# aehogan/lammps-induced-dipole-polarization-pair-style

Hardware: AMD Instinct MI355X
Metric: atom-steps/sec (higher is better)
Workload: dtype f64

## Files before the change

### lammps-induced-dipole-polarization-pair-style_amd/csrc/lab/api_env_knobs.inc

```
  if (const char *e = getenv("POLAR_ABLATE")) h->ablate = atoi(e);
  if (const char *e = getenv("POLAR_HOST_COLORS")) h->host_colors = atoi(e) != 0;
  if (const char *e = getenv("POLAR_SWEEP_KERNEL")) h->sweep_kernel = atoi(e);
  if (const char *e = getenv("POLAR_TILE_WAVES")) h->tile_waves = atoi(e) == 8 ? 8 : 4;
  if (const char *e = getenv("POLAR_TILE_WIDE")) h->tile_wide = atoi(e) != 0;
  if (const char *e = getenv("POLAR_CACHE_R2")) h->cache_r2 = atoi(e);
  if (const char *e = getenv("POLAR_LJ_TYPED")) h->lj_typed = atoi(e) != 0;
  if (const char *e = getenv("POLAR_STATIC_XQ")) h->static_xq = atoi(e) != 0;
  if (const char *e = getenv("POLAR_POL_FIRST")) h->pol_first = atoi(e) != 0;
  if (const char *e = getenv("POLAR_LP_WG_PER_CU")) h->lp_wg_per_cu = atoi(e);
  if (const char *e = getenv("POLAR_LP_QM")) h->lp_quad_major = atoi(e) != 0;
  if (const char *e = getenv("POLAR_LP_TILES")) h->lp_tiles = atoi(e) == 1 ? 1 : 2;
  if (const char *e = getenv("POLAR_LP_ROWS")) h->lp_rows = std::max(1, std::min(64, atoi(e)));
  if (const char *e = getenv("POLAR_LP_PAIRS")) h->lp_pairs = atoi(e) != 0;
  if (const char *e = getenv("POLAR_CLUSTER_DIST")) h->cluster_dist = atof(e);
  if (const char *e = getenv("POLAR_CLUSTER_MAX")) h->cluster_max = std::max(1, std::min(4, atoi(e)));
  if (const char *e = getenv("POLAR_LP_DEPTH")) { int v = atoi(e); h->lp_depth = (v == 2 || v == 3) ? v : 0; }
  if (const char *e = getenv("POLAR_QUAD_BLOCK")) { int v = atoi(e); if (v >= 64 && v <= 1024 && v % 64 == 0) h->quad_block = v; }
  if (const char *e = getenv("POLAR_FIELD_BLOCK")) { int v = atoi(e); if (v >= 64 && v <= 1024 && v % 64 == 0) h->field_block = v; }
  if (const char *e = getenv("POLAR_FORCE_LITERAL")) h->force_literal = atoi(e) != 0;
  if (const char *e = getenv("POLAR_NL_DENSE")) h->nl_dense = atoi(e) != 0;
```

### lammps-induced-dipole-polarization-pair-style_amd/csrc/polar_api.hip

```cpp
#include "polar_handle.hpp"

namespace {
void upload_types(polar_handle *h, int ntypes, const double *const t[7]) {
  need_device(h);
  std::vector<double> pack;
  const double r_cmax = pack_lj_table(ntypes, t, pack);
  h->d_lj.ensure(pack.size());
  HIPCHECK(hipMemcpy(h->d_lj.p, pack.data(), pack.size() * sizeof(double), hipMemcpyHostToDevice));
  h->P.ntypes = ntypes;
  h->P.ljpack = h->d_lj.p;
  h->ntypes = ntypes;
  h->types_set = true;
  h->r_cmax = r_cmax;
  h->skin_valid = false;
}

void upload_coul(polar_handle *h, double g_ewald, double qqrd2e, const double *slj, const double *scoul, int nbits,
                 int mask, int shift, double tabinnersq, const double *const t[8]) {
  need_device(h);
  h->P.g_ewald = g_ewald; h->P.qqrd2e = qqrd2e;
  for (int k = 0; k < 4; k++) { h->P.special_lj[k] = slj[k]; h->P.special_coul[k] = scoul[k]; }
  h->P.ncoultablebits = nbits; h->P.ncoulmask = mask; h->P.ncoulshiftbits = shift; h->P.tabinnersq = tabinnersq;
  std::vector<double> pack;
  pack_coul_table(nbits, t, pack);
// ... 100 lines not shown
      const long long lo = t0 + cnt * part / nt, hi = t0 + cnt * (part + 1) / nt;
      int a = (int)(std::lower_bound(at.begin() + ii0, at.begin() + ii1, lo) - at.begin());
      const int b = (int)(std::lower_bound(at.begin() + ii0, at.begin() + ii1, hi) - at.begin());
      int worst = 0;
      for (; a < b; a++) {
        const int i = ilist[a], m = numneigh[i];
        const int *src = row(i);
        int *d = dst + (at[a] - t0);
        int mx = 0;
        for (int k = 0; k < m; k++) { const int v = src[k]; d[k] = v; const int j = v & 0x3FFFFFFF; mx = j > mx ? j : mx; }
        worst = mx > worst ? mx : worst;
      }
      if (worst >= nall) bad[(size_t)part * 16] = 1;
    }, nt);
    for (int t = 0; t < nt; t++) if (bad[(size_t)t * 16]) { HIPCHECK(hipStreamSynchronize(s)); throw InputError("neighbor index out of range"); }
    if (cnt > 0) HIPCHECK(hipMemcpyAsync(h->d_neigh.p + t0, dst, (size_t)cnt * sizeof(int), hipMemcpyHostToDevice, s));
    HIPCHECK(hipEventRecord(h->ev_nl[buf], s));
    ii0 = ii1; chunk++;
  }
  HIPCHECK(hipEventRecord(h->ev_list_up, s));
  h->list_up_pending = true;
  h->neigh_set = true;
  h->sym_valid = false; h->lj_ran = false;
  if (h->colors_valid) h->colors_recheck = true;
  h->device_list = false;
  h->full_list = h->user_full_list;
}
}


extern "C" {

const char *polar_kernel_version(void) { return POLAR_KERNEL_VERSION; }

int polar_device_count(void) {
  int n = 0;
  if (hipGetDeviceCount(&n) != hipSuccess) return 0;
  return n;
}

int polar_create(int device, polar_handle **out) {
  if (!out) return POLAR_ERR_STATE;
  polar_handle *h = new polar_handle();
  *out = h;
  h->device = device;
  if (const char *e = getenv("POLAR_COLOR_DIST")) h->color_dist = atof(e);
  h->color_keep = std::max(h->color_dist - 0.4, 0.75 * h->color_dist);
  if (const char *e = getenv("POLAR_COLOR_KEEP")) h->color_keep = atof(e);
  if (const char *e = getenv("POLAR_DETERMINISTIC")) h->deterministic = atoi(e) != 0;
#ifdef POLAR_LAB
#include "lab/api_env_knobs.inc"
#endif
  int n = polar_device_count();
  if (n <= 0 || device < 0 || device >= n) {
    h->have_device = false;
    h->err = "no usable HIP device";
    return POLAR_OK;
  }
  return guarded(h, [&]() {
    HIPCHECK(hipSetDevice(device));
    h->device_set = true;
    h->stream.create();
    for (auto &e : h->ev) e.create();
    {
      int prio_lo = 0, prio_hi = 0;
      HIPCHECK(hipDeviceGetStreamPriorityRange(&prio_lo, &prio_hi));
      h->lj_stream.create(hipStreamNonBlocking, prio_lo);
    }
    h->ev_fork.create(); h->ev_join.create();
    h->ev_lj0.create(); h->ev_lj1.create();
    h->ev_dl0.create(hipEventDisableTiming); h->ev_dl1.create(hipEventDisableTiming);
    h->ev_mu_ready.create(hipEventDisableTiming);
    for (auto &e : h->ev_fchunk) e.create(hipEventDisableTiming);
    for (auto &e : h->ev_ks) e.create();
    h->dl_stream.create(hipStreamNonBlocking);
    if (getenv("POLAR_NO_OVERLAP")) h->overlap_lj = false;
    if (const char *e = getenv("POLAR_LJ_PERS")) h->lj_pers = atoi(e);
    if (const char *e = getenv("POLAR_LJ_SKIN")) h->lj_skin = atoi(e) != 0;
    if (const char *e = getenv("POLAR_NL_INERT")) h->nl_inert = atoi(e) != 0;
    if (const char *e = getenv("POLAR_CELL_INERT")) h->cell_inert = atoi(e) != 0;
    if (const char *e = getenv("POLAR_LJ_PERS_THREADS")) h->lj_pers_threads = std::max(256, std::min(POLAR_LJ_PERS_THREADS, (atoi(e) / 64) * 64));
    { int ncu = 0; if (hipDeviceGetAttribute(&ncu, hipDeviceAttributeMultiprocessorCount, device) == hipSuccess) h->ncu = ncu; }
    h->h_scal.ensure(1);
    h->h_flags.ensure(16);
    h->h_ddtot.ensure(64 * 16);
    h->d_overflow.ensure(16); h->d_ddtot.ensure(64 * 16);
    h->d_scal.ensure(1);
    h->d_slots.ensure((size_t)POLAR_NSLOT * POLAR_SLOT_STRIDE);
    h->have_device = true;
    return POLAR_OK;
  });
}

int polar_destroy(polar_handle *h) {
  if (!h) return POLAR_OK;
  delete h;
  return POLAR_OK;
}

const char *polar_last_error(const polar_handle *h) { return h ? h->err.c_str() : "null handle"; }
const char *polar_last_warning(const polar_handle *h) { return h ? h->warn.c_str() : ""; }

int polar_pair_settings(polar_handle *h, int narg, const char *const *arg) {
  return guarded(h, [&]() { h->ph.settings(narg, arg); h->reset_plan(); return POLAR_OK; });
}
int polar_pair_coeff(polar_handle *h, int ntypes, int narg, const char *const *arg) {
  return guarded(h, [&]() { h->ph.coeff(ntypes, narg, arg); return POLAR_OK; });
}
int polar_pair_modify(polar_handle *h, int narg, const char *const *arg) {
  return guarded(h, [&]() { h->ph.modify(narg, arg); return POLAR_OK; });
}
int polar_pair_init(polar_handle *h, double g_ewald, double qqrd2e, const double special_lj[4],
                    const double special_coul[4]) {
  return guarded(h, [&]() {
    PairHost &p = h->ph;
    p.init(g_ewald, qqrd2e, special_lj, special_coul);
    h->coul_set = false;
    h->field_ready = false;
    if (h->have_device) {
      HIPCHECK(hipSetDevice(h->device));
      const double *t[7] = {p.lj1.data(), p.lj2.data(), p.lj3.data(), p.lj4.data(), p.offset.data(), p.cut_ljsq.data(), p.cutsq.data()};
      upload_types(h, p.ntypes, t);
      if (p.ncoultablebits == 0) {
        const double *c[8];
        double dummy = 0.0;
        for (int k = 0; k < 8; k++) c[k] = &dummy;
        upload_coul(h, g_ewald, qqrd2e, special_lj, special_coul, 0, 0, 0, 0.0, c);
      }
    }
    return POLAR_OK;
  });
}
double polar_pair_cut(const polar_handle *h, int i, int j) {
  if (!h || !h->ph.inited || i < 1 || j < 1 || i > h->ph.ntypes || j > h->ph.ntypes) return -1.0;
  return std::sqrt(h->ph.cutsq[(size_t)i * h->ph.w() + j]);
}
double polar_pair_single(const polar_handle *h, double qi, double qj, int itype, int jtype, double rsq,
                         double factor_coul, double factor_lj, double *fforce) {
  double ff = 0.0, e;
  try {
    e = h->ph.single(qi, qj, itype, jtype, rsq, factor_coul, factor_lj, ff);
  } catch (const std::exception &ex) {
    const_cast<polar_handle *>(h)->err = ex.what();
    e = ff = std::nan("");
  }
  if (fforce) *fforce = ff;
  return e;
}
const void *polar_pair_extract(const polar_handle *h, const char *name, int *dim) {
  if (!h || !name) return nullptr;
  if (dim) *dim = 0;
  if (strcmp(name, "cut_coul") == 0) return &h->ph.st.cut_coul;
  if (strcmp(name, "nl_dense") == 0) return &h->nl_dense_used;
  if (strcmp(name, "lj_walked") == 0 || strcmp(name, "lj_entries") == 0) {
    polar_handle *m = const_cast<polar_handle *>(h);
    if (guarded(m, [&]() { lj_counters(m); return POLAR_OK; }) != POLAR_OK) return nullptr;
    return name[3] == 'w' ? &h->lj_walked : &h->lj_entries;
  }
  if (strcmp(name, "cell_active") == 0) {
    polar_handle *m = const_cast<polar_handle *>(h);
    m->cell_active = 0.0;
    if (h->have_device && h->sorted && h->ph.st.dd_cutoff > 0.0 && h->ncell > 0 && h->d_cell_first.p) {
      long long v = 0;
      if (guarded(m, [&]() {
            HIPCHECK(hipSetDevice(m->device));
            HIPCHECK(hipMemcpyAsync(&v, m->d_cell_first.p + m->ncell, sizeof(v), hipMemcpyDeviceToHost, m->stream));
            HIPCHECK(hipStreamSynchronize(m->stream));
            return POLAR_OK;
          }) != POLAR_OK) return nullptr;
      m->cell_active = (double)v;
    }
    return &h->cell_active;
  }
  if (strcmp(name, "nl_entries") == 0 || strcmp(name, "force_rows") == 0) {
    polar_handle *m = const_cast<polar_handle *>(h);
    if (guarded(m, [&]() { inert_counters(m); return POLAR_OK; }) != POLAR_OK) return nullptr;
    return name[0] == 'n' ? &h->nl_entries : &h->force_rows;
  }
  if (strcmp(name, "ewald_field_at_ms") == 0) { if (dim) *dim = 1; return h->ew_fa_ms; }
  if (strcmp(name, "ewald_field_ms") == 0) { if (dim) *dim = 0; return &h->ew_field_ms; }
  if (dim) *dim = 2;
  if (strcmp(name, "epsilon") == 0) return h->ph.epsilon.data();
  if (strcmp(name, "sigma") == 0) return h->ph.sigma.data();
  if (strcmp(name, "cut_lj") == 0) return h->ph.cut_lj.data();
  return nullptr;
}
int polar_get_settings(const polar_handle *h, polar_settings *out) {
  if (!h || !out) return POLAR_ERR_STATE;
  *out = h->ph.st;
  return POLAR_OK;
}
int polar_restart_pack(const polar_handle *h, void *buf, int max_bytes) {
  if (!h) return POLAR_ERR_STATE;
  return restart_pack(h->ph.st, buf, max_bytes);
}
int polar_restart_unpack(polar_handle *h, const void *buf, int nbytes) {
  return guarded(h, [&]() {
    h->ph.st = restart_unpack(h->ph.st, buf, nbytes);
    h->reset_plan();
    return POLAR_OK;
  });
}
int polar_set_settings(polar_handle *h, const polar_settings *s) {
  return guarded(h, [&]() {
    check_solver_choice(*s);
    polar_settings v = *s;
    if (v.polar_sor == 0.0) v.polar_sor = 1.0;
    if (!(v.polar_sor > 0.0 && v.polar_sor < 2.0)) throw InputError("polar_sor must lie in (0, 2)");
    if (v.polar_accel < 0 || v.polar_accel > POLAR_ACCEL_MAX) throw InputError("polar_accel must lie in 0 .. 8");
    if (!(v.polar_ewald >= 0.0 && v.polar_ewald < 1.0)) throw InputError("polar_ewald must lie in [0, 1)");
    h->ph.st = v;
    h->colors_valid = false;
    h->field_ready = false;
    return POLAR_OK;
  });
}
int polar_set_types(polar_handle *h, int ntypes, const double *lj1, const double *lj2, const double *lj3,
                    const double *lj4, const double *offset, const double *cut_ljsq, const double *cutsq) {
  return guarded(h, [&]() {
    HIPCHECK(hipSetDevice(h->device));
    const double *t[7] = {lj1, lj2, lj3, lj4, offset, cut_ljsq, cutsq};
    upload_types(h, ntypes, t);
    return POLAR_OK;
  });
}
int polar_set_coul(polar_handle *h, double g_ewald, double qqrd2e, const double special_lj[4],
                   const double special_coul[4], int nbits, int mask, int shift, double tabinnersq,
                   const double *rtable, const double *drtable, const double *ftable, const double *dftable,
                   const double *ctable, const double *dctable, const double *etable, const double *detable) {
  return guarded(h, [&]() {
    const double *c[8] = {rtable, drtable, ftable, dftable, ctable, dctable, etable, detable};
    h->ph.set_tables(nbits, mask, shift, tabinnersq, c);
    h->field_ready = false;
    h->ph.g_ewald = g_ewald; h->ph.qqrd2e = qqrd2e;
    for (int k = 0; k < 4; k++) { h->ph.special_lj[k] = special_lj[k]; h->ph.special_coul[k] = special_coul[k]; }
    if (h->have_device) {
      HIPCHECK(hipSetDevice(h->device));
      double dummy = 0.0;
      if (nbits <= 0) for (int k = 0; k < 8; k++) c[k] = &dummy;
      upload_coul(h, g_ewald, qqrd2e, special_lj, special_coul, nbits > 0 ? nbits : 0, mask, shift, tabinnersq, c);
    }
    return POLAR_OK;
  });
}

int polar_set_box(polar_handle *h, const double boxlo[3], const double prd[3], const double tilt[3],
                  const int periodic[3], int triclinic) {
  return guarded(h, [&]() {
    const bool tri = triclinic != 0;
    Box nb{};
    nb.triclinic = tri ? 1 : 0;
    nb.xy = tri && tilt ? tilt[0] : 0.0;
    nb.xz = tri && tilt ? tilt[1] : 0.0;
    nb.yz = tri && tilt ? tilt[2] : 0.0;
    bool same = h->box_set;
    for (int k = 0; k < 3; k++) {
      if (!(prd[k] > 0.0) || !std::isfinite(prd[k])) throw InputError("box lengths must be positive and finite");
      nb.prd[k] = prd[k]; nb.half[k] = 0.5 * prd[k]; nb.inv[k] = 1.0 / prd[k]; nb.periodic[k] = periodic[k] ? 1 : 0;
      same = same && h->boxlo[k] == boxlo[k] && h->box.prd[k] == nb.prd[k] && h->box.periodic[k] == nb.periodic[k];
      h->boxlo[k] = boxlo[k];
    }
    same = same && h->box.triclinic == nb.triclinic && h->box.xy == nb.xy && h->box.xz == nb.xz && h->box.yz == nb.yz;
    h->box = nb;
    h->box_set = true;
    h->field_ready = false;
    if (!same) h->colors_valid = false;
    return POLAR_OK;
  });
}

int polar_set_atoms(polar_handle *h, int nlocal, int nghost, const double *x, const double *q, const double *alpha,
                    const int *type, const int *molecule) {
  return guarded(h, [&]() {
    need_device(h);
    HIPCHECK(hipSetDevice(h->device));
    if (nlocal < 0 || nghost < 0) throw InputError("negative atom count");
    h->force_ran = false;
    h->field_ready = false;
    const size_t nall = (size_t)nlocal + nghost;
    const size_t words = 3 * nall + nall + nall + (nall + 1) / 2 + (nall + 1) / 2 + 8;
    double *st = staging(h, std::max(words, 3 * nall + 6 * (size_t)nlocal));
    double *sx = st, *sq = sx + 3 * nall, *sa = sq + nall;
    int *stype = reinterpret_cast<int *>(sa + nall), *smol = stype + 2 * ((nall + 1) / 2);
    struct Ext { double lo[3], hi[3]; int bad, neg; char pad[56]; };
    const int nparts = nall < (1u << 14) ? 1 : std::min(8, HostPool::get().width());
    Ext ext[8];
    for (auto &e : ext) { for (int k = 0; k < 3; k++) { e.lo[k] = 1e300; e.hi[k] = -1e300; } e.bad = e.neg = 0; }
    const size_t per = ((nall + nparts - 1) / nparts + 3) / 4 * 4;
    HostPool::get().run([&](int part) {
      Ext &e = ext[part];
      const size_t a0 = std::min(nall, (size_t)part * per), a1 = std::min(nall, ((size_t)part + 1) * per);
      if (!scan_positions(x, sx, a0, a1, e.lo, e.hi)) e.bad = 1;
      memcpy(sq + a0, q + a0, (a1 - a0) * sizeof(double));
      memcpy(sa + a0, alpha + a0, (a1 - a0) * sizeof(double));
      memcpy(stype + a0, type + a0, (a1 - a0) * sizeof(int));
      memcpy(smol + a0, molecule + a0, (a1 - a0) * sizeof(int));
      double amin = 0.0;
      for (size_t k = a0; k < a1; k++) amin = alpha[k] < amin ? alpha[k] : amin;
      if (amin < 0.0) e.neg = 1;
    }, nparts);
    for (const auto &e : ext) {
      if (e.bad) throw InputError("non-finite atom coordinate");
      if (e.neg) throw InputError("Invalid value in set command");
    }
    if (nlocal != h->nlocal) { h->colors_valid = false; h->mu_resident = false; }
    else if (h->colors_valid) {
// ... 598 lines not shown
```

### lammps-induced-dipole-polarization-pair-style_amd/csrc/polar_common.hpp

```cpp
#pragma once

#include <hip/hip_runtime.h>
#include <stdint.h>

#ifdef POLAR_LAB
#define POLAR_LAB_PARAM , int ablate
#define POLAR_LAB_PASS , ablate
#define POLAR_ABL(bit) (ablate & (bit))
#else
#define POLAR_LAB_PARAM
#define POLAR_LAB_PASS
#define POLAR_ABL(bit) 0
#endif

namespace polar {


struct __attribute__((aligned(64))) AtomRec {
  double x, mx;
  double y, my;
  double z, mz;
  double q, a;
};

struct Box {
  double prd[3], half[3], inv[3];
  double xy, xz, yz;
  int periodic[3];
  int triclinic;
};

struct Scal {
  double eng_vdwl, eng_coul, u_self, u_ef, u_dd;
  double virial[6];
  double change;
  double last_change;
  unsigned long long rmin_bits;
  int iterations, done, status, cur, sweeps, pad;
  double det_change;
};

#define POLAR_NSLOT 1024
#define POLAR_SLOT_STRIDE 16
enum { SL_EVDWL = 0, SL_ECOUL, SL_USELF, SL_UEF, SL_UDD, SL_V0, SL_V1, SL_V2, SL_V3, SL_V4, SL_V5, SL_CHANGE, SL_RMIN };
__device__ __forceinline__ double *slot_ptr(double *slots, int field) {
  return slots + (size_t)(blockIdx.x & (POLAR_NSLOT - 1)) * POLAR_SLOT_STRIDE + field;
}

#define POLAR_WAVE 64
#define POLAR_BLOCK 256
#define POLAR_ROWS_PER_BLOCK (POLAR_BLOCK / POLAR_WAVE)

template <int CTRL, int ROWMASK>
__device__ __forceinline__ double dpp_get(double v) {
  const int lo = __builtin_amdgcn_update_dpp(0, __double2loint(v), CTRL, ROWMASK, 0xF, false);
  const int hi = __builtin_amdgcn_update_dpp(0, __double2hiint(v), CTRL, ROWMASK, 0xF, false);
  return __hiloint2double(hi, lo);
}
__device__ __forceinline__ int xcd_block(int b, int nblocks) {
  const int chunk = (nblocks + 7) >> 3;
  const int lb = (b & 7) * chunk + (b >> 3);
  return lb < nblocks ? lb : -1;
}

template <int CTRL>
__device__ __forceinline__ double dpp_full(double v) {
  const int lo = __builtin_amdgcn_update_dpp(0, __double2loint(v), CTRL, 0xF, 0xF, true);
  const int hi = __builtin_amdgcn_update_dpp(0, __double2hiint(v), CTRL, 0xF, 0xF, true);
  return __hiloint2double(hi, lo);
}
__device__ __forceinline__ double wave_uniform(double v) {
  const int lo = __builtin_amdgcn_readfirstlane(__double2loint(v));
  const int hi = __builtin_amdgcn_readfirstlane(__double2hiint(v));
  return __hiloint2double(hi, lo);
}
__device__ __forceinline__ AtomRec uniform_rec(const AtomRec &r) {
  AtomRec u;
  u.x = wave_uniform(r.x); u.mx = wave_uniform(r.mx); u.y = wave_uniform(r.y); u.my = wave_uniform(r.my);
  u.z = wave_uniform(r.z); u.mz = wave_uniform(r.mz); u.q = wave_uniform(r.q); u.a = wave_uniform(r.a);
  return u;
}
__device__ __forceinline__ double lane63(double v) {
  const int lo = __builtin_amdgcn_readlane(__double2loint(v), 63);
  const int hi = __builtin_amdgcn_readlane(__double2hiint(v), 63);
  return __hiloint2double(hi, lo);
}
__device__ __forceinline__ double wave_sum(double v) {
  v += dpp_full<0xB1>(v);
  v += dpp_full<0x4E>(v);
  v += dpp_full<0x141>(v);
  v += dpp_full<0x140>(v);
  v += dpp_get<0x142, 0xA>(v);
  v += dpp_get<0x143, 0xC>(v);
  return lane63(v);
}
__device__ __forceinline__ double wave_min(double v) {
#pragma unroll
  for (int off = 32; off > 0; off >>= 1) v = fmin(v, __shfl_xor(v, off, 64));
  return v;
}

__device__ __forceinline__ double wrap_ci(double d, double L, double h, int periodic) {
  if (periodic) {
    if (d < 0.0) {
      while (d < 0.0) d += L;
      if (d > h) d -= L;
    } else {
      while (d > 0.0) d -= L;
      if (d < -h) d += L;
    }
  }
  return d;
}

__device__ __forceinline__ void min_image_del(const Box &b, double xi, double yi, double zi, double xj, double yj,
                                              double zj, double &dx, double &dy, double &dz) {
  if (!b.triclinic) {
    dx = -wrap_ci(xj - xi, b.prd[0], b.half[0], b.periodic[0]);
    dy = -wrap_ci(yj - yi, b.prd[1], b.half[1], b.periodic[1]);
    dz = -wrap_ci(zj - zi, b.prd[2], b.half[2], b.periodic[2]);
    return;
  }
  double ex = xj - xi, ey = yj - yi, ez = zj - zi;
  if (b.periodic[2]) {
    if (ez < 0.0) {
      while (ez < 0.0) { ez += b.prd[2]; ey += b.yz; ex += b.xz; }
      if (ez > b.half[2]) { ez -= b.prd[2]; ey -= b.yz; ex -= b.xz; }
    } else {
      while (ez > 0.0) { ez -= b.prd[2]; ey -= b.yz; ex -= b.xz; }
      if (ez < -b.half[2]) { ez += b.prd[2]; ey += b.yz; ex += b.xz; }
    }
  }
  if (b.periodic[1]) {
    if (ey < 0.0) {
      while (ey < 0.0) { ey += b.prd[1]; ex += b.xy; }
      if (ey > b.half[1]) { ey -= b.prd[1]; ex -= b.xy; }
    } else {
      while (ey > 0.0) { ey -= b.prd[1]; ex -= b.xy; }
      if (ey < -b.half[1]) { ey += b.prd[1]; ex += b.xy; }
    }
  }
  ex = wrap_ci(ex, b.prd[0], b.half[0], b.periodic[0]);
  dx = -ex; dy = -ey; dz = -ez;
}

__device__ __forceinline__ double quad_xor(double v, const int which) {
  int lo = __double2loint(v), hi = __double2hiint(v);
  if (which == 1) {
    lo = __builtin_amdgcn_update_dpp(0, lo, 0xB1, 0xF, 0xF, true);
    hi = __builtin_amdgcn_update_dpp(0, hi, 0xB1, 0xF, 0xF, true);
  } else {
    lo = __builtin_amdgcn_update_dpp(0, lo, 0x4E, 0xF, 0xF, true);
    hi = __builtin_amdgcn_update_dpp(0, hi, 0x4E, 0xF, 0xF, true);
  }
  return __hiloint2double(hi, lo);
}
__device__ __forceinline__ double quad_sum(double v) {
  v += quad_xor(v, 1);
  v += quad_xor(v, 2);
  return v;
}

struct RowList {
  const int *cnt;
  long long pitch;
};
__device__ __forceinline__ void row_range(const RowList &L, int i, long long &beg, long long &end) {
  beg = (long long)i * L.pitch;
  const long long c = L.cnt[i];
  end = beg + (c < L.pitch ? c : L.pitch);
}

__device__ __forceinline__ void min_image_rint(const Box &b, double xi, double yi, double zi, double xj, double yj,
                                               double zj, double &dx, double &dy, double &dz) {
  double ex = xi - xj, ey = yi - yj, ez = zi - zj;
  const double nz = b.periodic[2] ? rint(ez * b.inv[2]) : 0.0;
  ez = fma(-b.prd[2], nz, ez); ey = fma(-b.yz, nz, ey); ex = fma(-b.xz, nz, ex);
  const double ny = b.periodic[1] ? rint(ey * b.inv[1]) : 0.0;
  ey = fma(-b.prd[1], ny, ey); ex = fma(-b.xy, ny, ex);
  const double nx = b.periodic[0] ? rint(ex * b.inv[0]) : 0.0;
  ex = fma(-b.prd[0], nx, ex);
  dx = ex; dy = ey; dz = ez;
}
template <bool TRI>
__device__ __forceinline__ bool min_image_rint_w(const Box &b, double xi, double yi, double zi, double xj, double yj,
                                                 double zj, double &dx, double &dy, double &dz) {
  double ex = xi - xj, ey = yi - yj, ez = zi - zj;
  const double nz = b.periodic[2] ? rint(ez * b.inv[2]) : 0.0;
  ez = fma(-b.prd[2], nz, ez);
  if (TRI) { ey = fma(-b.yz, nz, ey); ex = fma(-b.xz, nz, ex); }
  const double ny = b.periodic[1] ? rint(ey * b.inv[1]) : 0.0;
  ey = fma(-b.prd[1], ny, ey);
  if (TRI) ex = fma(-b.xy, ny, ex);
  const double nx = b.periodic[0] ? rint(ex * b.inv[0]) : 0.0;
  ex = fma(-b.prd[0], nx, ex);
  dx = ex; dy = ey; dz = ez;
  return nz != 0.0 || ny != 0.0 || nx != 0.0;
}
template <bool TRI>
__device__ __forceinline__ unsigned long long min_image_rint_m(const Box &b, double xi, double yi, double zi, double xj, double yj,
                                                               double zj, double &dx, double &dy, double &dz) {
  double ex = xi - xj, ey = yi - yj, ez = zi - zj;
  const double nz = rint(ez * b.inv[2]);
  ez = fma(-b.prd[2], nz, ez);
  if (TRI) { ey = fma(-b.yz, nz, ey); ex = fma(-b.xz, nz, ex); }
  const double ny = rint(ey * b.inv[1]);
  ey = fma(-b.prd[1], ny, ey);
  if (TRI) ex = fma(-b.xy, ny, ex);
  const double nx = rint(ex * b.inv[0]);
  ex = fma(-b.prd[0], nx, ex);
  dx = ex; dy = ey; dz = ez;
  return __builtin_amdgcn_ballot_w64(nz != 0.0) | __builtin_amdgcn_ballot_w64(ny != 0.0) | __builtin_amdgcn_ballot_w64(nx != 0.0);
}
__host__ __device__ __forceinline__ void frac_coords(const Box &b, const double lo[3], double x, double y, double z, double fr[3]) {
  fr[2] = (z - lo[2]) * b.inv[2];
  if (b.triclinic) {
    fr[1] = ((y - lo[1]) - b.yz * fr[2] * 1.0) * b.inv[1];
    fr[0] = ((x - lo[0]) - b.xy * fr[1] - b.xz * fr[2]) * b.inv[0];
  } else {
    fr[1] = (y - lo[1]) * b.inv[1];
    fr[0] = (x - lo[0]) * b.inv[0];
  }
}
template <bool EXACT>
__device__ __forceinline__ void pair_del(const Box &b, double xi, double yi, double zi, double xj, double yj,
                                         double zj, double &dx, double &dy, double &dz) {
  if (EXACT) min_image_del(b, xi, yi, zi, xj, yj, zj, dx, dy, dz);
  else min_image_rint(b, xi, yi, zi, xj, yj, zj, dx, dy, dz);
}

__host__ __device__ __forceinline__ long long lp_slot(long long e, int qm = 1) {
  const long long p = e & 63;
  const long long lane = qm ? (((p & 15) << 2) | (p >> 4)) : p;
  return ((e >> 8) << 8) + (lane << 2) + ((e >> 6) & 3);
}
__host__ __device__ __forceinline__ unsigned lp_slot32(unsigned e, int qm) {
  const unsigned p = e & 63u;
  const unsigned lane = qm ? (((p & 15u) << 2) | (p >> 4)) : p;
  return (e & ~255u) + (lane << 2) + ((e >> 6) & 3u);
}

#define POLAR_NL_SAMEMOL 0x40000000
#define POLAR_NL_MASK 0x3FFFFFFF

enum { SITE_INERT = 0, SITE_CHARGED = 1, SITE_POLAR = 2 };
__host__ __device__ __forceinline__ bool site_is_inert(double q, double alpha) { return q == 0.0 && alpha == 0.0; }

// ... 148 lines not shown
```

### lammps-induced-dipole-polarization-pair-style_amd/csrc/polar_handle.hpp

```cpp
#pragma once
#include <hip/hip_runtime.h>

#include <algorithm>
#include <initializer_list>
#include <utility>
#include <chrono>
#include <cmath>
#include <cstdio>
#include <cstdlib>
#include <exception>
#include <cstring>
#include <numeric>
#include <string>
#include <thread>
#include <mutex>
#include <condition_variable>
#include <functional>
#include <memory>
#include <stdexcept>
#include <unistd.h>
#include <vector>

#include "pair_host.hpp"
#include "polar_input.hpp"
// ... 23 lines not shown
inline int nblk_xcd(long long n, int per) { return ((nblk(n, per) + 7) / 8) * 8; }

inline double min_image_dist2(const Box &b, const double *xi, const double *xj) {
  double d[3] = {xi[0] - xj[0], xi[1] - xj[1], xi[2] - xj[2]};
  if (b.triclinic) {
    if (b.periodic[2]) { const double n = std::nearbyint(d[2] / b.prd[2]); d[2] -= n * b.prd[2]; d[1] -= n * b.yz; d[0] -= n * b.xz; }
    if (b.periodic[1]) { const double n = std::nearbyint(d[1] / b.prd[1]); d[1] -= n * b.prd[1]; d[0] -= n * b.xy; }
    if (b.periodic[0]) d[0] -= b.prd[0] * std::nearbyint(d[0] / b.prd[0]);
  } else {
    for (int k = 0; k < 3; k++)
      if (b.periodic[k]) d[k] -= b.prd[k] * std::nearbyint(d[k] / b.prd[k]);
  }
  return d[0] * d[0] + d[1] * d[1] + d[2] * d[2];
}

struct polar_handle {
  int device = -1;
  bool have_device = false;
  bool device_set = false;
  Stream stream;
  std::string err, warn;
  PairHost ph;
  bool types_set = false, coul_set = false, box_set = false, atoms_set = false, neigh_set = false;
  int ntypes = 0;
  LJCoulParams P{};
  Box box{};
  double boxlo[3] = {0, 0, 0};
  int nlocal = 0, nghost = 0;
  int row_lo = 0, row_hi = -1;
  int full_list = 0;
  int newton_pair = 1;
  int step_eflag = 0, step_vflag = 0;
  bool in_step = false;
  std::vector<double> hx, halpha;
  DBuf<double> d_x, d_q, d_alpha, d_f, d_ef, d_F, d_mu, d_rank, d_dmu, d_tab, d_lj;
  DBuf<int> d_type, d_mol, d_order, d_pos, d_ilist, d_numneigh, d_neigh, d_rows;
  DBuf<int> d_mol_s, d_perm, d_inv, d_rows_orig, d_ownrows;
  DBuf<double> d_ef_s, d_T6, d_Minv, d_gsN, d_gsAT, d_cb, d_gs_part, d_eatom, d_vatom, d_dd_r2, d_fpol;
  bool dense_gs = false;
  CellGrid grid{};
  long long ncell = 0;
  bool sorted = false;
  DBuf<long long> d_first, d_sym_first;
  DBuf<int> d_gs_cnt;
  DBuf<long long> d_scan_a, d_scan_b;
  DBuf<int> d_sym_cnt, d_sym_fill, d_sym_j;
  bool sym_valid = false;
  DBuf<long long> d_sym_cfirst;
  DBuf<int> d_sym_cend, d_lj_walk;
  DBuf<unsigned char> d_sym_cls;
  DBuf<double4> d_xq_snap;
  DBuf<unsigned long long> d_lj_drift;
  double r_cmax = 0.0;
  int lj_skin = 1;
  bool skin_valid = false;
  int skin_nall = 0;
  bool lj_ran = false;
  bool lj_sym_last = false, lj_walk_last = false; int lj_rows_last = 0;
  double lj_walked = 0.0, lj_entries = 0.0;
  int nl_inert = 1;
  int cell_inert = 1;
  bool cell_split = false;
  double cell_active = 0.0;
  bool force_ran = false, force_listed = false; int force_nrows = 0;
  double nl_entries = 0.0, force_rows = 0.0;
  DBuf<unsigned long long> d_inert_sums;
  DBuf<AtomRec> d_rec0, d_rec1;
  DBuf<Scal> d_scal;
  DBuf<double> d_slots;
  DBuf<int> d_cell_id, d_cell_cnt, d_cell_fill, d_nl_cnt, d_dd_cnt, d_nl_j, d_dd_j, d_dd_wrap;
  DBuf<long long> d_cell_first, d_nl_first, d_dd_first;
  DBuf<double2> d_dd_s;
  DBuf<int2> d_lpdesc;
  DBuf<double> d_lp_pend;
  DBuf<double> d_lp_part;
  int lp_npart = 0;
  DBuf<int> d_slot;
  std::vector<int> h_cl;
  DBuf<int> d_cl_orig, d_cl_cnt, d_cl_wrap, d_cl_tw;
  DBuf<int4> d_cl_s;
  long long cl_pitch = 0;
  int ncl = 0;
  double cluster_dist = 2.0;
  int cluster_max = 4;
  long long cl_slots = 0;
  DBuf<double4> d_xq, d_pos4, d_xq_s;
  long long nl_pairs = 0, dd_pairs = 0;
  long long nl_pitch = 0, dd_pitch = 0;
  DBuf<int> d_overflow;
  DBuf<unsigned long long> d_ddtot;
  PinBuf<int> h_flags;
  PinBuf<unsigned long long> h_ddtot;
  int inum = 0;
  long long nneigh = 0;
  bool mu_resident = false;
  DBuf<double> d_dbgf;
  DBuf<double> d_acc_x, d_acc_f, d_acc_g, d_acc_dF, d_acc_dG, d_acc_part;
  DBuf<AccelState> d_acc_state;
  long long acc_pitch = 0; int acc_rows = 0;
  DBuf<double> d_mu0;
  bool mu0_saved = false;
  int attempt = 0;
  int last_sweeps = 0;
  bool mu_host_in_sync = false;
  std::vector<int> color_off;
  std::vector<int> color_sub;
  int color_nsub = 1;
  DBuf<int> d_bflag; int bflag_n = 0;
  std::vector<PinBuf<int>> h_nl_stage; std::vector<Event> ev_nl;
  Stream up_stream; Event ev_list_up; bool list_up_pending = false;
  std::vector<long long> h_first; std::vector<int> h_nn, h_ilist;
  bool colors_global = false;
  std::vector<int> user_colors;
  bool user_colors_clashed = false;
  std::vector<int> h_rows;
  bool colors_valid = false;
  double color_keep = 2.0;
  bool slots_by_color = false;
  long long color_epoch = 0;
  long long slots_epoch = -1;
  bool colors_recheck = false;
  std::vector<int> h_color;
  DBuf<int> d_color_orig, d_color_s;
  DBuf<int> d_klist;
  DBuf<int> d_cadj, d_cdeg, d_ccnt, d_cflags, d_crelabel;
  DBuf<unsigned long long> d_cprio;
  DBuf<double> d_cstat;
  DBuf<long long> d_coff;
  PinBuf<int> h_cflags;
  PinBuf<double> h_cstat;
  PinBuf<long long> h_coff;
  int cadj_pitch = 16;
  int host_colors = 0;
  int colors_reused = 0, colors_rebuilt = 0;
  double ms_color_host = 0.0;
  double color_dist = 2.4;
  int field_block = 256;
  double bbox_lo[3] = {0, 0, 0}, bbox_hi[3] = {0, 0, 0};
  long long global_count = 0;
  DBuf<double> d_xchg; DBuf<int> d_xidx;
  bool device_list = false;
  int user_full_list = 0;
  long long lj_pitch = 0;
  DBuf<double4> d_ljpos; DBuf<int2> d_ljaux; DBuf<int> d_tag, d_nspecial, d_special, d_ljcell_id, d_ljcell_cnt, d_ljcell_fill; DBuf<long long> d_ljcell_first; DBuf<double> d_cutneighsq;
  int lj_typed = 1;
  bool lj_tab_arith = false;
  int lj_pers = 1;
  int ncu = 0;
  int lj_pers_threads = 768;
  bool sym_typed = false, dev_typed = false;
  int static_xq = 1;
  int pol_first = 1;
  double nl_dense_used = 1.0;
#ifdef POLAR_LAB
  int nl_dense = 1;
  int force_literal = 0;
#endif
  int part_k = 0, part_n = 1;
  int lp_wg_per_cu = 0;
  int lp_quad_major = 1;
  int quad_block = POLAR_BLOCK;
  int lp_tiles = 2;
  int lp_rows = 1;
  int lp_pairs = 0;
  DBuf<int> d_ulead, d_udd_j;
  DBuf<long long> d_upos;
  DBuf<int2> d_unit;
  DBuf<int4> d_udesc;
  std::vector<int> unit_off;
  long long upitch = 0;
  int lp_depth = 0;
  int cache_r2 = -1;
  int stream_mode = 1;
  int sweep_kernel = 2;
  int ablate = 0;
  DBuf<SRec> d_srec0, d_srec1;
  DBuf<TileHdr> d_thdr;
  DBuf<TileRowEnt> d_trow;
  DBuf<int> d_un_j;
  DBuf<unsigned short> d_dd16;
  DBuf<double> d_pend;
  int un_pitch = 0;
  int un_lds = 0;
  long long pitch16 = 0;
  int tile_max_u = 0;
  bool tile_reported = false;
  double dens = 0.0;
  std::vector<TileLaunch> tile_launches;
  TileLaunch tile_all{};
  size_t tile_lds_attr[16] = {0, 0, 0, 0, 0, 0, 0, 0, 0, 0, 0, 0, 0, 0, 0, 0};
  size_t tile_build_lds_attr = 0;
  int tile_waves = 4;
  int tile_wide = 0;
  int tile_sw[3] = {2, 2, 2};
  int deterministic = 0;
  PinBuf<Scal> h_scal;
  Event ev[8];
  Stream lj_stream;
  Event ev_fork, ev_join, ev_lj0, ev_lj1, ev_dl0, ev_dl1;
  Stream dl_stream;
  Event ev_mu_ready;
  double *early_mu = nullptr, *early_ef = nullptr, *user_mu = nullptr, *user_ef = nullptr;
  Event ev_fchunk[4];
  bool overlap_lj = true;
  bool lj_forked = false;
  std::vector<double> h_tmp;
  PinBuf<double> h_stage;
  DBuf<double> d_trace;
  DBuf<double4> d_ew_kv; DBuf<int4> d_ew_hkl, d_ew_rows;
  DBuf<double2> d_ew_s, d_ew_m, d_ew_part;
  DBuf<double> d_ew_erec, d_ew_vpart, d_ew_out;
  std::vector<double> ew_key;
  int ew_nk = 0, ew_nrow = 0, ew_nm = 0;
  double ew_cell[6] = {0, 0, 0, 0, 0, 0};
  Event ev_ks[4];
  int ntrace = 0;
  bool field_ready = false;
  DBuf<double> d_fa_x, d_fa_out;
  DBuf<int> d_fa_idx;
  Event ev_fa[2];
  DBuf<double> d_fa_part, d_fa_q;
  bool ew_q_valid = false;
  Event ev_fa_k;
  double ew_fa_ms[2] = {0.0, 0.0};
  double ew_field_ms = 0.0;
  ~polar_handle() {
    if (!device_set) return;
    (void)hipSetDevice(device);
    for (hipStream_t s : {(hipStream_t)stream, (hipStream_t)lj_stream, (hipStream_t)up_stream, (hipStream_t)dl_stream})
      if (s) (void)hipStreamSynchronize(s);
  }
  void reset_plan() { field_ready = false; colors_valid = false; nl_pitch = dd_pitch = 0; cl_pitch = 0; un_pitch = 0; pitch16 = 0; }
};
inline int fail(polar_handle *h, int code, const std::string &m) {
  if (h) h->err = m;
  return code;
}

template <typename F>
int guarded(polar_handle *h, F &&fn) {
  if (!h) return POLAR_ERR_STATE;
  try {
    return fn();
  } catch (...) {
    return error_code(h->err);
  }
}

inline double *staging(polar_handle *h, size_t count) {
  if (count > h->h_stage.cap) {
    if (h->h_stage.p) {
      if (h->stream) (void)hipStreamSynchronize(h->stream);
      if (h->dl_stream) (void)hipStreamSynchronize(h->dl_stream);
    }
    h->h_stage.release();
    h->h_stage.ensure(count + count / 4 + 1024);
  }
  return h->h_stage.p;
}

inline void need_device(polar_handle *h) {
  if (!h->have_device) throw NoDevice();
}

class HostPool {
 public:
  static HostPool &get() { static HostPool p; return p; }
  int width() const { return (int)th_.size() + 1; }
  void run(const std::function<void(int)> &fn, int parts) {
    if (parts <= 1 || th_.empty() || getpid() != pid_) { for (int k = 0; k < parts; k++) fn(k); return; }
    std::unique_lock<std::mutex> job(job_m_);
    {
      std::lock_guard<std::mutex> g(m_);
      fn_ = &fn; parts_ = parts; pending_ = std::min(parts - 1, (int)th_.size()); gen_++; failed_ = nullptr;
    }
    cv_.notify_all();
    std::exception_ptr mine;
    try {
      fn(0);
      for (int k = (int)th_.size() + 1; k < parts; k++) fn(k);
    } catch (...) { mine = std::current_exception(); }
    std::unique_lock<std::mutex> g(m_);
    done_.wait(g, [&] { return pending_ == 0; });
    fn_ = nullptr;
    std::exception_ptr theirs = failed_;
    failed_ = nullptr;
    g.unlock();
    if (mine) std::rethrow_exception(mine);
    if (theirs) std::rethrow_exception(theirs);
  }
 private:
  HostPool() {
    pid_ = getpid();
    const unsigned hw = std::thread::hardware_concurrency();
    const int n = hw >= 16 ? 7 : (hw >= 4 ? 3 : (hw >= 2 ? (int)hw - 1 : 0));
    for (int t = 0; t < n; t++) th_.emplace_back([this, t]() { loop(t); });
  }
  ~HostPool() {
    { std::lock_guard<std::mutex> g(m_); stop_ = true; gen_++; }
    cv_.notify_all();
    for (auto &t : th_) t.join();
  }
  void loop(int t) {
    unsigned long long seen = 0;
    for (;;) {
      const std::function<void(int)> *fn = nullptr;
      int part = -1;
// ... 100 lines not shown
```

### lammps-induced-dipole-polarization-pair-style_amd/csrc/polar_lists.hpp

```cpp
#pragma once

#include "polar_common.hpp"
#include "polar_nl_dense.hpp"
#include "polar_plan.hpp"

namespace polar {

struct CellGrid {
  int trim;
  int nc[3];
  double lo[3], inv[3];
};

__device__ __forceinline__ int cell_of(const CellGrid &g, const Box &b, double x, double y, double z) {
  int c[3];
  double fr3[3];
  frac_coords(b, g.lo, x, y, z, fr3);
#pragma unroll
  for (int k = 0; k < 3; k++) {
    double fr = fr3[k];
    fr -= floor(fr);
    int ck = (int)(fr * g.nc[k]);
    c[k] = ck >= g.nc[k] ? g.nc[k] - 1 : ck;
  }
// ... 309 lines not shown
  }
}
static __global__ __launch_bounds__(64) void k_color_ball(const int *__restrict__ count, int cap, const int *__restrict__ list, const int *__restrict__ prev,
                                                   int *__restrict__ state, const double4 *__restrict__ pos4, Box box, double reachsq, int top, int hops,
                                                   int budget, int apitch, const int *__restrict__ adj, const int *__restrict__ deg, int *__restrict__ color_s) {
  __shared__ int ball[64];
  const int m_all = *count;
  const int w = blockIdx.x, lane = threadIdx.x;
  if (m_all > cap || w >= m_all) return;
  if (prev[w]) { if (lane == 0) state[w] = 1; return; }
  const int v = list[w];
  const double4 rv = pos4[v];
  bool blocked = false;
  for (int q = lane; q < w; q += 64) {
    if (prev[q]) continue;
    const double4 rq = pos4[list[q]];
    double dx, dy, dz;
    min_image_del(box, rv.x, rv.y, rv.z, rq.x, rq.y, rq.z, dx, dy, dz);
    blocked |= dx * dx + dy * dy + dz * dz < reachsq;
  }
  if (__ballot(blocked)) { if (lane == 0) state[w] = 0; return; }
  if (lane == 0) state[w] = 1;
  if (lane == 0) ball[0] = v;
  int m = 1, level0 = 0;
  __syncthreads();
  for (int hop = 0; hop < hops; hop++) {
    const int level1 = m;
    for (int q = level0; q < level1 && m < 64; q++) {
      const int node = ball[q];
      const int d = deg[node];
      int j = lane < d ? adj[(size_t)node * apitch + lane] : -1;
      if (j >= 0 && deg[j] < 0) j = -1;
      if (j >= 0) for (int k = 0; k < m; k++) if (ball[k] == j) { j = -1; break; }
      const unsigned long long fresh = __ballot(j >= 0);
      const int at = m + __popcll(fresh & ((1ull << lane) - 1ull));
      if (j >= 0 && at < 64) ball[at] = j;
      m = min(64, m + __popcll(fresh));
      __syncthreads();
    }
    level0 = level1;
  }
  unsigned long long in = 0ull, allow = 0ull;
  if (lane < m) {
    const int node = ball[lane];
    unsigned long long used = 0ull;
    const int d = deg[node];
    for (int k = 0; k < d; k++) {
      const int j = adj[(size_t)node * apitch + k];
      int at = -1;
      for (int q = 0; q < m; q++) if (ball[q] == j) { at = q; break; }
      if (at >= 0) in |= 1ull << at;
      else { const int cj = color_s[j]; if (cj >= 0) used |= 1ull << cj; }
    }
    allow = ~used & ((1ull << top) - 1ull);
  }
  int mycol = -1;
  int k = 0;
  for (int step = 0; step < budget && k >= 0 && k < m; step++) {
    const unsigned long long ek = __shfl(in, k, 64) & ((1ull << k) - 1ull);
    const bool nb = (ek >> lane) & 1ull;
    unsigned long long ok = __shfl(allow, k, 64);
    for (int c = 0; c < top; c++)
      if (((ok >> c) & 1ull) && __ballot(nb && mycol == c)) ok &= ~(1ull << c);
    const int cur = __shfl(mycol, k, 64);
    if (cur >= 0) ok &= ~((2ull << cur) - 1ull);
    if (ok) {
      const int c = __ffsll((long long)ok) - 1;
      if (lane == k) mycol = c;
      k++;
      if (lane == k) mycol = -1;
    } else {
      if (lane == k) mycol = -1;
      k--;
    }
  }
  if (k >= m && lane < m) color_s[ball[lane]] = mycol;
}
static __global__ void k_color_regroup(int n, const int *__restrict__ deg, const int *__restrict__ class_rank, const int *__restrict__ perm,
                                int *__restrict__ color_s, unsigned long long *__restrict__ prio) {
  const int i = blockIdx.x * blockDim.x + threadIdx.x;
  if (i >= n || deg[i] < 0) return;
  const unsigned o = (unsigned)perm[i];
  prio[i] = ((unsigned long long)(63 - class_rank[color_s[i]]) << 56) | ((unsigned long long)(color_hash(o) >> 8) << 32) | o;
  color_s[i] = -1;
}
static __global__ __launch_bounds__(256) void k_color_stats(int n, const int *__restrict__ color_s, const double *__restrict__ rank,
                                                     double *__restrict__ sums, const int *__restrict__ perm, int own_lo, int own_hi) {
  __shared__ double part[128];
  if (threadIdx.x < 128) part[threadIdx.x] = 0.0;
  __syncthreads();
  const int i = blockIdx.x * blockDim.x + threadIdx.x;
  int c = i < n ? color_s[i] : -1;
  if (c >= 0) { const int o = perm[i]; if (o < own_lo || o >= own_hi) c = -1; }
  if (c >= 0) {
    atomicAdd(&part[2 * c], 1.0);
    atomicAdd(&part[2 * c + 1], rank ? rank[i] : 1.0);
  }
  __syncthreads();
  if (threadIdx.x < 128 && part[threadIdx.x] != 0.0) atomicAdd(sums + threadIdx.x, part[threadIdx.x]);
}
static __global__ void k_color_relabel(int n, const int *__restrict__ relabel, const int *__restrict__ perm, int *__restrict__ color_s,
                                int *__restrict__ color_orig) {
  const int i = blockIdx.x * blockDim.x + threadIdx.x;
  if (i >= n) return;
  const int c = color_s[i] >= 0 ? relabel[color_s[i]] : -1;
  color_s[i] = c;
  color_orig[perm[i]] = c;
}
__device__ __forceinline__ int color_class(int j, const int *__restrict__ color_s, const int *__restrict__ perm, int own_lo, int own_hi,
                                           const int *__restrict__ sub, int nsub) {
  const int c = color_s[j];
  if (c < 0) return -1;
  const int o = perm[j];
  if (o < own_lo || o >= own_hi) return -1;
  return sub ? nsub * c + sub[o] : c;
}
static __global__ void k_color_cellcount(long long ncell, int nclass, const long long *__restrict__ cell_first, const int *__restrict__ npol,
                                  const int *__restrict__ color_s, int *__restrict__ cnt, const int *__restrict__ perm, int own_lo, int own_hi,
                                  const int *__restrict__ sub, int nsub) {
  const long long c = blockIdx.x * (long long)blockDim.x + threadIdx.x;
  if (c >= ncell) return;
  const int a = (int)cell_first[c], e = a + npol[c];
  for (int q = 0; q < nclass; q++) {
    int k = 0;
    for (int j = a; j < e; j++) k += color_class(j, color_s, perm, own_lo, own_hi, sub, nsub) == q;
    cnt[(size_t)q * ncell + c] = k;
  }
}
static __global__ void k_color_fill(long long ncell, int nclass, const long long *__restrict__ cell_first, const int *__restrict__ npol,
                             const int *__restrict__ color_s, const int *__restrict__ perm, const long long *__restrict__ off,
                             int *__restrict__ rows_orig, int own_lo, int own_hi, const int *__restrict__ sub, int nsub) {
  const long long c = blockIdx.x * (long long)blockDim.x + threadIdx.x;
  if (c >= ncell) return;
  const int a = (int)cell_first[c], e = a + npol[c];
  for (int q = 0; q < nclass; q++) {
    long long w = off[(size_t)q * ncell + c];
    for (int j = a; j < e; j++) if (color_class(j, color_s, perm, own_lo, own_hi, sub, nsub) == q) rows_orig[w++] = perm[j];
  }
}

__device__ __forceinline__ int prefix_count(unsigned long long m, int base) {
  return __builtin_amdgcn_mbcnt_hi((unsigned)(m >> 32), __builtin_amdgcn_mbcnt_lo((unsigned)m, base));
}
struct NlRunLanes {
  int s0v, k0v, s1v, k1v, endv;
  unsigned m1;
  __device__ __forceinline__ int s0(int sr) const { return __builtin_amdgcn_readlane(s0v, sr); }
  __device__ __forceinline__ int k0(int sr) const { return __builtin_amdgcn_readlane(k0v, sr); }
  __device__ __forceinline__ int s1(int sr) const { return __builtin_amdgcn_readlane(s1v, sr); }
  __device__ __forceinline__ int k1(int sr) const { return __builtin_amdgcn_readlane(k1v, sr); }
  __device__ __forceinline__ int end(int sr) const { return __builtin_amdgcn_readlane(endv, sr); }
  __device__ __forceinline__ bool two(int sr) const { return (m1 >> sr) & 1u; }
};
template <bool TRI, bool RECHECK, bool DENSE = true>
static __global__ __launch_bounds__(POLAR_BLOCK) void k_nl_build(const int *__restrict__ rows, int nrows,
                                                          const double4 *__restrict__ pos4, Box box, CellGrid g,
                                                          const long long *__restrict__ cell_first, double cutallsq,
                                                          double ddcutsq, long long nl_pitch, long long dd_pitch,
                                                          int *__restrict__ nl_cnt, int *__restrict__ dd_cnt,
                                                          int *__restrict__ nl_j, int *__restrict__ dd_j,
                                                          double *__restrict__ dd_r2, int pad_dd,
                                                          int dd_shift_qm, int dd_pad_index, int *__restrict__ dd_wrap,
                                                          const int *__restrict__ color_s, double colordistsq,
                                                          int *__restrict__ color_conflict,
                                                          const int *__restrict__ dd_slot,
                                                          int *__restrict__ overflow,
                                                          unsigned long long *__restrict__ dd_total) {
  const int dd_shift = dd_shift_qm & 255, dd_qm = dd_shift_qm >> 8;
  const int lane = threadIdx.x & 63;
  const int row = blockIdx.x * POLAR_ROWS_PER_BLOCK + (threadIdx.x >> 6);
  if (row >= nrows) return;
  const int i = __builtin_amdgcn_readfirstlane(rows ? rows[row] : row);
  const double4 ri = pos4[i];
  const int imol = __double2hiint(ri.w), ipol = __double2loint(ri.w) >= SITE_POLAR;
  const int icol = (RECHECK && color_s && ipol) ? color_s[i] : -2;
  bool clash = RECHECK && color_s && ipol && icol < 0;
  int cc[3];
  double uu[3], edge[3];
  {
    double fr3[3];
    frac_coords(box, g.lo, ri.x, ri.y, ri.z, fr3);
#pragma unroll
    for (int k = 0; k < 3; k++) {
      double fr = fr3[k];
      fr -= floor(fr);
      const double t = fr * g.nc[k];
      int ck = (int)t;
      ck = ck >= g.nc[k] ? g.nc[k] - 1 : ck;
      cc[k] = __builtin_amdgcn_readfirstlane(ck);
      uu[k] = wave_uniform(t - ck); edge[k] = wave_uniform(box.prd[k] / g.nc[k]);
    }
  }
  const int c0 = cc[0], c1 = cc[1], c2 = cc[2];
  const int slot_i = __builtin_amdgcn_readfirstlane(dd_slot ? dd_slot[i] : i);
  const long long nl0 = (long long)i * nl_pitch, dd0 = (long long)(slot_i >= 0 ? slot_i : 0) * dd_pitch;
  char *const nl_row = reinterpret_cast<char *>(nl_j + nl0), *const dd_row = reinterpret_cast<char *>(dd_j + dd0);
  char *const r2_row = reinterpret_cast<char *>(dd_r2 ? dd_r2 + dd0 : nullptr);
  const char *const pos_b = reinterpret_cast<const char *>(pos4);
  const int nl_cap = (int)nl_pitch, dd_cap = (int)dd_pitch;
  const unsigned long long dd_im = (ipol && slot_i >= 0) ? ~0ull : 0ull;
  Box pbox = box;
#pragma unroll
  for (int k = 0; k < 3; k++) { pbox.inv[k] = box.periodic[k] ? box.inv[k] : 0.0; pbox.periodic[k] = 1; }
  int ncount = 0, dcount = 0;
  unsigned long long wrap_m = 0ull;
  const int same_i = imol != 0 ? POLAR_NL_SAMEMOL : 0;
  const unsigned long long below = (lane == 0) ? 0ull : (~0ull >> (64 - lane));
  const int n0 = g.nc[0], n1 = g.nc[1], n2 = g.nc[2];
  const int zlo = n2 >= 5 ? c2 - 2 : 0, zcnt = n2 >= 5 ? 5 : n2;
  const int ylo = n1 >= 5 ? c1 - 2 : 0, ycnt = n1 >= 5 ? 5 : n1;
  const double reach = sqrt(cutallsq > ddcutsq ? cutallsq : ddcutsq) + 1e-6;
  const double reach2 = wave_uniform(reach * reach);
  const int nsr = zcnt * ycnt;
  int ra0 = 0, rb0 = 0, ra1 = 0, rb1 = 0;
  if (lane < nsr) {
    const int lz = (lane >= ycnt) + (lane >= 2 * ycnt) + (lane >= 3 * ycnt) + (lane >= 4 * ycnt);
    const int zz = zlo + lz, yy = ylo + (lane - lz * ycnt);
    int b2 = zz, b1 = yy;
    bool ok = true;
    if (b2 < 0 || b2 >= n2) { if (!box.periodic[2]) ok = false; b2 = b2 < 0 ? b2 + n2 : b2 - n2; }
    if (b1 < 0 || b1 >= n1) { if (!box.periodic[1]) ok = false; b1 = b1 < 0 ? b1 + n1 : b1 - n1; }
    double dzmin = 0.0, dymin = 0.0;
    if (n2 >= 5) { const int d = zz - c2; dzmin = d > 0 ? (d - uu[2]) * edge[2] : (d < 0 ? (uu[2] - (d + 1)) * edge[2] : 0.0); }
    if (n1 >= 5) { const int d = yy - c1; dymin = d > 0 ? (d - uu[1]) * edge[1] : (d < 0 ? (uu[1] - (d + 1)) * edge[1] : 0.0); }
    const double rem2 = reach2 - dzmin * dzmin - dymin * dymin;
    if (g.trim && rem2 < 0.0) ok = false;
    int xlo = n0 >= 5 ? c0 - 2 : 0, xhi = n0 >= 5 ? c0 + 2 : n0 - 1;
    if (ok && g.trim && n0 >= 5) {
      const double xr = sqrt(rem2) / edge[0];
      int lo_off = (int)floor(uu[0] - xr), hi_off = (int)floor(uu[0] + xr);
      lo_off = lo_off < -2 ? -2 : lo_off; hi_off = hi_off > 2 ? 2 : hi_off;
      xlo = c0 + lo_off; xhi = c0 + hi_off;
    }
    if (ok) {
      const long long rowbase = ((long long)b2 * n1 + b1) * n0;
      const int xa = xlo < 0 ? 0 : xlo, xb = xhi >= n0 ? n0 - 1 : xhi;
      ra0 = (int)cell_first[rowbase + xa]; rb0 = (int)cell_first[rowbase + xb + 1];
      if (box.periodic[0]) {
        if (xlo < 0) { ra1 = (int)cell_first[rowbase + xlo + n0]; rb1 = (int)cell_first[rowbase + n0]; }
        else if (xhi >= n0) { ra1 = (int)cell_first[rowbase]; rb1 = (int)cell_first[rowbase + xhi - n0 + 1]; }
      }
    }
  }
  auto candidate = [&](const int p, const bool valid) {
    const int j = valid ? p : i;
    const double4 rj = *reinterpret_cast<const double4 *>(pos_b + ((unsigned)j << 5));
    double ex, ey, ez;
    const unsigned long long shifted = min_image_rint_m<TRI>(pbox, ri.x, ri.y, ri.z, rj.x, rj.y, rj.z, ex, ey, ez);
    const double rsq = ex * ex + ey * ey + ez * ez;
    const unsigned long long m_pair = __builtin_amdgcn_ballot_w64(j != i);
    const int jkind = __double2loint(rj.w);
    const unsigned long long m_nl = m_pair & __builtin_amdgcn_ballot_w64(rsq <= cutallsq) & __builtin_amdgcn_ballot_w64(jkind != SITE_INERT);
    const unsigned long long m_dd = m_pair & dd_im & __builtin_amdgcn_ballot_w64(jkind >= SITE_POLAR) & __builtin_amdgcn_ballot_w64(rsq < ddcutsq);
    wrap_m |= m_dd & shifted;
    const bool in_nl = (j != i) & (rsq <= cutallsq) & (jkind != SITE_INERT);
    const bool in_dd = (j != i) & (dd_im != 0ull) & (jkind >= SITE_POLAR) & (rsq < ddcutsq);
    if (RECHECK) { if (icol >= 0 && j != i && rsq < colordistsq && jkind >= SITE_POLAR && color_s[j] == icol) clash = true; }
    int jmol = __double2hiint(rj.w);
    asm("" : "+v"(jmol));
    const int same = imol == jmol ? same_i : 0;
    const int kn = prefix_count(m_nl, ncount), kd = prefix_count(m_dd, dcount);
    if (in_nl && kn < nl_cap) *reinterpret_cast<int *>(nl_row + ((unsigned)kn << 2)) = j | same;
    if (in_dd && kd < dd_cap) {
      *reinterpret_cast<int *>(dd_row + ((dd_shift ? lp_slot32((unsigned)kd, dd_qm) : (unsigned)kd) << 2)) = j << dd_shift;
      if (dd_r2) *reinterpret_cast<double *>(r2_row + ((unsigned)kd << 3)) = rsq;
    }
    ncount += __popcll(m_nl);
    dcount += __popcll(m_dd);
  };
  if (DENSE) {
    const int len = nl_run_len(ra0, rb0, ra1, rb1);
    int inc = len;
    inc += __builtin_amdgcn_update_dpp(0, inc, 0x111, 0xF, 0xF, true);
    inc += __builtin_amdgcn_update_dpp(0, inc, 0x112, 0xF, 0xF, true);
    inc += __builtin_amdgcn_update_dpp(0, inc, 0x114, 0xF, 0xF, true);
    inc += __builtin_amdgcn_update_dpp(0, inc, 0x118, 0xF, 0xF, true);
    const int row0 = __builtin_amdgcn_readlane(inc, 15);
    inc += (lane >= 16 && lane < 32) ? row0 : 0;
    const int total = __builtin_amdgcn_readlane(inc, 31);
    const NlRunEntry e = nl_run_entry(ra0, rb0, ra1, rb1, inc - len);
    const NlRunLanes tab{e.s0, e.k0, e.s1, e.k1, e.end, (unsigned)__ballot(rb1 > ra1)};
    unsigned rem = (unsigned)__ballot(len > 0);
    for (int t0 = 0; t0 < total; t0 += 64) {
      const int g = t0 + lane;
      const int k = nl_dense_shift(tab, rem, t0, g);
      candidate(g + k, g < total);
    }
  } else {
    for (int sr = 0; sr < nsr; sr++) {
#pragma unroll
      for (int piece = 0; piece < 2; piece++) {
        const int a = __builtin_amdgcn_readlane(piece ? ra1 : ra0, sr), b = __builtin_amdgcn_readlane(piece ? rb1 : rb0, sr);
        for (int base = a; base < b; base += 64) candidate(base + lane, base + lane < b);
      }
    }
  }
  if (pad_dd) {
    const int have = dcount < dd_pitch ? dcount : (int)dd_pitch;
    const int padded = (have + 63) & ~63;
    for (int k = have + lane; k < padded; k += 64) {
      dd_j[dd0 + (dd_shift ? lp_slot(k, dd_qm) : (long long)k)] = (dd_pad_index >= 0 ? dd_pad_index : i) << dd_shift;
      if (dd_r2) dd_r2[dd0 + k] = 1e60;
    }
  }
  if (RECHECK && color_s && __ballot(clash) != 0ull && lane == 0) atomicOr(color_conflict, 1);
  if (lane == 0) {
    nl_cnt[i] = ncount; dd_cnt[i] = dcount;
    if (dd_wrap) dd_wrap[i] = wrap_m != 0ull;
    if (ncount > nl_pitch || dcount > dd_pitch) atomicMax(overflow, ncount > dcount ? ncount : dcount);
    if (dcount) atomicAdd(dd_total + (blockIdx.x & 63) * 16, (unsigned long long)(dcount < dd_pitch ? dcount : (int)dd_pitch));
  }
}

#ifdef POLAR_LAB
#include "lab/lists_paired_rows.hpp"
#endif

#ifdef POLAR_LAB
#include "lab/lists_cluster_rows.hpp"
#endif

struct LJGrid {
  int nc[3];
  double lo[3], inv[3];
};
__device__ __forceinline__ int lj_cell_of(const LJGrid &g, double x, double y, double z) {
  const double p[3] = {x, y, z};
  int c[3];
#pragma unroll
  for (int k = 0; k < 3; k++) {
    int ck = (int)floor((p[k] - g.lo[k]) * g.inv[k]);
    c[k] = ck < 0 ? 0 : (ck >= g.nc[k] ? g.nc[k] - 1 : ck);
  }
  return (c[2] * g.nc[1] + c[1]) * g.nc[0] + c[0];
}
static __global__ void k_lj_cell_count(int nall, const double *__restrict__ x, LJGrid g, int *__restrict__ cell_id,
                                int *__restrict__ cell_cnt) {
  int i = blockIdx.x * blockDim.x + threadIdx.x;
  if (i >= nall) return;
  const int c = lj_cell_of(g, x[3 * i], x[3 * i + 1], x[3 * i + 2]);
  cell_id[i] = c;
  atomicAdd(&cell_cnt[c], 1);
}
static __global__ void k_lj_cell_fill(int nall, const int *__restrict__ cell_id, const long long *__restrict__ cell_first,
                               int *__restrict__ fill, const double *__restrict__ x, const int *__restrict__ type,
                               const int *__restrict__ mol, const int *__restrict__ tag, double4 *__restrict__ pos,
                               int2 *__restrict__ aux) {
  int i = blockIdx.x * blockDim.x + threadIdx.x;
  if (i >= nall) return;
  const int c = cell_id[i];
  const int s = (int)cell_first[c] + atomicAdd(&fill[c], 1);
  pos[s] = make_double4(x[3 * i], x[3 * i + 1], x[3 * i + 2], __hiloint2double(mol[i], type[i]));
  aux[s] = make_int2(i, tag ? tag[i] : i + 1);
}

static __global__ __launch_bounds__(POLAR_BLOCK) void k_lj_nl_build(int row_lo, int nrows, int ntypes, const double *__restrict__ x,
                                                             const int *__restrict__ type, const int *__restrict__ mol,
                                                             const double4 *__restrict__ pos, const int2 *__restrict__ aux,
                                                             LJGrid g, const long long *__restrict__ cell_first,
                                                             const double *__restrict__ cutneighsq, Box box,
                                                             int exclude_intra, const int *__restrict__ nspecial,
                                                             const int *__restrict__ special, int maxspecial, int sf1,
                                                             int sf2, int sf3, long long pitch, int *__restrict__ cnt,
                                                             int *__restrict__ out_j, int *__restrict__ overflow,
                                                             unsigned long long *__restrict__ total, int typed) {
  extern __shared__ double cn_lds[];
  const int w = ntypes + 1;
  for (int t = threadIdx.x; t < w * w; t += blockDim.x) cn_lds[t] = cutneighsq[t];
  __syncthreads();
  const int lane = threadIdx.x & 63;
  const int r_ = blockIdx.x * POLAR_ROWS_PER_BLOCK + (threadIdx.x >> 6);
  if (r_ >= nrows) return;
  const int i = row_lo + r_;
  const double xi = x[3 * i], yi = x[3 * i + 1], zi = x[3 * i + 2];
  const int itype = type[i], imol = mol[i];
  const double *cn = cn_lds + itype * w;
  int n1 = 0, n2 = 0, n3 = 0;
  if (nspecial) { n1 = nspecial[3 * i]; n2 = nspecial[3 * i + 1]; n3 = nspecial[3 * i + 2]; }
  const int *sp = special ? special + (size_t)i * maxspecial : nullptr;
  const int ci = lj_cell_of(g, xi, yi, zi);
  const int n0 = g.nc[0], n1c = g.nc[1], n2c = g.nc[2];
// ... 180 lines not shown
```

### lammps-induced-dipole-polarization-pair-style_amd/csrc/polar_plan.hpp

```cpp
#pragma once

#include <algorithm>
#include <cmath>
#include <cstddef>
#include <vector>

namespace polar {

constexpr double PLAN_PI = 3.14159265358979323846;

struct PlanD4 { double x, y, z, w; };
struct PlanI4 { int x, y, z, w; };

inline int nblk(long long n, int per) { return n <= 0 ? 1 : (int)((n + per - 1) / per); }

template <class B>
inline void box_widths(const B &b, double w[3]) {
  w[0] = b.prd[0]; w[1] = b.prd[1]; w[2] = b.prd[2];
  if (!b.triclinic) return;
  const double vol = b.prd[0] * b.prd[1] * b.prd[2];
  const double bxc[3] = {b.prd[1] * b.prd[2], -b.xy * b.prd[2], b.xy * b.yz - b.prd[1] * b.xz};
  w[0] = vol / std::sqrt(bxc[0] * bxc[0] + bxc[1] * bxc[1] + bxc[2] * bxc[2]);
  w[1] = vol / (b.prd[0] * std::sqrt(b.prd[2] * b.prd[2] + b.yz * b.yz));
}
inline bool ewald_short_box(const double width[3], double cut_coul) {
  return cut_coul > 0.5 * std::min(width[0], std::min(width[1], width[2]));
}

inline bool list_grid(const double width[3], const int periodic[3], double cutall, int nc[3]) {
  for (int k = 0; k < 3; k++)
    if (periodic[k] && width[k] < 2.0 * cutall * (1.0 - 1e-12)) return false;
  for (int k = 0; k < 3; k++) nc[k] = std::max(1, (int)std::floor(width[k] / (0.5 * cutall)));
  return true;
}

#if defined(__HIPCC__)
#define POLAR_PLAN_FN __host__ __device__ inline
#else
#define POLAR_PLAN_FN inline
#endif
POLAR_PLAN_FN long long cell_bin(long long c, long long ncell, bool inert, bool split) { return (split && inert) ? ncell + c : c; }
struct CellBins { long long nbins, cnt, fill, fill_back, first; };
inline CellBins cell_bins(long long ncell, bool split) {
  const long long nb = split ? 2 * ncell : ncell;
  return CellBins{nb, nb + 1, 2 * (nb + 1), nb + 1, nb + 2};
}
inline bool cell_bins_fit(long long ncell, bool split) { return cell_bins(ncell, split).nbins < (1ll << 31) - 1; }

inline long long pitch_first(double mean, double factor) { return (((long long)(factor * mean) + 64) / 64 + 1) * 64; }
inline long long pitch_grown(int flag) { return ((long long)(1.25 * flag) / 64 + 1) * 64; }
inline int pitch_forced(int value) { return ((std::max(64, value) + 63) / 64) * 64; }

inline double occupied_volume(int n, const double *x, const double lo[3], const double prd[3], double cutall) {
  double vol = prd[0] * prd[1] * prd[2];
  int nc[3];
  long long tot = 1;
  for (int k = 0; k < 3; k++) { nc[k] = std::max(1, std::min(64, (int)(prd[k] / cutall))); tot *= nc[k]; }
  std::vector<char> occ((size_t)tot, 0);
  for (int a = 0; a < n; a++) {
    long long c = 0, mul = 1;
    for (int k = 0; k < 3; k++) {
      double fr = (x[3 * (size_t)a + k] - lo[k]) / prd[k];
      fr -= std::floor(fr);
      c += mul * std::min(nc[k] - 1, (int)(fr * nc[k]));
      mul *= nc[k];
    }
    occ[(size_t)c] = 1;
  }
  long long filled = 0;
  for (char v : occ) filled += v;
  if (filled > 0) vol *= (double)filled / (double)tot;
  return vol;
}

inline int stream_mode(int cache_r2, int sweep_kernel, long long dd_pairs, int own_rows, long long dd_pitch) {
  int mode = cache_r2;
  if (sweep_kernel == 1) mode = 0;
  if (sweep_kernel == 2) mode = 3;
  if (sweep_kernel >= 3) mode = 4;
  if (mode < 0) {
    const double est_pairs = dd_pairs > 0 ? (double)dd_pairs : 0.35 * (double)own_rows * (double)dd_pitch;
    mode = (12.0 * est_pairs < 200.0e6) ? 1 : 2;
  }
  return mode;
}

struct EwaldPlan {
  std::vector<PlanD4> kv;
  std::vector<PlanI4> hkl, rows;
  int nk = 0, nrow = 0, nm = 0;
  double cell[6] = {0, 0, 0, 0, 0, 0};
};
template <class B>
inline EwaldPlan ewald_kvectors(const B &b, double g, double acc) {
  EwaldPlan p;
  const double lx = b.prd[0], ly = b.prd[1], lz = b.prd[2], xy = b.xy, xz = b.xz, yz = b.yz;
  const double i00 = 1.0 / lx, i01 = -xy / (lx * ly), i02 = (xy * yz - ly * xz) / (lx * ly * lz), i11 = 1.0 / ly,
               i12 = -yz / (ly * lz), i22 = 1.0 / lz;
  const double vol = lx * ly * lz, twopi = 2.0 * PLAN_PI;
  const double kcut = 2.0 * g * std::sqrt(-std::log(acc)), kcut2 = kcut * kcut;
  const int hm = (int)std::floor(kcut * lx / twopi), km = (int)std::floor(kcut * std::sqrt(xy * xy + ly * ly) / twopi),
            lm = (int)std::floor(kcut * std::sqrt(xz * xz + yz * yz + lz * lz) / twopi);
  for (int ih = 0; ih <= hm; ih++)
    for (int ik = (ih == 0 ? 0 : -km); ik <= km; ik++) {
      int row = -1;
      for (int il = (ih == 0 && ik == 0 ? 1 : -lm); il <= lm; il++) {
        const double kx = twopi * (ih * i00), ky = twopi * (ih * i01 + ik * i11), kz = twopi * (ih * i02 + ik * i12 + il * i22);
        const double k2 = kx * kx + ky * ky + kz * kz;
        if (k2 > kcut2 || k2 == 0.0) continue;
        if (row < 0) { row = (int)p.rows.size(); p.rows.push_back(PlanI4{ih, ik, il, (int)p.kv.size()}); }
        p.kv.push_back(PlanD4{kx, ky, kz, 8.0 * PLAN_PI / vol * std::exp(-k2 / (4.0 * g * g)) / k2});
        p.hkl.push_back(PlanI4{ih, ik, il, 0});
      }
    }
  p.nk = (int)p.kv.size();
  p.nrow = (int)p.rows.size();
  p.rows.push_back(PlanI4{0, 0, 0, p.nk});
  p.nm = std::max(hm, std::max(km, lm));
  p.cell[0] = i00; p.cell[1] = i01; p.cell[2] = i02; p.cell[3] = i11; p.cell[4] = i12; p.cell[5] = i22;
  return p;
}

inline size_t ewald_lds_per_atom(int nm) { return 3 * (size_t)(nm + 1) * 16 + 3 * sizeof(double); }
inline int ewald_tile(int nm) { return (int)std::max<size_t>(1, std::min<size_t>(32, (48 * 1024) / ewald_lds_per_atom(nm))); }
struct SfacChunks { int kb, nchunk, chunk; };
inline SfacChunks ewald_sfac_chunks(int n, int nk, int tile) {
  SfacChunks c;
  c.kb = nblk(nk, 256);
  c.nchunk = std::max(1, std::min(nblk(std::max(n, 1), tile), nblk(4096, c.kb)));
  c.chunk = std::max(1, nblk(std::max(n, 1), c.nchunk));
  c.nchunk = nblk(std::max(n, 1), c.chunk);
  return c;
}

inline bool dense_gs_fits(int n) { return n > 64 && 48.0 * (double)n * (double)n <= 3.2e10; }
inline int dense_gs_block(int n) { return n >= 1024 ? 256 : n >= 384 ? 128 : 64; }

struct SweepEnd {
  bool mix;
  bool decide_in_mix;
  int count;
  bool reduce;
  bool jacobi;
};
inline SweepEnd sweep_end(int sw, int max_sweeps, bool fixed_iteration, bool gs, bool accel, int reduce_every) {
  const bool lazy = fixed_iteration && gs;
  SweepEnd e;
  e.mix = accel && (!lazy || sw < max_sweeps - 1);
  e.decide_in_mix = accel && !lazy;
  if (lazy) e.count = sw == max_sweeps - 2 ? max_sweeps - 1 : sw == max_sweeps - 1 ? 1 : 0;
  else e.count = accel ? 0 : 1;
  e.reduce = reduce_every > 0 && !fixed_iteration && !accel && ((sw % reduce_every) == reduce_every - 1 || sw >= max_sweeps - 1);
  e.jacobi = !gs;
  return e;
}
inline bool look_at_state(int last_sweeps, int sw, int every, int step = 1) {
  const int done_sweeps = sw + 1;
  const int pred = last_sweeps;
  if (pred <= 0) return (sw % every) == every - 1;
  if (done_sweeps < pred) return (done_sweeps % 16) == 0;
  const int past = done_sweeps - pred;
  if (past <= 4 * step) return (past % step) == 0;
  return (past % every) == 0;
}

}
```

### lammps-induced-dipole-polarization-pair-style_amd/csrc/polar_rows.hpp

```cpp
#pragma once

#include "polar_common.hpp"
#include "polar_force_pair.hpp"
#include "polar_skin.hpp"
#ifdef POLAR_LAB
#include "lab/force_pair_literal.hpp"
#define POLAR_LIT_PARAM , int literal
#define POLAR_LIT_PASS , literal
#else
#define POLAR_LIT_PARAM
#define POLAR_LIT_PASS
#endif

namespace polar {

static __global__ void k_pack(int n, const int *__restrict__ perm, const double *__restrict__ x, const double *__restrict__ q,
                       const double *__restrict__ alpha, const int *__restrict__ mol, const double *__restrict__ mu0,
                       AtomRec *__restrict__ r0, AtomRec *__restrict__ r1, int *__restrict__ mol_s,
                       double4 *__restrict__ pos4, double4 *__restrict__ xq_s, int wrap, Box box, double lo0, double lo1,
                       double lo2, int keep_inert) {
  int i = blockIdx.x * blockDim.x + threadIdx.x;
  if (i == n) {
    AtomRec d;
    d.x = n > 0 ? x[0] : 0.0; d.y = n > 0 ? x[1] : 0.0; d.z = n > 0 ? x[2] : 0.0;
    d.mx = d.my = d.mz = d.q = d.a = 0.0;
    r0[n] = d; r1[n] = d;
  }
  if (i >= n) return;
  const int o = perm ? perm[i] : i;
  AtomRec r;
  r.x = x[3 * o]; r.y = x[3 * o + 1]; r.z = x[3 * o + 2]; r.q = q[o];
  if (wrap) {
    const double lo[3] = {lo0, lo1, lo2};
    double fr[3];
    frac_coords(box, lo, r.x, r.y, r.z, fr);
    const double n2 = box.periodic[2] ? floor(fr[2]) : 0.0, n1 = box.periodic[1] ? floor(fr[1]) : 0.0,
                 n0 = box.periodic[0] ? floor(fr[0]) : 0.0;
    r.z -= n2 * box.prd[2]; r.y -= n2 * box.yz + n1 * box.prd[1]; r.x -= n2 * box.xz + n1 * box.xy + n0 * box.prd[0];
  }
  r.mx = mu0 ? mu0[3 * o] : 0.0; r.my = mu0 ? mu0[3 * o + 1] : 0.0; r.mz = mu0 ? mu0[3 * o + 2] : 0.0;
  r.a = alpha[o];
  r0[i] = r;
  r1[i] = r;
  mol_s[i] = mol[o];
  if (pos4) pos4[i] = make_double4(r.x, r.y, r.z, __hiloint2double(mol[o], r.a != 0.0 ? SITE_POLAR : ((site_is_inert(r.q, r.a) && !keep_inert) ? SITE_INERT : SITE_CHARGED)));
  if (xq_s) xq_s[i] = make_double4(r.x, r.y, r.z, r.q);
}

template <bool ALLPAIRS, int PASS>
static __global__ __launch_bounds__(POLAR_BLOCK) void k_rank(int nlocal, int ntotal, const double *__restrict__ x,
                                                      const double *__restrict__ alpha, const int *__restrict__ mol,
                                                      Box box, RowList nl,
                                                      const int *__restrict__ nl_j,
                                                      const AtomRec *__restrict__ rec,
                                                      const int *__restrict__ mol_s, Scal *scal,
                                                      double *__restrict__ slots,
                                                      double *__restrict__ rank_metric, int nchunk) {
  const int lane = threadIdx.x & 63;
  const int gw = blockIdx.x * POLAR_ROWS_PER_BLOCK + (threadIdx.x >> 6);
  if (gw >= nlocal * nchunk) return;
  const int i = gw % nlocal, chunk = gw / nlocal;
  const double xi = ALLPAIRS ? x[3 * i] : rec[i].x, yi = ALLPAIRS ? x[3 * i + 1] : rec[i].y,
               zi = ALLPAIRS ? x[3 * i + 2] : rec[i].z, ai = ALLPAIRS ? alpha[i] : rec[i].a;
  const int mi = ALLPAIRS ? mol[i] : mol_s[i];
  double rmin = (PASS == 1) ? 1000.0 : __longlong_as_double((long long)scal->rmin_bits);
  double rmin2 = 1.0e6;
  const double far2 = (rmin * 1.5) * (rmin * 1.5) * 1.000001;
  double acc = 0.0;
  long long beg = 0, end = ntotal;
  if (!ALLPAIRS) row_range(nl, i, beg, end);
  else if (nchunk > 1) { const long long per = ((ntotal + nchunk - 1) / nchunk + 255) / 256 * 256; beg = chunk * per; end = beg + per < ntotal ? beg + per : ntotal; }
  constexpr int U = ALLPAIRS ? 4 : 1;
  for (long long base = beg; base < end; base += 64 * U) {
    double px[U], py[U], pz[U], pa[U];
    int pj[U], pm[U];
#pragma unroll
    for (int u = 0; u < U; u++) {
      const long long p = base + 64 * u + lane;
      pj[u] = i;
      if (p < end) pj[u] = ALLPAIRS ? (int)p : (nl_j[p] & POLAR_NL_MASK);
      if (ALLPAIRS) {
        px[u] = x[3 * pj[u]]; py[u] = x[3 * pj[u] + 1]; pz[u] = x[3 * pj[u] + 2];
        pa[u] = alpha[pj[u]]; pm[u] = mol[pj[u]];
      } else {
        const AtomRec rj = rec[pj[u]];
        px[u] = rj.x; py[u] = rj.y; pz[u] = rj.z; pa[u] = rj.a; pm[u] = mol_s[pj[u]];
      }
    }
#pragma unroll
    for (int u = 0; u < U; u++) {
      bool hit = false;
      double term = 0.0;
      if (pj[u] != i) {
        double dx, dy, dz;
        if (ALLPAIRS) { dx = xi - px[u]; dy = yi - py[u]; dz = zi - pz[u]; }
        else min_image_rint(box, xi, yi, zi, px[u], py[u], pz[u], dx, dy, dz);
        const double rsq = dx * dx + dy * dy + dz * dz;
        const bool molok = (mi != pm[u]) || mi == 0;
        if (PASS == 1) {
          if (ai > 0 && pa[u] > 0 && molok) rmin2 = fmin(rmin2, rsq);
        } else if (rsq < far2 && molok && rmin * 1.5 > sqrt(rsq)) {
          hit = true;
          term = ai * pa[u];
        }
      }
      if (PASS == 2) {
        unsigned long long m = __ballot(hit);
        while (m) {
          const int b = __ffsll((long long)m) - 1;
          acc += __shfl(term, b, 64);
          m &= m - 1;
        }
      }
    }
  }
  if (PASS == 1) {
    rmin = wave_min(fmin(rmin, sqrt(rmin2)));
    if (lane == 0)
      atomicMin((unsigned long long *)slot_ptr(slots, SL_RMIN), (unsigned long long)__double_as_longlong(rmin));
  } else {
    if (lane == 0) rank_metric[i] = acc;
  }
}

static __global__ __launch_bounds__(POLAR_BLOCK) void k_rank_order(int n, const double *__restrict__ rk, int *__restrict__ order, int *__restrict__ pos) {
  const int lane = threadIdx.x & 63;
  const int i = blockIdx.x * POLAR_ROWS_PER_BLOCK + (threadIdx.x >> 6);
  if (i >= n) return;
  const double ri = rk[i];
  int before = 0;
  for (int j0 = 0; j0 < n; j0 += 64) {
    const int j = j0 + lane;
    const double rj = j < n ? rk[j] : 0.0;
    before += __popcll(__ballot(j < n && (rj > ri || (rj == ri && j < i))));
  }
  if (lane == 0) { pos[i] = before; order[before] = i; }
}

struct LJCoulParams {
  int ntypes, newton_pair, nlocal;
  int full_list;
  int ncoultablebits, ncoulmask, ncoulshiftbits;
  int ablate;
  int typed_list;
  int tab_lowmask;
  int i_special[2];
  double dr_special[2];
  double tabinnersq, cut_coulsq, g_ewald, qqrd2e;
  double special_lj[4], special_coul[4];
  const double *ljpack;
  const double *ctab;
};

static __global__ void k_pack_lj(int nall, const double *__restrict__ x, const double *__restrict__ q, double4 *__restrict__ xq,
                                 const double4 *__restrict__ snap, unsigned long long *__restrict__ dmax2_bits) {
  int i = blockIdx.x * blockDim.x + threadIdx.x;
  double d2 = 0.0;
  if (i < nall) {
    const double4 p = make_double4(x[3 * i], x[3 * i + 1], x[3 * i + 2], q[i]);
    xq[i] = p;
    if (snap) {
      const double4 o = snap[i];
      const double dx = p.x - o.x, dy = p.y - o.y, dz = p.z - o.z;
      d2 = dx * dx + dy * dy + dz * dz;
// ... 178 lines not shown
          const int itable = (rbits & P.ncoulmask) >> P.ncoulshiftbits;
          const double2 *bin = reinterpret_cast<const double2 *>(P.ctab + (size_t)itable * 8);
          double2 rdr, fdf;
          if (TAB == 2) {
            rdr.x = (double)__int_as_float(rbits & ~P.tab_lowmask);
            rdr.y = __hiloint2double((1173 - P.ncoulshiftbits - ((rbits >> 23) & 0xFF)) << 20, 0);
            if (itable == P.i_special[0]) rdr.y = P.dr_special[0];
            if (itable == P.i_special[1]) rdr.y = P.dr_special[1];
          } else rdr = bin[0];
          if (TAB == 0) {
            fdf = bin[1];
            if (EFLAG) tab_e = bin[2];
          } else {
            const double4 t4 = ctab_lds[itable];
            fdf = make_double2(t4.x, t4.y);
            if (EFLAG) tab_e = make_double2(t4.z, t4.w);
          }
          fraction = ((double)rsqf - rdr.x) * rdr.y;
          forcecoul = qiqj * (fdf.x + fraction * fdf.y);
          if (factor_coul < 1.0) {
            const double2 cdc = bin[3];
            prefactor = qiqj * (cdc.x + fraction * cdc.y);
            forcecoul -= (1.0 - factor_coul) * prefactor;
          }
        }
      }
      if (rsq < lj[1]) {
        r6inv = r2inv * r2inv * r2inv;
        forcelj = r6inv * (lj[2] * r6inv - lj[3]);
      }
      const double fpair = (forcecoul + factor_lj * forcelj) * r2inv;
      fx += delx * fpair; fy += dely * fpair; fz += delz * fpair;
      if (!P.full_list && (P.newton_pair || j < P.nlocal) && !(P.ablate & 32)) {
        atomicAdd(&f[3 * j], -delx * fpair);
        atomicAdd(&f[3 * j + 1], -dely * fpair);
        atomicAdd(&f[3 * j + 2], -delz * fpair);
      }
      double wgt = 1.0;
      if (P.full_list) wgt = 0.5;
      else if (!P.newton_pair) wgt = 0.5 * ((i < P.nlocal) + (j < P.nlocal));
      if (EFLAG) {
        if (rsq < P.cut_coulsq) {
          double ecoul;
          if (direct) ecoul = prefactor * erfc_;
          else ecoul = qiqj * (tab_e.x + fraction * tab_e.y);
          if (factor_coul < 1.0) ecoul -= (1.0 - factor_coul) * prefactor;
          ec += wgt * ecoul;
        }
        if (rsq < lj[1]) ev += wgt * factor_lj * (r6inv * (lj[4] * r6inv - lj[5]) - lj[6]);
      }
      if (VPAIR) {
        v0 += wgt * delx * delx * fpair; v1 += wgt * dely * dely * fpair; v2 += wgt * delz * delz * fpair;
        v3 += wgt * delx * dely * fpair; v4 += wgt * delx * delz * fpair; v5 += wgt * dely * delz * fpair;
      }
    }
  }
  fx = wave_sum(fx); fy = wave_sum(fy); fz = wave_sum(fz);
  if (lane == 0) {
    atomicAdd(&f[3 * i], fx); atomicAdd(&f[3 * i + 1], fy); atomicAdd(&f[3 * i + 2], fz);
  }
  if (EFLAG) {
    ev = wave_sum(ev); ec = wave_sum(ec);
    ev_sum += ev; ec_sum += ec;
    if (lane == 0 && eatom) eatom[i] += ev + ec;
  }
  if (VPAIR) {
    v0 = wave_sum(v0); v1 = wave_sum(v1); v2 = wave_sum(v2); v3 = wave_sum(v3); v4 = wave_sum(v4); v5 = wave_sum(v5);
    vsum[0] += v0; vsum[1] += v1; vsum[2] += v2; vsum[3] += v3; vsum[4] += v4; vsum[5] += v5;
    if (lane == 0 && vatom) {
      double *va = vatom + 6 * (size_t)i;
      va[0] += v0; va[1] += v1; va[2] += v2; va[3] += v3; va[4] += v4; va[5] += v5;
    }
  }
}
template <bool EFLAG, bool VPAIR>
__device__ __forceinline__ void ljcoul_tally(double *__restrict__ slots, int slot, int lane, int vglobal, double ev, double ec, const double (&v)[6]) {
  if (lane != 0) return;
  double *s = slots + (size_t)(slot & (POLAR_NSLOT - 1)) * POLAR_SLOT_STRIDE;
  if (EFLAG) { atomicAdd(s + SL_EVDWL, ev); atomicAdd(s + SL_ECOUL, ec); }
  if (VPAIR && vglobal) {
    atomicAdd(s + SL_V0, v[0]); atomicAdd(s + SL_V1, v[1]); atomicAdd(s + SL_V2, v[2]);
    atomicAdd(s + SL_V3, v[3]); atomicAdd(s + SL_V4, v[4]); atomicAdd(s + SL_V5, v[5]);
  }
}

template <bool EFLAG, bool VPAIR>
static __global__ __launch_bounds__(POLAR_BLOCK) void k_ljcoul(LJCoulParams P, int inum, const int *__restrict__ ilist,
                                                        const int *__restrict__ numneigh,
                                                        const long long *__restrict__ first,
                                                        const int *__restrict__ neigh,
                                                        const double4 *__restrict__ xq, const int *__restrict__ type,
                                                        double *__restrict__ f, double *__restrict__ slots,
                                                        double *__restrict__ eatom, double *__restrict__ vatom,
                                                        int vglobal) {
  extern __shared__ double lj_lds[];
  const int w = P.ntypes + 1;
  for (int t = threadIdx.x; t < w * w * 8; t += blockDim.x) lj_lds[t] = P.ljpack[t];
  __syncthreads();
  const int lane = threadIdx.x & 63;
  const int ii = blockIdx.x * POLAR_ROWS_PER_BLOCK + (threadIdx.x >> 6);
  if (ii >= inum) return;
  const int i = ilist ? ilist[ii] : ii;
  const int jnum = numneigh ? numneigh[i] : (int)(first[i + 1] - first[i]);
  if (jnum == 0) return;
  double ev = 0.0, ec = 0.0, v[6] = {0, 0, 0, 0, 0, 0};
  ljcoul_row<EFLAG, VPAIR, 0>(P, i, jnum, neigh + first[i], xq[i], xq, type, lj_lds, nullptr, lane, f, eatom, vatom, ev, ec, v);
  ljcoul_tally<EFLAG, VPAIR>(slots, blockIdx.x, lane, vglobal, ev, ec, v);
}

#define POLAR_LJ_PERS_THREADS 1024
template <bool EFLAG, bool VPAIR, int TAB>
static __global__ __launch_bounds__(POLAR_LJ_PERS_THREADS) void k_ljcoul_pers(LJCoulParams P, int inum, const int *__restrict__ ilist,
                                                        const int *__restrict__ numneigh,
                                                        const long long *__restrict__ first,
                                                        const int *__restrict__ neigh,
                                                        const double4 *__restrict__ xq, const int *__restrict__ type,
                                                        double *__restrict__ f, double *__restrict__ slots,
                                                        double *__restrict__ eatom, double *__restrict__ vatom,
                                                        int vglobal) {
  extern __shared__ double lj_lds[];
  const int w = P.ntypes + 1, nlj = (w * w * 8 + 3) & ~3;
  double4 *ctab_lds = reinterpret_cast<double4 *>(lj_lds + nlj);
  for (int t = threadIdx.x; t < w * w * 8; t += blockDim.x) lj_lds[t] = P.ljpack[t];
  const int ntable = 1 << P.ncoultablebits;
  for (int b = threadIdx.x; b < ntable; b += blockDim.x) {
    const double2 *bin = reinterpret_cast<const double2 *>(P.ctab + (size_t)b * 8);
    const double2 fdf = bin[1], ede = bin[2];
    ctab_lds[b] = make_double4(fdf.x, fdf.y, ede.x, ede.y);
  }
  __syncthreads();
  const int lane = threadIdx.x & 63, wv = threadIdx.x >> 6, nwv = blockDim.x >> 6;
  double ev = 0.0, ec = 0.0;
  for (int ii = blockIdx.x + gridDim.x * wv; ii < inum; ii += gridDim.x * nwv) {
    const int i = ilist ? ilist[ii] : ii;
    const int jnum = numneigh ? numneigh[i] : (int)(first[i + 1] - first[i]);
    if (jnum == 0) continue;
    double v[6] = {0, 0, 0, 0, 0, 0};
    ljcoul_row<EFLAG, VPAIR, TAB>(P, i, jnum, neigh + first[i], xq[i], xq, type, lj_lds, ctab_lds, lane, f, eatom, vatom, ev, ec, v);
    if (VPAIR) ljcoul_tally<false, true>(slots, ii, lane, vglobal, 0.0, 0.0, v);
  }
  const double none[6] = {0, 0, 0, 0, 0, 0};
  ljcoul_tally<EFLAG, false>(slots, blockIdx.x * nwv + wv, lane, 0, ev, ec, none);
}

template <bool ALLPAIRS, bool EW>
static __device__ __forceinline__ void static_field_body(const int *__restrict__ rows, int nrows, int nlocal,
                                                              const AtomRec *__restrict__ rec,
                                                              const int *__restrict__ mol, Box box,
                                                              RowList nl,
                                                              const int *__restrict__ nl_j, double cut_coulsq,
                                                              double e2s, double gamma, int use_previous,
                                                              double *__restrict__ ef, AtomRec *__restrict__ rec0,
                                                              AtomRec *__restrict__ rec1, const double4 *__restrict__ xq_s,
                                                              double g_ewald, const double *__restrict__ erec) {
  const int lane = threadIdx.x & 63;
  const int row = blockIdx.x * POLAR_ROWS_PER_BLOCK + (threadIdx.x >> 6);
  if (row >= nrows) return;
  const int i = rows ? rows[row] : row;
  const AtomRec ri = uniform_rec(rec[i]);
  const int mi = mol[i];
  const double f_shift = -1.0 / cut_coulsq;
  double ex = 0, ey = 0, ez = 0;
  long long beg = 0, end = nlocal;
  if (!ALLPAIRS) row_range(nl, i, beg, end);
  if (ALLPAIRS) {
    for (long long p = beg + lane; p < end; p += 64) {
      const int j = (int)p;
      if (j == i) continue;
      const AtomRec rj = rec[j];
      double dx, dy, dz;
      pair_del<ALLPAIRS>(box, ri.x, ri.y, ri.z, rj.x, rj.y, rj.z, dx, dy, dz);
      const double rsq = dx * dx + dy * dy + dz * dz;
      if (EW) {
        if (rsq <= cut_coulsq) {
          const double ef_temp = ewald_b1(rsq, g_ewald, (mi != mol[j]) || mi == 0) * rj.q;
          ex += ef_temp * dx; ey += ef_temp * dy; ez += ef_temp * dz;
        }
      } else if (rsq <= cut_coulsq && ((mi != mol[j]) || mi == 0)) {
        const double rinv = rsqrt(rsq);
        const double ef_temp = (rinv * rinv + f_shift) * rinv * rj.q;
        ex += ef_temp * dx; ey += ef_temp * dy; ez += ef_temp * dz;
      }
    }
  } else {
    __shared__ double2 s_stage[POLAR_ROWS_PER_BLOCK][64 * 5];
    double2 *stage = s_stage[threadIdx.x >> 6];
    for (long long base = beg; base < end; base += 64) {
      const long long p = base + lane;
      const bool valid = p < end;
      const int e = valid ? nl_j[p] : i;
      const int j = e & POLAR_NL_MASK;
      double xj, yj, zj, qj;
      if (xq_s) { const XQ t = fetch_xq(xq_s, j, stage, lane); xj = t.a.x; yj = t.a.y; zj = t.b.x; qj = t.b.y; }
      else { const RecQuad rj = fetch_records(rec, j, stage, lane); xj = rj.a.x; yj = rj.b.x; zj = rj.c.x; qj = rj.d.x; }
      double dx, dy, dz;
      pair_del<ALLPAIRS>(box, ri.x, ri.y, ri.z, xj, yj, zj, dx, dy, dz);
      const double rsq = dx * dx + dy * dy + dz * dz;
      if (EW) {
        if (valid && j != i && rsq <= cut_coulsq) {
          const double ef_temp = ewald_b1(rsq, g_ewald, !(e & POLAR_NL_SAMEMOL)) * qj;
          ex += ef_temp * dx; ey += ef_temp * dy; ez += ef_temp * dz;
        }
      } else if (valid && j != i && rsq <= cut_coulsq && !(e & POLAR_NL_SAMEMOL)) {
        const double rinv = rsqrt(rsq);
        const double ef_temp = (rinv * rinv + f_shift) * rinv * qj;
        ex += ef_temp * dx; ey += ef_temp * dy; ez += ef_temp * dz;
      }
    }
  }
  ex = wave_sum(ex); ey = wave_sum(ey); ez = wave_sum(ez);
  if (lane == 0) {
    ex *= e2s; ey *= e2s; ez *= e2s;
    if (EW) { ex += erec[3 * i]; ey += erec[3 * i + 1]; ez += erec[3 * i + 2]; }
    ef[3 * i] = ex; ef[3 * i + 1] = ey; ef[3 * i + 2] = ez;
    if (!use_previous) {
      const double a = ri.a;
      double mx = a * ex, my = a * ey, mz = a * ez;
      mx *= gamma; my *= gamma; mz *= gamma;
      rec0[i].mx = mx; rec0[i].my = my; rec0[i].mz = mz;
      rec1[i].mx = mx; rec1[i].my = my; rec1[i].mz = mz;
    }
  }
}

template <bool ALLPAIRS>
static __global__ __launch_bounds__(POLAR_BLOCK) void k_static_field(const int *__restrict__ rows, int nrows, int nlocal,
                                                              const AtomRec *__restrict__ rec,
                                                              const int *__restrict__ mol, Box box,
                                                              RowList nl,
                                                              const int *__restrict__ nl_j, double cut_coulsq,
                                                              double e2s, double gamma, int use_previous,
                                                              double *__restrict__ ef, AtomRec *__restrict__ rec0,
                                                              AtomRec *__restrict__ rec1, const double4 *__restrict__ xq_s) {
  static_field_body<ALLPAIRS, false>(rows, nrows, nlocal, rec, mol, box, nl, nl_j, cut_coulsq, e2s, gamma, use_previous, ef, rec0, rec1,
                                     xq_s, 0.0, nullptr);
}
template <bool ALLPAIRS>
static __global__ __launch_bounds__(POLAR_BLOCK) void k_ew_static_field(const int *__restrict__ rows, int nrows, int nlocal,
                                                                 const AtomRec *__restrict__ rec,
                                                                 const int *__restrict__ mol, Box box,
                                                                 RowList nl,
                                                                 const int *__restrict__ nl_j, double cut_coulsq,
                                                                 double e2s, double gamma, int use_previous,
                                                                 double *__restrict__ ef, AtomRec *__restrict__ rec0,
                                                                 AtomRec *__restrict__ rec1, const double4 *__restrict__ xq_s,
                                                                 double g_ewald, const double *__restrict__ erec) {
  static_field_body<ALLPAIRS, true>(rows, nrows, nlocal, rec, mol, box, nl, nl_j, cut_coulsq, e2s, gamma, use_previous, ef, rec0, rec1,
                                    xq_s, g_ewald, erec);
}

struct PairMath {
  const ExpCoef &K;
  double g_ewald;
  __device__ __forceinline__ double rsqrt(double x) const { return rsqrt_pos3(x); }
  __device__ __forceinline__ double exp_neg(double x) const { return exp_neg_fast<12>(x, K); }
  __device__ __forceinline__ void ewald_b12(double rsq, bool kept, double &b1, double &b2) const { polar::ewald_b12(rsq, g_ewald, kept, b1, b2); }
};

template <bool ALLPAIRS, int DAMP, bool EFLAG, bool VPAIR, bool EW>
static __device__ __forceinline__ void polar_force_body(const int *__restrict__ rows, int nrows, const int *__restrict__ perm,
                                                             int nlocal, const Scal *scal_in,
                                                             const AtomRec *__restrict__ recA,
                                                             const AtomRec *__restrict__ recB,
                                                             const int *__restrict__ mol, Box box,
                                                             RowList nl,
                                                             const int *__restrict__ nl_j, double cut_coulsq,
                                                             double ddcutsq, double pd, double e2s,
                                                             double *__restrict__ f, double *__restrict__ slots,
                                                             double *__restrict__ vatom, int vglobal, ExpCoef K,
                                                             double *__restrict__ dbg6, double g_ewald, int skip_inert POLAR_LIT_PARAM) {
  const int lane = threadIdx.x & 63;
  const int row = blockIdx.x * POLAR_ROWS_PER_BLOCK + (threadIdx.x >> 6);
  if (row >= nrows) return;
  const int i = rows ? rows[row] : row;
  const AtomRec *__restrict__ rec = __builtin_amdgcn_readfirstlane(scal_in->cur) ? recB : recA;
  const AtomRec ri = uniform_rec(rec[i]);
  if (skip_inert && site_is_inert(ri.q, ri.a)) return;
  const int mi = mol[i];
  const PairRow pri = make_pair_row(ri.mx, ri.my, ri.mz, ri.q, ri.a, e2s);
  const PairCut cut{cut_coulsq, ddcutsq, -1.0 / cut_coulsq, pd};
  const PairMath pm{K, g_ewald};
  double fx = 0, fy = 0, fz = 0, uef = 0, udd = 0;
  double v0 = 0, v1 = 0, v2 = 0, v3 = 0, v4 = 0, v5 = 0;
  const bool isdbg = dbg6 && (perm ? perm[i] : i) == 0;
  double ddx = 0, ddy = 0, ddz = 0;
  long long beg = 0, end = nlocal;
  if (!ALLPAIRS) row_range(nl, i, beg, end);
  Box pbox = box;
  if (!ALLPAIRS) {
#pragma unroll
    for (int k = 0; k < 3; k++) { pbox.inv[k] = box.periodic[k] ? box.inv[k] : 0.0; pbox.periodic[k] = 1; }
  }
  int e_n1 = i, e_n2 = i;
  if (!ALLPAIRS) {
    if (beg + lane < end) e_n1 = nl_j[beg + lane];
    if (beg + lane + 64 < end) e_n2 = nl_j[beg + lane + 64];
  }
  AtomRec r_n1 = rec[e_n1 & POLAR_NL_MASK];
  for (long long p = beg + lane; p < end; p += 64) {
    const int e = ALLPAIRS ? (int)p : e_n1;
    const int j = ALLPAIRS ? e : (e & POLAR_NL_MASK);
    const AtomRec rj = ALLPAIRS ? rec[j] : r_n1;
    if (!ALLPAIRS) {
      e_n1 = e_n2;
      r_n1 = *reinterpret_cast<const AtomRec *>(reinterpret_cast<const char *>(rec) + ((unsigned)(e_n1 & POLAR_NL_MASK) << 6));
      e_n2 = p + 128 < end ? nl_j[p + 128] : i;
    }
    if (j == i) continue;
    const bool molok = ALLPAIRS ? ((mi != mol[j]) || mi == 0) : !(e & POLAR_NL_SAMEMOL);
    double dx, dy, dz;
    pair_del<ALLPAIRS>(pbox, ri.x, ri.y, ri.z, rj.x, rj.y, rj.z, dx, dy, dz);
    double px, py, pz;
#ifdef POLAR_LAB
    if (literal) {
      double qx, qy, qz, ue, ud;
      polar_force_pair_literal<ALLPAIRS, DAMP, EFLAG, EW>(K, g_ewald, dx, dy, dz, ri, rj, molok, cut_coulsq, ddcutsq, pd, e2s, px, py, pz,
                                                          qx, qy, qz, ue, ud);
      fx += px; fy += py; fz += pz;
      ddx += qx; ddy += qy; ddz += qz;
      if (VPAIR) { px += qx; py += qy; pz += qz; }
      if (EFLAG) { uef += ue; udd += ud; }
    } else
#endif
    polar_force_pair<ALLPAIRS, DAMP, EFLAG, EW, VPAIR>(pm, dx, dy, dz, pri, rj.mx, rj.my, rj.mz, rj.q, rj.a, molok, cut, fx, fy, fz,
                                                       ddx, ddy, ddz, uef, udd, px, py, pz);
    if (VPAIR) {
      v0 += 0.5 * dx * px; v1 += 0.5 * dy * py; v2 += 0.5 * dz * pz;
      v3 += 0.5 * dx * py; v4 += 0.5 * dx * pz; v5 += 0.5 * dy * pz;
    }
  }
  fx += ddx; fy += ddy; fz += ddz;
  fx = wave_sum(fx); fy = wave_sum(fy); fz = wave_sum(fz);
  if (lane == 0) {
    const int o = perm ? perm[i] : i;
    atomicAdd(&f[3 * o], fx); atomicAdd(&f[3 * o + 1], fy); atomicAdd(&f[3 * o + 2], fz);
  }
  if (isdbg) {
    ddx = wave_sum(ddx); ddy = wave_sum(ddy); ddz = wave_sum(ddz);
    if (lane == 0) { dbg6[0] = fx; dbg6[1] = fy; dbg6[2] = fz; dbg6[3] = ddx; dbg6[4] = ddy; dbg6[5] = ddz; }
  }
  if (EFLAG) {
    uef = wave_sum(uef); udd = wave_sum(udd);
    if (lane == 0) {
      if (ri.a != 0.0) atomicAdd(slot_ptr(slots, SL_USELF), 0.5 * (ri.mx * ri.mx + ri.my * ri.my + ri.mz * ri.mz) / ri.a);
      atomicAdd(slot_ptr(slots, SL_UEF), 0.5 * uef);
      atomicAdd(slot_ptr(slots, SL_UDD), 0.5 * udd);
    }
  }
  if (VPAIR) {
    v0 = wave_sum(v0); v1 = wave_sum(v1); v2 = wave_sum(v2); v3 = wave_sum(v3); v4 = wave_sum(v4); v5 = wave_sum(v5);
    if (lane == 0) {
      if (vglobal) {
        atomicAdd(slot_ptr(slots, SL_V0), v0); atomicAdd(slot_ptr(slots, SL_V1), v1); atomicAdd(slot_ptr(slots, SL_V2), v2);
        atomicAdd(slot_ptr(slots, SL_V3), v3); atomicAdd(slot_ptr(slots, SL_V4), v4); atomicAdd(slot_ptr(slots, SL_V5), v5);
      }
      if (vatom) {
        double *va = vatom + 6 * (size_t)(perm ? perm[i] : i);
        va[0] += v0; va[1] += v1; va[2] += v2; va[3] += v3; va[4] += v4; va[5] += v5;
      }
    }
  }
}

template <bool ALLPAIRS, int DAMP, bool EFLAG, bool VPAIR>
static __global__ __launch_bounds__(POLAR_BLOCK) void k_polar_force(
    const int *__restrict__ rows, int nrows, const int *__restrict__ perm, int nlocal, const Scal *scal_in,
    const AtomRec *__restrict__ recA, const AtomRec *__restrict__ recB, const int *__restrict__ mol, Box box, RowList nl,
    const int *__restrict__ nl_j, double cut_coulsq, double ddcutsq, double pd, double e2s, double *__restrict__ f,
    double *__restrict__ slots, double *__restrict__ vatom, int vglobal, ExpCoef K, double *__restrict__ dbg6, int skip_inert POLAR_LIT_PARAM) {
  polar_force_body<ALLPAIRS, DAMP, EFLAG, VPAIR, false>(rows, nrows, perm, nlocal, scal_in, recA, recB, mol, box, nl, nl_j, cut_coulsq, ddcutsq, pd, e2s, f, slots, vatom, vglobal, K, dbg6, 0.0, skip_inert POLAR_LIT_PASS);
}
template <bool ALLPAIRS, int DAMP, bool EFLAG, bool VPAIR>
static __global__ __launch_bounds__(POLAR_BLOCK) void k_ew_polar_force(
    const int *__restrict__ rows, int nrows, const int *__restrict__ perm, int nlocal, const Scal *scal_in,
    const AtomRec *__restrict__ recA, const AtomRec *__restrict__ recB, const int *__restrict__ mol, Box box, RowList nl,
    const int *__restrict__ nl_j, double cut_coulsq, double ddcutsq, double pd, double e2s, double *__restrict__ f,
    double *__restrict__ slots, double *__restrict__ vatom, int vglobal, ExpCoef K, double *__restrict__ dbg6, double g_ewald, int skip_inert POLAR_LIT_PARAM) {
  polar_force_body<ALLPAIRS, DAMP, EFLAG, VPAIR, true>(rows, nrows, perm, nlocal, scal_in, recA, recB, mol, box, nl, nl_j, cut_coulsq, ddcutsq, pd, e2s, f, slots, vatom, vglobal, K, dbg6, g_ewald, skip_inert POLAR_LIT_PASS);
}

static __global__ void k_add_into(long long n, const double *__restrict__ src, double *__restrict__ dst) {
  long long i = blockIdx.x * (long long)blockDim.x + threadIdx.x;
  if (i < n) dst[i] += src[i];
}

static __global__ __launch_bounds__(POLAR_BLOCK) void k_virial_fdotr(int nall, const double *__restrict__ x,
                                                              const double *__restrict__ f, double *__restrict__ slots) {
  double v[6] = {0, 0, 0, 0, 0, 0};
  for (int i = blockIdx.x * blockDim.x + threadIdx.x; i < nall; i += gridDim.x * blockDim.x) {
    const double fx = f[3 * i], fy = f[3 * i + 1], fz = f[3 * i + 2];
    const double xx = x[3 * i], yy = x[3 * i + 1], zz = x[3 * i + 2];
    v[0] += fx * xx; v[1] += fy * yy; v[2] += fz * zz; v[3] += fy * xx; v[4] += fz * xx; v[5] += fz * yy;
  }
  const int lane = threadIdx.x & 63;
#pragma unroll
  for (int k = 0; k < 6; k++) {
    double s = wave_sum(v[k]);
    if (lane == 0 && s != 0.0) atomicAdd(slot_ptr(slots, SL_V0 + k), s);
  }
}

}

#undef POLAR_LIT_PARAM
#undef POLAR_LIT_PASS
```

### lammps-induced-dipole-polarization-pair-style_amd/csrc/polar_step.hip

```cpp
#include "polar_handle.hpp"

void launch_scan(long long n, const int *in, long long *out, DBuf<long long> &tot, hipStream_t s) {
  const int nb = (int)std::max<long long>(1, (n + POLAR_SCAN_ITEMS - 1) / POLAR_SCAN_ITEMS);
  tot.ensure((size_t)nb + 1);
  k_scan_block<<<nb, 1024, 0, s>>>(n, in, out, tot.p);
  if (nb > 1) {
    k_scan_totals<<<1, 1024, 0, s>>>(nb, tot.p, out + n);
    k_scan_add<<<nblk(n - POLAR_SCAN_ITEMS, 256), 256, 0, s>>>(n, out, tot.p);
  }
}

void build_cells(polar_handle *h) {
  const polar_settings &st = h->ph.st;
  const int n = h->nlocal;
  const double cutall = std::max(st.cut_coul, st.dd_cutoff);
  double width[3];
  box_widths(h->box, width);
  CellGrid &g = h->grid;
  if (!list_grid(width, h->box.periodic, cutall, g.nc))
    throw InputError("dd_cutoff mode needs box lengths >= 2*max(cut_coul,dd_cutoff); use exact mode (dd_cutoff 0)");
  g.trim = 1;
#ifdef POLAR_LAB
  if (const char *e = getenv("POLAR_NL_TRIM")) g.trim = atoi(e);
#endif
  if (h->box.triclinic) g.trim = 0;
  long long ncell = 1;
  for (int k = 0; k < 3; k++) {
    if (h->sweep_kernel == 4 && k == 0 && h->tile_wide) g.nc[k] = std::max(1, (int)std::floor(width[k] / cutall));
    if (h->sweep_kernel == 4 && h->box.periodic[k] && g.nc[k] >= 7 && (g.nc[k] & 1)) g.nc[k] -= 1;
    h->tile_sw[k] = std::max(1, std::min(2, (int)std::ceil(st.dd_cutoff / (width[k] / g.nc[k]) - 1e-9)));
    g.lo[k] = h->boxlo[k];
    g.inv[k] = g.nc[k] / h->box.prd[k];
    ncell *= g.nc[k];
  }
  h->ncell = ncell;
  if (h->sweep_kernel == 4) {
    struct Cls { int start, stride, count; };
    std::vector<Cls> cls[3];
    for (int k = 0; k < 3; k++) {
      const int nc = g.nc[k];
      const bool seam = h->box.periodic[k] && (nc & 1) && nc > 1;
      const int lim = seam ? nc - 1 : nc;
      if ((lim + 1) / 2 > 0) cls[k].push_back(Cls{0, 2, (lim + 1) / 2});
      if (lim / 2 > 0) cls[k].push_back(Cls{1, 2, lim / 2});
      if (seam) cls[k].push_back(Cls{nc - 1, 1, 1});
    }
    h->tile_launches.clear();
    for (const Cls &cz : cls[2]) for (const Cls &cy : cls[1]) for (const Cls &cx : cls[0]) {
      TileLaunch L;
      L.start[0] = cx.start; L.stride[0] = cx.stride; L.count[0] = cx.count;
      L.start[1] = cy.start; L.stride[1] = cy.stride; L.count[1] = cy.count;
      L.start[2] = cz.start; L.stride[2] = cz.stride; L.count[2] = cz.count;
      for (int k = 0; k < 3; k++) L.nc[k] = g.nc[k];
      h->tile_launches.push_back(L);
    }
    for (int k = 0; k < 3; k++) { h->tile_all.start[k] = 0; h->tile_all.stride[k] = 1; h->tile_all.count[k] = g.nc[k]; h->tile_all.nc[k] = g.nc[k]; }
  }
  hipStream_t s = h->stream;
  const bool split = h->nl_inert && h->cell_inert;
  if (!cell_bins_fit(ncell, split)) throw InputError("the list grid has more cells than a 32-bit bin index holds");
  const CellBins cb = cell_bins(ncell, split);
  const bool pol_first = h->pol_first || h->sweep_kernel == 4;
  h->cell_split = split;
  h->d_cell_id.ensure(n); h->d_cell_cnt.ensure(cb.cnt); h->d_cell_fill.ensure(cb.fill);
  h->d_cell_first.ensure(cb.first); h->d_perm.ensure(n + 1); h->d_inv.ensure(n + 1);
  zero_many(s, {{h->d_cell_cnt.p, (size_t)cb.cnt * sizeof(int)}, {h->d_cell_fill.p, (size_t)cb.fill * sizeof(int)}});
  k_cell_count<<<nblk(n, 256), 256, 0, s>>>(n, h->d_x.p, h->d_q.p, h->d_alpha.p, g, h->box, split ? ncell : 0, h->d_cell_id.p, h->d_cell_cnt.p);
  launch_scan(cb.nbins, h->d_cell_cnt.p, h->d_cell_first.p, h->d_scan_a, s);
  k_cell_fill<<<nblk(n, 256), 256, 0, s>>>(n, h->d_cell_id.p, h->d_cell_first.p, h->d_cell_fill.p,
                                           pol_first ? h->d_cell_fill.p + cb.fill_back : nullptr, h->d_alpha.p, h->d_perm.p, h->d_inv.p);
  k_cell_sort<<<nblk(cb.nbins, 4), 256, 0, s>>>(cb.nbins, h->d_cell_first.p, pol_first ? h->d_cell_fill.p : nullptr, h->d_perm.p, h->d_inv.p);
  h->sorted = true;
  if (sharded(h)) {
    h->d_ownrows.ensure(own_n(h) + 1);
    k_map_range<<<nblk(own_n(h), 256), 256, 0, s>>>(own_lo(h), own_n(h), h->d_inv.p, h->d_ownrows.p);
  }
}

void compute_slots(polar_handle *h) {
  const polar_settings &st = h->ph.st;
  const bool gs = st.polar_gs || st.polar_gs_ranked;
  const int n = h->nlocal;
  hipStream_t s = h->stream;
  h->d_slot.ensure(n + 1);
  HIPCHECK(hipMemsetAsync(h->d_slot.p, 0xFF, (size_t)(n + 1) * sizeof(int), s));
  if (gs && h->colors_valid) {
    const int tot = h->color_off.empty() ? 0 : h->color_off.back();
    if (tot > 0) k_slot_from_rows<<<nblk(tot, 256), 256, 0, s>>>(tot, h->d_rows.p, h->d_slot.p);
    h->slots_by_color = true;
    h->slots_epoch = h->color_epoch;
  } else {
    k_slot_from_rows<<<nblk(own_n(h), 256), 256, 0, s>>>(own_n(h), own_rows(h), h->d_slot.p);
    h->slots_by_color = false;
  }
}

void build_lists(polar_handle *h) {
  const polar_settings &st = h->ph.st;
  const int n = h->nlocal;
  const double cutall = std::max(st.cut_coul, st.dd_cutoff);
  hipStream_t s = h->stream;
  const CellGrid &g = h->grid;
  if (h->nl_pitch == 0 && getenv("POLAR_INIT_PITCH")) h->nl_pitch = h->dd_pitch = pitch_forced(atoi(getenv("POLAR_INIT_PITCH")));
  if (h->nl_pitch == 0) {
    const double vol = occupied_volume(n, h->hx.data(), g.lo, h->box.prd, cutall);
    h->dens = n / vol;
    double mean = n / vol * 4.18879020478639 * cutall * cutall * cutall;
    h->nl_pitch = h->dd_pitch = pitch_first(mean, 1.5);
  }
  if (h->sweep_kernel == 2) h->dd_pitch = ((h->dd_pitch + 255) / 256) * 256;
  if ((h->sweep_kernel == 2 || h->sweep_kernel == 3) && ((long long)n + 1) * (long long)sizeof(AtomRec) >= (1ll << 31))
    throw InputError("more than 2^25 atoms on one handle: the 32-bit record offsets of the sweep's index stream would wrap (shard the system)");
  h->d_nl_cnt.ensure(n + 1); h->d_dd_cnt.ensure(n + 1);
  h->d_nl_j.ensure((size_t)n * h->nl_pitch + 64);
  if (h->sweep_kernel < 3) h->d_dd_j.ensure((size_t)n * h->dd_pitch + 1024);
  else h->d_dd_j.ensure(64);
  const int mode = h->stream_mode = stream_mode(h->cache_r2, h->sweep_kernel, h->dd_pairs, own_n(h), h->dd_pitch);
  const bool r2c = mode == 1;
  if (mode == 1) h->d_dd_r2.ensure((size_t)n * h->dd_pitch + 64);
  else if (mode == 0) h->d_dd_s.ensure((size_t)n * h->dd_pitch + 64);
  double *r2p = r2c ? h->d_dd_r2.p : nullptr;
  double2 *sp = mode == 0 ? h->d_dd_s.p : nullptr;
  bool fuse = mode != 0 && mode != 4;
#ifdef POLAR_LAB
  if (getenv("POLAR_NO_FUSE_R2")) fuse = false;
#endif
  const double cutallsq = cutall * cutall, ddsq = mode == 4 ? -1.0 : st.dd_cutoff * st.dd_cutoff;
  const int nr = own_n(h);
  const int *rows = own_rows(h);
  zero_many(s, {{h->d_nl_cnt.p, (size_t)(n + 1) * sizeof(int)}, {h->d_dd_cnt.p, (size_t)(n + 1) * sizeof(int)},
                {h->d_overflow.p, 16 * sizeof(int)}, {h->d_ddtot.p, 64 * 16 * sizeof(unsigned long long)}});
  const bool lp = mode == 3;
  if (lp) h->d_dd_wrap.ensure(n + 1);
  const bool recheck = h->colors_valid && h->colors_recheck && h->sweep_kernel < 3 && (int)h->h_color.size() == n;
  if (h->colors_recheck && !recheck) { h->colors_valid = false; h->colors_recheck = false; }
  if (recheck) {
    h->d_color_s.ensure(n + 1);
    k_color_map<<<nblk(n, 256), 256, 0, s>>>(n, h->d_perm.p, h->d_color_orig.p, h->d_color_s.p);
  }
  if (((long long)n + 1) * (long long)sizeof(double4) >= (1ll << 32))
    throw InputError("more than 2^27 atoms on one handle: the 32-bit position offsets of the list build would wrap (shard the system)");
#define NLB3(TRI, RC, DENSE)                                                                                                  \
  k_nl_build<TRI, RC, DENSE><<<nblk(nr, POLAR_ROWS_PER_BLOCK), POLAR_BLOCK, 0, s>>>(                                          \
      rows, nr, h->d_pos4.p, h->box, g, h->d_cell_first.p, cutallsq, ddsq, h->nl_pitch, h->dd_pitch, h->d_nl_cnt.p,            \
      h->d_dd_cnt.p, h->d_nl_j.p, h->d_dd_j.p, fuse ? r2p : nullptr, fuse ? 1 : 0, lp ? (6 | (h->lp_quad_major << 8)) : 0,    \
      lp ? n : -1, lp ? h->d_dd_wrap.p : nullptr, recheck ? h->d_color_s.p : nullptr, h->color_keep * h->color_keep,           \
      h->d_overflow.p + 8, lp ? h->d_slot.p : nullptr, h->d_overflow.p, h->d_ddtot.p)
#ifdef POLAR_LAB
#define NLB(TRI, RC) do { if (h->nl_dense) NLB3(TRI, RC, true); else NLB3(TRI, RC, false); } while (0)
  h->nl_dense_used = h->nl_dense ? 1.0 : 0.0;
#else
#define NLB(TRI, RC) NLB3(TRI, RC, true)
#endif
  if (h->box.triclinic) { if (recheck) NLB(true, true); else NLB(true, false); }
  else                  { if (recheck) NLB(false, true); else NLB(false, false); }
#undef NLB
#undef NLB3
  const RowList ddl{h->d_dd_cnt.p, h->dd_pitch};
  if (fuse || mode == 4) {
  }
#ifdef POLAR_LAB
  else if (st.damping_type == POLAR_DAMP_EXPONENTIAL)
    k_dd_scalars<0><<<nblk(nr, POLAR_ROWS_PER_BLOCK), POLAR_BLOCK, 0, s>>>(rows, nr, h->d_rec0.p, h->box, ddl, h->d_dd_j.p, st.polar_damp, sp, r2p);
  else
    k_dd_scalars<1><<<nblk(nr, POLAR_ROWS_PER_BLOCK), POLAR_BLOCK, 0, s>>>(rows, nr, h->d_rec0.p, h->box, ddl, h->d_dd_j.p, st.polar_damp, sp, r2p);
#endif
  HIPCHECK(hipMemcpyAsync(h->h_flags.p, h->d_overflow.p, sizeof(int), hipMemcpyDeviceToHost, s));
  HIPCHECK(hipMemcpyAsync(h->h_ddtot.p, h->d_ddtot.p, 64 * 16 * sizeof(unsigned long long), hipMemcpyDeviceToHost, s));
}
template <bool AP>
static void launch_rank(polar_handle *h, int pass) {
  const int n = h->nlocal, ntot = h->nlocal + h->nghost;
  dim3 grid(nblk(n, POLAR_ROWS_PER_BLOCK)), block(POLAR_BLOCK);
  if (pass == 2) k_fold_scal<<<1, POLAR_NSLOT, 0, h->stream>>>(h->d_scal.p, h->d_slots.p, 1);
  const int nchunk = (AP && pass == 1) ? std::max(1, std::min(16, 8192 / std::max(n, 1))) : 1;
  if (pass == 1)
    k_rank<AP, 1><<<nblk((long long)n * nchunk, POLAR_ROWS_PER_BLOCK), block, 0, h->stream>>>(n, ntot, h->d_x.p, h->d_alpha.p, h->d_mol.p, h->box, RowList{h->d_nl_cnt.p, h->nl_pitch},
                                                 h->d_nl_j.p, h->d_rec0.p, h->d_mol_s.p, h->d_scal.p, h->d_slots.p, h->d_rank.p, nchunk);
  else
    k_rank<AP, 2><<<grid, block, 0, h->stream>>>(n, ntot, h->d_x.p, h->d_alpha.p, h->d_mol.p, h->box, RowList{h->d_nl_cnt.p, h->nl_pitch},
                                                 h->d_nl_j.p, h->d_rec0.p, h->d_mol_s.p, h->d_scal.p, h->d_slots.p, h->d_rank.p, 1);
}

void launch_rank_pass(polar_handle *h, bool allpairs, int pass) {
  if (allpairs) launch_rank<true>(h, pass); else launch_rank<false>(h, pass);
}

template <bool AP, int DAMP, int EP>
void launch_field(polar_handle *h, int nrows, const int *rows) {
  const polar_settings &st = h->ph.st;
  if (nrows <= 0) return;
  const int fb = h->field_block;
  const size_t lds = AP ? 0 : (size_t)(fb / 64) * 64 * 5 * sizeof(double2);
  k_field<AP, DAMP, EP><<<nblk(nrows, fb / 64), fb, lds, h->stream>>>(
      nrows, rows, h->nlocal, h->d_rec0.p, h->d_rec1.p, h->box, RowList{h->d_dd_cnt.p, h->dd_pitch}, h->d_dd_j.p, h->d_dd_s.p,
      st.dd_cutoff * st.dd_cutoff, st.polar_damp, h->d_ef_s.p, h->d_F.p, h->d_scal.p, h->d_slots.p
#ifdef POLAR_LAB
      , h->ablate
#endif
      );
}
template <int EP>
void launch_field_dyn(polar_handle *h, bool ap, int nrows, const int *rows) {
  const bool expd = h->ph.st.damping_type == POLAR_DAMP_EXPONENTIAL;
  if (ap) { if (expd) launch_field<true, 0, EP>(h, nrows, rows); else launch_field<true, 1, EP>(h, nrows, rows); }
#ifdef POLAR_LAB
  else    { if (expd) launch_field<false, 0, EP>(h, nrows, rows); else launch_field<false, 1, EP>(h, nrows, rows); }
#else
  else throw std::logic_error("k_field's list branch exists in the lab build only");
#endif
}

#ifdef POLAR_LAB
#include "lab/launch_quad.inc"
#else
template <int EP> inline void launch_field_quad(polar_handle *, int, const int *) { throw std::logic_error("lab build only"); }
#endif

void prepare_lp(polar_handle *h) {
  const polar_settings &st = h->ph.st;
  const bool gs = st.polar_gs || st.polar_gs_ranked;
  const int tot = gs ? (h->color_off.empty() ? 0 : h->color_off.back()) : own_n(h);
  h->d_lpdesc.ensure((size_t)tot + 1);
  h->lp_npart = 0;
  if (deterministic(h)) {
    h->d_lp_pend.ensure(4 * (size_t)tot + 4);
    const int nlaunch = gs ? (int)h->color_off.size() - 1 : 1;
    h->lp_npart = tot / 256 + nlaunch + 1;
    h->d_lp_part.ensure((size_t)h->lp_npart + 1);
    HIPCHECK(hipMemsetAsync(h->d_lp_part.p, 0, (size_t)h->lp_npart * sizeof(double), h->stream));
  }
  if (tot > 0)
    k_lp_desc<<<nblk(tot, 256), 256, 0, h->stream>>>(tot, gs ? h->d_rows.p : own_rows(h), RowList{h->d_dd_cnt.p, h->dd_pitch},
                                                     h->d_dd_wrap.p, h->d_lpdesc.p);
}
template <int EP>
void launch_field_lp(polar_handle *h, int nrows, const int2 *desc) {
  const long long row0 = desc - h->d_lpdesc.p;
  if (nrows <= 0) return;
  const polar_settings &st = h->ph.st;
  const int qb = h->quad_block;
  const bool det = deterministic(h);
  const int nt = det ? 2 : h->lp_tiles;
  size_t lds = (size_t)(qb / 64) * nt * POLAR_LP_TILE;
  if (h->lp_wg_per_cu > 0) lds = std::max(lds, std::min((size_t)64 * 1024, (size_t)160 * 1024 / h->lp_wg_per_cu));
  if (lds > (size_t)64 * 1024) throw InputError("k_field_lp: workgroup size x tiles needs more than 64 KB of LDS (POLAR_QUAD_BLOCK <= 512 with two tiles)");
  const double omega = EP == EP_INPLACE ? st.polar_sor : 1.0;
#ifdef POLAR_LAB
#define POLAR_LAB_ARG , h->ablate
#else
#define POLAR_LAB_ARG
#endif
#define FL(D, NT, DT) k_field_lp<EP, D, NT, DT><<<nblk_xcd(nrows, qb / 64), qb, lds, h->stream>>>(                   \
      nrows, row0, desc, h->d_rec0.p, h->d_rec1.p, h->box, h->dd_pitch, h->d_dd_j.p,                               \
      st.polar_damp, make_expcoef(), h->d_ef_s.p, h->d_scal.p, h->d_slots.p, omega, h->d_lp_pend.p POLAR_LAB_ARG)
  const bool expd = st.damping_type == POLAR_DAMP_EXPONENTIAL;
#ifdef POLAR_LAB
#include "lab/launch_lpa.inc"
#endif
#ifdef POLAR_LAB
#include "lab/launch_lpr.inc"
#endif
  if (det) {
    if (expd) FL(0, 2, true); else FL(1, 2, true);
    int launch_no = 0;
    if (EP == EP_INPLACE) while (launch_no + 1 < (int)h->color_off.size() && h->color_off[launch_no] < row0) launch_no++;
    k_lp_commit<<<nblk(nrows, 256), 256, 0, h->stream>>>(nrows, row0, desc, h->d_lp_pend.p, h->d_rec0.p, h->d_rec1.p, EP == EP_JACOBI ? 1 : 0,
                                                      h->d_scal.p, h->d_lp_part.p + row0 / 256 + launch_no);
  } else {
    if (expd) FL(0, 2, false); else FL(1, 2, false);
  }
#undef FL
#undef POLAR_LAB_ARG
}

#ifdef POLAR_LAB
#include "lab/launch_cluster_tile.inc"
#else
template <int EP> inline void launch_field_cl(polar_handle *, int, int) { throw std::logic_error("lab build only"); }
inline size_t tile_lds_bytes(int) { return 0; }
inline int tile_lds_cap() { return 0; }
inline void build_tiles(polar_handle *) { throw std::logic_error("lab build only"); }
template <int EP> inline void launch_field_tile(polar_handle *, const TileLaunch &) { throw std::logic_error("lab build only"); }
#endif

#ifdef POLAR_LAB
#include "lab/build_units_paired_rows.inc"
#endif

void sweep_once(polar_handle *h, bool ap) {
  const polar_settings &st = h->ph.st;
  const bool gs = st.polar_gs || st.polar_gs_ranked;
  if (!ap && h->sweep_kernel == 4) {
    if (!gs) { launch_field_tile<EP_JACOBI>(h, h->tile_all); return; }
    const int ncol = (int)h->tile_launches.size();
    const int c0 = h->part_n > 1 ? ncol * h->part_k / h->part_n : 0, c1 = h->part_n > 1 ? ncol * (h->part_k + 1) / h->part_n : ncol;
    for (int c = c0; c < c1; c++) launch_field_tile<EP_INPLACE>(h, h->tile_launches[c]);
    return;
  }
  if (!ap && h->sweep_kernel == 3) {
    const int ncol = (int)h->color_off.size() - 1;
    for (int c = 0; c < ncol; c++) {
      if (gs) launch_field_cl<EP_INPLACE>(h, h->color_off[c + 1] - h->color_off[c], h->color_off[c]);
      else launch_field_cl<EP_JACOBI>(h, h->color_off[c + 1] - h->color_off[c], h->color_off[c]);
    }
    return;
  }
#ifdef POLAR_LAB
  if (!ap && h->sweep_kernel == 2 && h->lp_pairs && !deterministic(h) && h->part_n <= 1) {
    if (!gs) { launch_field_lp2<EP_JACOBI>(h, 0); return; }
    for (int c = 0; c + 1 < (int)h->unit_off.size(); c++) launch_field_lp2<EP_INPLACE>(h, c);
    return;
  }
#endif
  if (!ap && h->sweep_kernel == 2) {
    if (!gs) { launch_field_lp<EP_JACOBI>(h, own_n(h), h->d_lpdesc.p); return; }
    const int ncol = (int)h->color_off.size() - 1;
    const int c0 = h->part_n > 1 ? ncol * h->part_k / h->part_n : 0, c1 = h->part_n > 1 ? ncol * (h->part_k + 1) / h->part_n : ncol;
    for (int c = c0; c < c1; c++)
      launch_field_lp<EP_INPLACE>(h, h->color_off[c + 1] - h->color_off[c], h->d_lpdesc.p + h->color_off[c]);
    return;
  }
  if (!ap && h->sweep_kernel == 0) {
    if (!gs) { launch_field_quad<EP_JACOBI>(h, own_n(h), own_rows(h)); return; }
    const int ncol = (int)h->color_off.size() - 1;
    for (int c = 0; c < ncol; c++)
      launch_field_quad<EP_INPLACE>(h, h->color_off[c + 1] - h->color_off[c], h->d_rows.p + h->color_off[c]);
    return;
  }
  if (!gs) {
    launch_field_dyn<EP_JACOBI>(h, ap, own_n(h), own_rows(h));
    return;
  }
  const int ncol = (int)h->color_off.size() - 1;
  for (int c = 0; c < ncol; c++) {
    const int cnt = h->color_off[c + 1] - h->color_off[c];
    if (cnt <= 0) continue;
    launch_field_dyn<EP_INPLACE>(h, false, cnt, h->d_rows.p + h->color_off[c]);
  }
}

void sweep_phase(polar_handle *h, int c, int part) {
  const int ncol = (int)h->color_off.size() - 1;
  if (c < 0 || c >= ncol) throw std::logic_error("sweep_phase: no such colour");
  const int a = h->color_off[c], b = h->color_off[c + 1];
  const int m = (h->color_nsub == 2 && !deterministic(h)) ? h->color_sub[2 * c + 1] : b;
  const int lo = part == 2 ? m : a, hi = part == 1 ? m : b;
  launch_field_lp<EP_INPLACE>(h, hi - lo, h->d_lpdesc.p + lo);
}
template <bool AP, int DAMP>
void launch_force(polar_handle *h, int eflag, int vglobal, double *vatom, double *fdst) {
  const bool vpair = vglobal || vatom;
  const polar_settings &st = h->ph.st;
  dim3 grid(nblk(own_n(h), POLAR_ROWS_PER_BLOCK)), block(POLAR_BLOCK);
  const double ccs = st.cut_coul * st.cut_coul, dds = st.dd_cutoff * st.dd_cutoff, e2s = std::sqrt(h->P.qqrd2e);
  double *dbg6 = nullptr;
  if (st.debug) {
    h->d_dbgf.ensure(8);
    HIPCHECK(hipMemsetAsync(h->d_dbgf.p, 0, 8 * sizeof(double), h->stream));
    dbg6 = h->d_dbgf.p;
  }
  const bool ew = ewald_on(h);
  const double g = h->P.g_ewald;
#ifdef POLAR_LAB
#define POLAR_LIT_ARG , h->force_literal
#else
#define POLAR_LIT_ARG
#endif
#define LF(E, V)                                                                                                    \
  if (ew) k_ew_polar_force<AP, DAMP, E, V><<<grid, block, 0, h->stream>>>(own_rows(h), own_n(h), h->sorted ? h->d_perm.p : nullptr, h->nlocal, h->d_scal.p, h->d_rec0.p, h->d_rec1.p,  \
                                                               h->d_mol_s.p, h->box, RowList{h->d_nl_cnt.p, h->nl_pitch}, h->d_nl_j.p,  \
                                                               ccs, dds, st.polar_damp, e2s, fdst, h->d_slots.p, vatom, vglobal, make_expcoef(),  \
                                                               dbg6, g, h->nl_inert POLAR_LIT_ARG);             \
  else k_polar_force<AP, DAMP, E, V><<<grid, block, 0, h->stream>>>(own_rows(h), own_n(h), h->sorted ? h->d_perm.p : nullptr, h->nlocal, h->d_scal.p, h->d_rec0.p, h->d_rec1.p,  \
                                                               h->d_mol_s.p, h->box, RowList{h->d_nl_cnt.p, h->nl_pitch}, h->d_nl_j.p,  \
                                                               ccs, dds, st.polar_damp, e2s, fdst, h->d_slots.p, vatom, vglobal, make_expcoef(),  \
                                                               dbg6, h->nl_inert POLAR_LIT_ARG)
  h->force_ran = true; h->force_listed = !AP; h->force_nrows = own_n(h);
  if (eflag) { if (vpair) { LF(true, true); } else { LF(true, false); } }
  else       { if (vpair) { LF(false, true); } else { LF(false, false); } }
#undef LF
#undef POLAR_LIT_ARG
}

static_assert(sizeof(PlanD4) == sizeof(double4) && sizeof(PlanI4) == sizeof(int4), "polar_plan.hpp's vectors go to the device as bytes");

void ewald_upload_kvectors(polar_handle *h) {
  const Box &b = h->box;
  const double g = h->P.g_ewald, acc = h->ph.st.polar_ewald;
  std::vector<double> key = {b.prd[0], b.prd[1], b.prd[2], b.xy, b.xz, b.yz, g, acc};
  if (key == h->ew_key) return;
  const EwaldPlan p = ewald_kvectors(b, g, acc);
  const auto &kv = p.kv; const auto &hkl = p.hkl; const auto &rows = p.rows;
  h->ew_nk = p.nk; h->ew_nrow = p.nrow; h->ew_nm = p.nm;
  std::copy(p.cell, p.cell + 6, h->ew_cell);
  h->d_ew_kv.ensure(kv.size() + 1); h->d_ew_hkl.ensure(hkl.size() + 1); h->d_ew_rows.ensure(rows.size());
  h->d_ew_s.ensure(kv.size() + 1); h->d_ew_m.ensure(kv.size() + 1);
  if (!kv.empty()) {
    HIPCHECK(hipMemcpyAsync(h->d_ew_kv.p, kv.data(), kv.size() * sizeof(double4), hipMemcpyHostToDevice, h->stream));
    HIPCHECK(hipMemcpyAsync(h->d_ew_hkl.p, hkl.data(), hkl.size() * sizeof(int4), hipMemcpyHostToDevice, h->stream));
  }
  HIPCHECK(hipMemcpyAsync(h->d_ew_rows.p, rows.data(), rows.size() * sizeof(int4), hipMemcpyHostToDevice, h->stream));
  HIPCHECK(hipStreamSynchronize(h->stream));
  h->ew_key = key;
}

void ewald_check(polar_handle *h, int vflag) {
  const polar_settings &st = h->ph.st;
  if (sharded(h)) throw Unsupported("polar_ewald needs one handle over all atoms: on a row-sharded handle the structure factors would need an all-reduce across the ranks");
  if (st.rccl_halo) throw Unsupported("polar_ewald is not offered with rccl_halo yes: the structure factors would need an all-reduce across the ranks");
  if (!(h->box.periodic[0] && h->box.periodic[1] && h->box.periodic[2])) throw Unsupported("polar_ewald needs a box periodic in x, y and z");
  if (vflag & 4) throw Unsupported("polar_ewald offers no per-atom virial (vflag & 4): the reciprocal-space virial has no pairwise definition");
  if (!(h->P.g_ewald > 0.0)) throw InputError("polar_ewald needs g_ewald > 0 (polar_pair_init / polar_set_coul)");
  ewald_upload_kvectors(h);
  if ((size_t)ewald_tile(h->ew_nm) * ewald_lds_per_atom(h->ew_nm) > 64 * 1024)
    throw Unsupported("polar_ewald: the k-vector range per box axis is too large for the structure-factor kernel (raise the accuracy value or g_ewald)");
}

bool ewald_short_box(const polar_handle *h) {
  double width[3];
  box_widths(h->box, width);
  return ewald_short_box(width, h->ph.st.cut_coul);
}

EwCell ew_cell(const polar_handle *h) {
  const double *c = h->ew_cell;
  return EwCell{c[0], c[1], c[2], c[3], c[4], c[5]};
}

void ewald_sfac(polar_handle *h, bool mu, double2 *out) {
  const int n = h->nlocal, nk = h->ew_nk, nm = h->ew_nm;
  if (nk == 0) return;
  const int tile = ewald_tile(nm);
  const size_t lds = (size_t)tile * ewald_lds_per_atom(nm);
  const SfacChunks ck = ewald_sfac_chunks(n, nk, tile);
  const int kb = ck.kb, nchunk = ck.nchunk, chunk = ck.chunk;
  h->d_ew_part.ensure((size_t)nchunk * nk);
  dim3 grid(kb, nchunk);
  if (mu) k_ew_sfac<true><<<grid, 256, lds, h->stream>>>(nk, h->d_ew_hkl.p, h->d_ew_kv.p, n, chunk, tile, nm, ew_cell(h), h->d_scal.p, h->d_rec0.p, h->d_rec1.p, h->d_ew_part.p);
  else    k_ew_sfac<false><<<grid, 256, lds, h->stream>>>(nk, h->d_ew_hkl.p, h->d_ew_kv.p, n, chunk, tile, nm, ew_cell(h), nullptr, h->d_rec0.p, h->d_rec1.p, h->d_ew_part.p);
  k_ew_fold<<<kb, 256, 0, h->stream>>>(nk, nchunk, h->d_ew_part.p, out);
}

void ewald_field(polar_handle *h) {
  const int n = h->nlocal;
  HIPCHECK(hipEventRecord(h->ev_ks[0], h->stream));
  h->d_ew_erec.ensure(3 * (size_t)n + 3);
  ewald_sfac(h, false, h->d_ew_s.p);
  if (n > 0) {
    if (h->ew_nk > 0)
      k_ew_field<<<nblk(n, 256), 256, 0, h->stream>>>(n, h->ew_nrow, h->d_ew_rows.p, h->d_ew_kv.p, h->d_ew_s.p, ew_cell(h), std::sqrt(h->P.qqrd2e), h->d_rec0.p, h->d_ew_erec.p);
    else HIPCHECK(hipMemsetAsync(h->d_ew_erec.p, 0, 3 * (size_t)n * sizeof(double), h->stream));
  }
  HIPCHECK(hipEventRecord(h->ev_ks[1], h->stream));
}

void ewald_forces(polar_handle *h) {
  const int n = h->nlocal, nk = h->ew_nk;
  hipStream_t s = h->stream;
  HIPCHECK(hipEventRecord(h->ev_ks[2], s));
  ewald_sfac(h, true, h->d_ew_m.p);
  const int nba = nblk(std::max(n, 1), 256), nbk = nk > 0 ? nblk(nk, 256) : 0;
  h->d_ew_vpart.ensure(8 * (size_t)(nba + nbk)); h->d_ew_out.ensure(8);
  const double e2s = std::sqrt(h->P.qqrd2e), g = h->P.g_ewald;
  k_ew_force<<<nba, 256, 0, s>>>(n, nk > 0 ? h->ew_nrow : 0, h->d_ew_rows.p, h->d_ew_kv.p, h->d_ew_s.p, h->d_ew_m.p, ew_cell(h), e2s, h->d_scal.p,
                                 h->d_rec0.p, h->d_rec1.p, h->sorted ? h->d_perm.p : nullptr, h->d_ef_s.p, h->d_ew_erec.p, h->d_f.p, h->d_ew_vpart.p);
  if (nbk) k_ew_kvirial<<<nbk, 256, 0, s>>>(nk, h->d_ew_kv.p, h->d_ew_s.p, h->d_ew_m.p, e2s, 1.0 / (4.0 * g * g), h->d_ew_vpart.p + 8 * (size_t)nba);
  k_ew_finish<<<1, 256, 0, s>>>(nba + nbk, h->d_ew_vpart.p, h->d_ew_out.p);
  HIPCHECK(hipEventRecord(h->ev_ks[3], s));
}

void read_scal(polar_handle *h) {
  HIPCHECK(hipGetLastError());
  HIPCHECK(hipMemcpyAsync(h->h_scal.p, h->d_scal.p, sizeof(Scal), hipMemcpyDeviceToHost, h->stream));
  HIPCHECK(hipStreamSynchronize(h->stream));
}
#ifdef POLAR_LAB
#include "lab/build_cluster_lists.inc"
#else
void build_cluster_lists(polar_handle *) { throw std::logic_error("lab build only"); }
#endif
void debug_trace(polar_handle *h, int sw) {
  if (!h->ph.st.debug) return;
  h->d_trace.ensure((size_t)h->ph.st.iterations_max + 8);
  if (sw > h->ph.st.iterations_max + 1) return;
  const MuView mv = mu_view(h);
  k_debug_upolar<<<1, 1024, 0, h->stream>>>(h->nlocal, h->d_scal.p, mv.a, mv.b, mv.stride, h->d_ef_s.p, h->d_trace.p, sw, 0);
  h->ntrace = sw + 1;
}

bool accel_begin(polar_handle *h, bool ap) {
  const polar_settings &st = h->ph.st;
  const bool gs = st.polar_gs || st.polar_gs_ranked;
  if (st.polar_accel <= 0) return false;
  if (ap || !gs || h->sweep_kernel != 2) throw InputError("polar_accel needs the Gauss-Seidel sweep of list mode (dd_cutoff > 0 with polar_gs or polar_gs_ranked)");
  if (deterministic(h)) throw InputError("polar_accel and `deterministic yes` exclude each other");
  const int tot = h->color_off.empty() ? 0 : h->color_off.back();
  const long long pitch = ((long long)tot + 255) / 256 * 256;
  const int M = POLAR_ACCEL_MAXM;
  h->acc_pitch = pitch; h->acc_rows = tot;
  const bool fresh = h->d_acc_dF.cap < (size_t)M * 3 * pitch + 1;
  h->d_acc_x.ensure(3 * pitch + 1); h->d_acc_f.ensure(3 * pitch + 1); h->d_acc_g.ensure(3 * pitch + 1);
  h->d_acc_dF.ensure((size_t)M * 3 * pitch + 1); h->d_acc_dG.ensure((size_t)M * 3 * pitch + 1);
  h->d_acc_part.ensure((size_t)2 * M * nblk(tot, 256) + 2 * M); h->d_acc_state.ensure(1);
  if (fresh) {
    HIPCHECK(hipMemsetAsync(h->d_acc_dF.p, 0, h->d_acc_dF.cap * sizeof(double), h->stream));
    HIPCHECK(hipMemsetAsync(h->d_acc_dG.p, 0, h->d_acc_dG.cap * sizeof(double), h->stream));
  }
  k_accel_init<<<nblk(tot, 256), 256, 0, h->stream>>>(tot, pitch, h->d_lpdesc.p, h->d_rec0.p, h->d_acc_x.p, h->d_acc_state.p);
  return true;
}
static void launch_accel_diff(polar_handle *h, int tot, int nb, int ring) {
  k_accel_diff<POLAR_ACCEL_MAXM><<<nb, 256, 0, h->stream>>>(tot, h->acc_pitch, h->d_lpdesc.p, h->d_rec0.p, h->d_scal.p, h->d_acc_state.p, h->d_acc_x.p,
                                                           h->d_acc_f.p, h->d_acc_g.p, h->d_acc_dF.p, h->d_acc_dG.p, h->d_acc_part.p, ring);
}
static void launch_accel_mix(polar_handle *h, int tot, int nb);
void accel_export(polar_handle *h, double *dev_local_dots) {
  const int tot = h->acc_rows, nb = nblk(tot, 256), ring = std::min(h->ph.st.polar_accel, POLAR_ACCEL_MAXM);
// ... 180 lines not shown
    hipStream_t ms = s;
    h->lj_forked = h->overlap_lj && h->inum > 0;
    if (h->lj_forked) {
      HIPCHECK(hipEventRecord(h->ev_fork, ms));
      HIPCHECK(hipStreamWaitEvent(h->lj_stream, h->ev_fork, 0));
    }
    hipStream_t s = h->lj_forked ? h->lj_stream : ms;
    if (h->list_up_pending) {
      HIPCHECK(hipStreamWaitEvent(s, h->ev_list_up, 0));
    }
    HIPCHECK(hipEventRecord(h->ev_lj0, s));
    LJCoulParams P = h->P;
    P.newton_pair = h->newton_pair; P.nlocal = n; P.cut_coulsq = st.cut_coul * st.cut_coul; P.full_list = h->full_list; P.ablate = 0;
    h->d_xq.ensure(nall + 1);
    const size_t ljlds = (size_t)(h->ntypes + 1) * (h->ntypes + 1) * 8 * sizeof(double);
    if (ljlds > 64 * 1024) throw InputError("too many atom types for the LDS-resident LJ table (max 31)");
    dim3 block(POLAR_BLOCK);
    bool symmetrise = !h->full_list;
#ifdef POLAR_LAB
    if (getenv("POLAR_LJ_ATOMICS")) symmetrise = false;
#endif
    const bool lj_pairwise_virial = h->full_list && vmode == 2;
    if ((eatom || vatom) && !symmetrise && !h->full_list) throw InputError("per-atom tallies need the row-complete pair list");
    const bool sym_build = symmetrise && !h->sym_valid && h->inum > 0;
    const bool skin_kept = symmetrise && !sym_build && h->sym_valid && h->skin_valid && h->skin_nall == nall;
    if (skin_kept && h->lj_skin) {
      HIPCHECK(hipMemsetAsync(h->d_lj_drift.p, 0, sizeof(unsigned long long), s));
      k_pack_lj<<<nblk(nall, 256), 256, 0, s>>>(nall, h->d_x.p, h->d_q.p, h->d_xq.p, h->d_xq_snap.p, h->d_lj_drift.p);
    } else k_pack_lj<<<nblk(nall, 256), 256, 0, s>>>(nall, h->d_x.p, h->d_q.p, h->d_xq.p, nullptr, nullptr);
    if (sym_build) {
      dim3 g0(nblk(h->inum, POLAR_ROWS_PER_BLOCK));
      const int nclass = h->lj_skin ? SKIN_CLASSES : 1;
      const size_t nk = (size_t)nall * nclass;
      h->d_sym_cnt.ensure(nk + 4); h->d_sym_fill.ensure(nk + 4); h->d_sym_cfirst.ensure(nk + 2); h->d_sym_first.ensure(nall + 2);
      h->d_sym_j.ensure(2 * (size_t)h->nneigh + 64);
      if (h->lj_skin) {
        h->d_sym_cend.ensure(nk + 1); h->d_lj_walk.ensure(nall + 1); h->d_sym_cls.ensure((size_t)h->nneigh + 64);
        h->d_xq_snap.ensure(nall + 1); h->d_lj_drift.ensure(2);
      }
      HIPCHECK(hipMemsetAsync(h->d_sym_cnt.p, 0, (nk + 4) * sizeof(int), s));
      HIPCHECK(hipMemsetAsync(h->d_sym_fill.p, 0, (nk + 4) * sizeof(int), s));
      h->sym_typed = h->lj_typed && nall < (1 << 24) && h->ntypes < 64;
      const int *ty = h->sym_typed ? h->d_type.p : nullptr;
      if (h->lj_skin) {
        k_sym_count<SKIN_CLASSES><<<g0, block, 0, s>>>(h->inum, h->d_ilist.p, h->d_numneigh.p, h->d_first.p, h->d_neigh.p, h->d_xq.p, h->r_cmax,
                                                     h->d_sym_cnt.p, h->d_sym_cls.p, h->d_sym_fill.p);
        launch_scan((long long)nk, h->d_sym_cnt.p, h->d_sym_cfirst.p, h->d_scan_b, s);
        k_sym_ends<SKIN_CLASSES><<<nblk(nall + 1, 256), 256, 0, s>>>(nall, h->d_sym_cfirst.p, h->d_sym_first.p, h->d_sym_cend.p);
        k_sym_fill<SKIN_CLASSES><<<g0, block, 0, s>>>(h->inum, h->d_ilist.p, h->d_numneigh.p, h->d_first.p, h->d_neigh.p, h->d_sym_cfirst.p,
                                                    h->d_sym_fill.p, h->d_sym_j.p, ty, h->d_sym_cls.p);
        HIPCHECK(hipMemcpyAsync(h->d_xq_snap.p, h->d_xq.p, (size_t)nall * sizeof(double4), hipMemcpyDeviceToDevice, s));
        HIPCHECK(hipMemsetAsync(h->d_lj_drift.p, 0, sizeof(unsigned long long), s));
      } else {
        k_sym_count<1><<<g0, block, 0, s>>>(h->inum, h->d_ilist.p, h->d_numneigh.p, h->d_first.p, h->d_neigh.p, nullptr, 0.0,
                                          h->d_sym_cnt.p, nullptr, h->d_sym_fill.p);
        launch_scan((long long)nk, h->d_sym_cnt.p, h->d_sym_cfirst.p, h->d_scan_b, s);
        k_sym_ends<1><<<nblk(nall + 1, 256), 256, 0, s>>>(nall, h->d_sym_cfirst.p, h->d_sym_first.p, nullptr);
        k_sym_fill<1><<<g0, block, 0, s>>>(h->inum, h->d_ilist.p, h->d_numneigh.p, h->d_first.p, h->d_neigh.p, h->d_sym_cfirst.p,
                                         h->d_sym_fill.p, h->d_sym_j.p, ty, nullptr);
      }
      h->sym_valid = true; h->skin_valid = h->lj_skin != 0; h->skin_nall = nall;
    }
    const int nrows_lj = symmetrise ? (h->newton_pair ? nall : n) : h->inum;
    dim3 grid(nblk(nrows_lj, POLAR_ROWS_PER_BLOCK));
    if (symmetrise) P.full_list = 1;
    P.typed_list = symmetrise ? (h->sym_typed ? 1 : 0) : (h->device_list && h->dev_typed ? 1 : 0);
    const bool walk = (sym_build || skin_kept) && h->lj_skin && h->skin_valid && h->inum > 0;
    if (walk) k_lj_walk<<<nblk(nall, 256), 256, 0, s>>>(nall, h->d_sym_cend.p, h->d_lj_drift.p, h->r_cmax, h->d_lj_walk.p);
    h->lj_sym_last = symmetrise; h->lj_walk_last = walk; h->lj_rows_last = nrows_lj; h->lj_ran = h->inum > 0;
    const int *il = symmetrise ? nullptr : h->d_ilist.p;
    const int *nn = symmetrise ? (walk ? h->d_lj_walk.p : nullptr) : h->d_numneigh.p;
    const long long *fi = symmetrise ? h->d_sym_first.p : h->d_first.p;
    const int *nj = symmetrise ? h->d_sym_j.p : h->d_neigh.p;
    if (h->inum > 0) {
      const bool vrow = vmode == 1 || vatom || lj_pairwise_virial;
      const size_t ljlds_al = ((ljlds / sizeof(double) + 3) & ~(size_t)3) * sizeof(double);
      const size_t plds = ljlds_al + ((size_t)32 << P.ncoultablebits);
      const bool pers = h->lj_pers && P.ncoultablebits > 0 && plds <= (size_t)160 * 1024 && h->ncu > 0 && (nrows_lj >= 16 * h->ncu || h->lj_pers >= 2);
      if (pers) {
#define LJP(E, V, T) do {                                                                                                              \
          static size_t raised[64] = {0};    \
          size_t &rs = raised[h->device & 63];                                                                                          \
          if (rs < plds) { HIPCHECK(hipFuncSetAttribute((const void *)k_ljcoul_pers<E, V, T>, hipFuncAttributeMaxDynamicSharedMemorySize, (int)plds)); rs = plds; } \
          k_ljcoul_pers<E, V, T><<<h->ncu, h->lj_pers_threads, plds, s>>>(P, nrows_lj, il, nn, fi, nj, h->d_xq.p, h->d_type.p, h->d_f.p, h->d_slots.p, eatom, vatom, vmode == 1 || lj_pairwise_virial); \
        } while (0)
#define LJPT(E, V) do { if (h->lj_tab_arith) LJP(E, V, 2); else LJP(E, V, 1); } while (0)
        if (eflag) { if (vrow) LJPT(true, true); else LJPT(true, false); }
        else       { if (vrow) LJPT(false, true); else LJPT(false, false); }
#undef LJPT
#undef LJP
      } else {
#define LJ(E, V) k_ljcoul<E, V><<<grid, block, ljlds, s>>>(P, nrows_lj, il, nn, fi, nj, h->d_xq.p, h->d_type.p, h->d_f.p, h->d_slots.p, eatom, vatom, vmode == 1 || lj_pairwise_virial)
        if (eflag) { if (vrow) LJ(true, true); else LJ(true, false); }
        else       { if (vrow) LJ(false, true); else LJ(false, false); }
#undef LJ
      }
    }
    HIPCHECK(hipEventRecord(h->ev_lj1, s));
    if (h->lj_forked) HIPCHECK(hipEventRecord(h->ev_join, s));
  };
  bool lj_late = false;
#ifdef POLAR_LAB
  lj_late = getenv("POLAR_LJ_LATE") != nullptr;
#endif
  if (!lj_late) launch_lj();
  const double *mu0 = nullptr;
  if (st.use_previous) {
    if (h->attempt > 0) {
      if (h->mu0_saved) { HIPCHECK(hipMemcpyAsync(h->d_mu.p, h->d_mu0.p, 3 * (size_t)n * sizeof(double), hipMemcpyDeviceToDevice, s)); mu0 = h->d_mu.p; }
    } else {
      if (mu_host && !(h->mu_resident && h->mu_host_in_sync)) {
        HIPCHECK(hipMemcpyAsync(h->d_mu.p, mu_host, 3 * (size_t)n * sizeof(double), hipMemcpyHostToDevice, s));
        mu0 = h->d_mu.p;
      } else if (h->mu_resident) mu0 = h->d_mu.p;
      h->mu0_saved = mu0 != nullptr;
      if (mu0) { h->d_mu0.ensure(3 * (size_t)n + 3); HIPCHECK(hipMemcpyAsync(h->d_mu0.p, h->d_mu.p, 3 * (size_t)n * sizeof(double), hipMemcpyDeviceToDevice, s)); }
    }
  }
  h->sorted = false;
  h->dense_gs = false;
  const bool gs_mode = (st.polar_gs || st.polar_gs_ranked) && !st.zodid;
  bool ranked_done = false;
  if (ap && gs_mode && dense_gs_fits(n) && !getenv("POLAR_NO_DENSE_GS")) {
    h->dense_gs = true;
    if (st.polar_gs_ranked) {
      launch_rank<true>(h, 1); launch_rank<true>(h, 2);
      ranked_done = true;
      h->d_perm.ensure(n + 1); h->d_inv.ensure(n + 1);
      k_rank_order<<<nblk(n, POLAR_ROWS_PER_BLOCK), POLAR_BLOCK, 0, s>>>(n, h->d_rank.p, h->d_perm.p, h->d_inv.p);
      h->sorted = true;
    }
  }
  if (!ap) { build_cells(h); h->d_pos4.ensure(n + 1); if (h->static_xq) h->d_xq_s.ensure(n + 2); }
  k_pack<<<nblk(n + 1, 256), 256, 0, s>>>(n, h->sorted ? h->d_perm.p : nullptr, h->d_x.p, h->d_q.p, h->d_alpha.p, h->d_mol.p, mu0,
                                      h->d_rec0.p, h->d_rec1.p, h->d_mol_s.p, ap ? nullptr : h->d_pos4.p, (!ap && h->static_xq) ? h->d_xq_s.p : nullptr,
                                      (!ap && h->sweep_kernel == 4) ? 1 : 0, h->box, h->boxlo[0], h->boxlo[1], h->boxlo[2], h->nl_inert ? 0 : 1);
  if (!ap) {
    if (h->colors_valid && h->sweep_kernel < 3) map_color_rows(h);
    if (h->sweep_kernel == 2) compute_slots(h);
    build_lists(h);
    if (h->colors_valid && h->sweep_kernel == 3) build_cluster_lists(h);
    if (h->sweep_kernel == 4) build_tiles(h);
  }
  HIPCHECK(hipEventRecord(h->ev[1], s));

  if (st.polar_gs_ranked && (ap || (!h->colors_valid && h->sweep_kernel != 4)) && !ranked_done) {
    if (ap) { launch_rank<true>(h, 1); launch_rank<true>(h, 2); }
    else    { launch_rank<false>(h, 1); launch_rank<false>(h, 2); }
  }
  HIPCHECK(hipEventRecord(h->ev[2], s));

  HIPCHECK(hipEventRecord(h->ev[3], s));

  {
    dim3 grid(nblk(own_n(h), POLAR_ROWS_PER_BLOCK)), block(POLAR_BLOCK);
    const double ccs = st.cut_coul * st.cut_coul, e2s = std::sqrt(h->P.qqrd2e);
    if (ewald_on(h)) {
      ewald_field(h);
      const double g = h->P.g_ewald;
      if (ap) k_ew_static_field<true><<<grid, block, 0, s>>>(nullptr, n, n, h->d_rec0.p, h->d_mol_s.p, h->box, RowList{nullptr, 0}, nullptr, ccs, e2s, st.polar_gamma, st.use_previous, h->d_ef_s.p, h->d_rec0.p, h->d_rec1.p, nullptr, g, h->d_ew_erec.p);
      else    k_ew_static_field<false><<<grid, block, 0, s>>>(own_rows(h), own_n(h), n, h->d_rec0.p, h->d_mol_s.p, h->box, RowList{h->d_nl_cnt.p, h->nl_pitch}, h->d_nl_j.p, ccs, e2s, st.polar_gamma, st.use_previous, h->d_ef_s.p, h->d_rec0.p, h->d_rec1.p, h->static_xq ? h->d_xq_s.p : nullptr, g, h->d_ew_erec.p);
    } else if (ap) k_static_field<true><<<grid, block, 0, s>>>(nullptr, n, n, h->d_rec0.p, h->d_mol_s.p, h->box, RowList{nullptr, 0}, nullptr, ccs, e2s, st.polar_gamma, st.use_previous, h->d_ef_s.p, h->d_rec0.p, h->d_rec1.p, nullptr);
    else    k_static_field<false><<<grid, block, 0, s>>>(own_rows(h), own_n(h), n, h->d_rec0.p, h->d_mol_s.p, h->box, RowList{h->d_nl_cnt.p, h->nl_pitch}, h->d_nl_j.p, ccs, e2s, st.polar_gamma, st.use_previous, h->d_ef_s.p, h->d_rec0.p, h->d_rec1.p, h->static_xq ? h->d_xq_s.p : nullptr);
  }
#ifdef POLAR_LAB
  if (!ap && h->sweep_kernel == 4 && !st.zodid)
    k_srec_pack<<<nblk(n, 256), 256, 0, s>>>(n, h->d_rec0.p, h->d_srec0.p, h->d_srec1.p);
#endif
  HIPCHECK(hipEventRecord(h->ev[4], s));
  if (lj_late) launch_lj();
}

int phase_finish(polar_handle *h, polar_result *out) {
  const polar_settings &st = h->ph.st;
  const int n = h->nlocal, nall = h->nlocal + h->nghost;
  const bool ap = !(st.dd_cutoff > 0.0);
  const bool expd = st.damping_type == POLAR_DAMP_EXPONENTIAL;
  const int eflag = h->step_eflag, vmode = h->step_vflag % 4;
  hipStream_t s = h->stream;
#ifdef POLAR_LAB
  if (!ap && h->sweep_kernel == 4 && !st.zodid)
    k_srec_unpack<<<nblk(n, 256), 256, 0, s>>>(n, h->d_scal.p, h->d_srec0.p, h->d_srec1.p, h->d_rec0.p, h->d_rec1.p);
#endif
  k_fallback<<<nblk(n, 256), 256, 0, s>>>(n, h->d_scal.p, h->d_rec0.p, h->d_rec1.p, h->d_ef_s.p);
  HIPCHECK(hipEventRecord(h->ev[5], s));
  k_unpack<<<nblk(n, 256), 256, 0, s>>>(n, h->sorted ? h->d_perm.p : nullptr, h->d_scal.p, h->d_rec0.p, h->d_rec1.p, h->d_ef_s.p, h->d_mu.p, h->d_ef.p);
  if (h->early_mu && n > 0) {
    HIPCHECK(hipEventRecord(h->ev_mu_ready, s));
    HIPCHECK(hipStreamWaitEvent(h->dl_stream, h->ev_mu_ready, 0));
    HIPCHECK(hipMemcpyAsync(h->early_mu, h->d_mu.p, 3 * (size_t)n * sizeof(double), hipMemcpyDeviceToHost, h->dl_stream));
    if (h->early_ef) HIPCHECK(hipMemcpyAsync(h->early_ef, h->d_ef.p, 3 * (size_t)n * sizeof(double), hipMemcpyDeviceToHost, h->dl_stream));
    HIPCHECK(hipEventRecord(h->ev_dl1, h->dl_stream));
  }
  double *vatom = (h->step_vflag / 4) ? h->d_vatom.p : nullptr;
  auto join_lj = [&]() { if (h->lj_forked) { HIPCHECK(hipStreamWaitEvent(s, h->ev_join, 0)); h->lj_forked = false; } };
  if (vatom) join_lj();
  const bool split_f = h->full_list && vmode == 2;
  double *fdst = h->d_f.p;
  if (split_f) {
    h->d_fpol.ensure(3 * (size_t)n + 3);
    HIPCHECK(hipMemsetAsync(h->d_fpol.p, 0, 3 * (size_t)n * sizeof(double), s));
    fdst = h->d_fpol.p;
  }
  if (ap) { if (expd) launch_force<true, 0>(h, eflag, vmode == 1, vatom, fdst); else launch_force<true, 1>(h, eflag, vmode == 1, vatom, fdst); }
  else    { if (expd) launch_force<false, 0>(h, eflag, vmode == 1, vatom, fdst); else launch_force<false, 1>(h, eflag, vmode == 1, vatom, fdst); }
  join_lj();
  if (split_f) {
    k_virial_fdotr<<<std::min(1024, nblk(n, 256)), 256, 0, s>>>(n, h->d_x.p, h->d_fpol.p, h->d_slots.p);
    k_add_into<<<nblk(3 * (long long)n, 256), 256, 0, s>>>(3 * (long long)n, h->d_fpol.p, h->d_f.p);
  } else if (vmode == 2) k_virial_fdotr<<<std::min(1024, nblk(nall, 256)), 256, 0, s>>>(nall, h->d_x.p, h->d_f.p, h->d_slots.p);
  if (ewald_on(h)) ewald_forces(h);
  k_fold_scal<<<1, POLAR_NSLOT, 0, s>>>(h->d_scal.p, h->d_slots.p, 0);
  HIPCHECK(hipEventRecord(h->ev[6], s));
  if (h->early_mu && h->user_mu && n > 0) {
    HIPCHECK(hipEventSynchronize(h->ev_dl1));
    const double *sm = h->early_mu, *se = h->early_ef;
    double *um = h->user_mu, *ue = h->user_ef;
    host_chunks(3 * (size_t)n, [&](size_t a, size_t b) {
      memcpy(um + a, sm + a, (b - a) * sizeof(double));
      if (ue && se) memcpy(ue + a, se + a, (b - a) * sizeof(double));
    });
  }
  read_scal(h);
  h->mu_resident = true;
  h->mu_host_in_sync = false;

  const Scal &sc = *h->h_scal.p;
  out->eng_vdwl = sc.eng_vdwl; out->eng_coul = sc.eng_coul;
  out->u_self = sc.u_self; out->u_ef = sc.u_ef; out->u_dd = sc.u_dd;
  out->eng_pol = sc.u_self + sc.u_ef + sc.u_dd;
  for (int k = 0; k < 6; k++) out->virial[k] = sc.virial[k];
  if (ewald_on(h)) {
    double ew[7];
    HIPCHECK(hipMemcpyAsync(ew, h->d_ew_out.p, sizeof(ew), hipMemcpyDeviceToHost, h->stream));
    HIPCHECK(hipStreamSynchronize(h->stream));
    if (eflag) { out->u_ef = ew[0]; out->eng_pol = sc.u_self + ew[0] + sc.u_dd; }
    if (vmode) for (int k = 0; k < 6; k++) out->virial[k] += ew[1 + k];
    float a = 0.f, b = 0.f;
    HIPCHECK(hipEventElapsedTime(&a, h->ev_ks[0], h->ev_ks[1]));
    HIPCHECK(hipEventElapsedTime(&b, h->ev_ks[2], h->ev_ks[3]));
    out->ms_kspace = (double)a + (double)b;
    h->ew_field_ms = (double)a;
    out->nkvec = h->ew_nk;
  }
  long long rb = (long long)sc.rmin_bits;
  memcpy(&out->rmin, &rb, sizeof(double));
  out->rms_dmu = std::sqrt(std::max(0.0, sc.last_change));
  h->ntrace = std::min(h->ntrace, sc.sweeps);
  out->iterations = sc.iterations; out->sweeps = sc.sweeps; out->status = sc.status ? POLAR_WARN_NOT_CONVERGED : POLAR_OK;
  h->last_sweeps = (!st.fixed_iteration && !st.zodid && !sc.status && sc.done) ? sc.sweeps : 0;
  if (!ap) {
    unsigned long long tot = 0;
    for (int k = 0; k < 64; k++) tot += h->h_ddtot.p[16 * k];
    h->dd_pairs = (long long)tot;
  }
  out->dd_pairs = ap ? (long long)n * (n - 1) : h->dd_pairs;
  out->ms_color_host = h->ms_color_host;
  h->ms_color_host = 0.0;
  float ms;
  auto el = [&](int a, int b) { HIPCHECK(hipEventElapsedTime(&ms, h->ev[a], h->ev[b])); return (double)ms; };
  out->ms_list = el(0, 1); out->ms_rank = el(1, 2); out->ms_static = el(3, 4);
  HIPCHECK(hipEventElapsedTime(&ms, h->ev_lj0, h->ev_lj1));
  out->ms_ljcoul = ms;
  out->ms_solve = el(4, 5); out->ms_force = el(5, 6); out->ms_total = el(0, 6);
  if (sc.status) h->warn = "Number of iterations exceeding max_iterations, setting dipoles to alpha*E";
  return out->status;
}

void clear_flags(polar_handle *h) { for (int k = 0; k < 16; k++) h->h_flags.p[k] = 0; }
void tile_fallback(polar_handle *h) {
  h->sweep_kernel = 2;
  h->colors_valid = false; h->slots_by_color = false;
  h->nl_pitch = h->dd_pitch = 0;
  h->warn = "tile sweep unavailable for this system (cell neighbourhood beyond the LDS, or a cell beyond the builder's limits): row sweep in use";
}
bool grow_pitches(polar_handle *h) {
  bool again = false;
  if (h->h_flags.p[0] != 0) {
    h->nl_pitch = h->dd_pitch = std::max(pitch_grown(h->h_flags.p[0]), h->nl_pitch + 64);
    again = true;
  }
  if (h->h_flags.p[4] != 0) { h->cl_pitch = (((long long)(1.25 * h->h_flags.p[4]) + 255) / 256) * 256; again = true; }
  if (h->sweep_kernel == 4) {
    if (h->h_flags.p[7] != 0) { tile_fallback(h); return true; }
    if (h->h_flags.p[5] != 0) {
      const int need = (int)(((long long)(1.15 * h->h_flags.p[5]) + 16 + 63) / 64 * 64);
      if (need > tile_lds_cap()) { tile_fallback(h); return true; }
      h->un_pitch = std::max(h->un_pitch, need); h->un_lds = h->un_pitch;
      again = true;
    }
    if (h->h_flags.p[6] != 0) { h->pitch16 = ((long long)(1.25 * h->h_flags.p[6]) + 511) / 512 * 512; again = true; }
    if (!again && h->h_flags.p[9] > 0) {
      h->tile_max_u = h->h_flags.p[9];
      h->un_lds = std::min(h->un_pitch, (int)((long long)(1.06 * (h->tile_max_u + 1)) + 8 + 7) / 8 * 8);
      if (getenv("POLAR_DEBUG") && !h->tile_reported) {
        h->tile_reported = true;
        fprintf(stderr, "[polar] tile sweep: %lld cells (%d x %d x %d), %d launches per sweep, largest union %d records, union pitch %d, "
                "LDS request %zu bytes (%d records), row pitch %lld entries\n", h->ncell, h->grid.nc[0], h->grid.nc[1], h->grid.nc[2],
                (int)h->tile_launches.size(), h->tile_max_u, h->un_pitch, tile_lds_bytes(std::min(h->un_pitch, h->un_lds)), h->un_lds, h->pitch16);
      }
    }
  }
  return again;
}

int do_compute(polar_handle *h, int eflag, int vflag, const double *mu_host, polar_result *out) {
  memset(out, 0, sizeof(*out));
  const bool ap = !(h->ph.st.dd_cutoff > 0.0);
  int rc = 0;
  bool done = false;
  struct Attempt { polar_handle *h; ~Attempt() { h->attempt = 0; } } guard{h};
  for (int attempt = 0; attempt < 5; attempt++) {
    clear_flags(h);
    h->attempt = attempt;
    try {
      phase_begin(h, eflag, vflag, mu_host);
    } catch (const TileUnavailable &) {
// ... 157 lines not shown
```

Baseline: 17.10 million.

## Precompute list-build row constants on host and prefetch neighbor rows speculatively

Neighbor-list build kernel now receives host-precomputed cell edges, periodic inverses, window counts and reach squared instead of recomputing divisions and sqrt per wave. Static-field and polar-force kernels speculatively load the first two 64-entry chunks of each row's neighbor list alongside the count, before dependent record loads, and pipeline later chunk loads two iterations ahead. Final reductions of the three force/field components (plus energy) are merged into a single four-way DPP/shuffle reduction with lanes 0-3 writing results. This adds unconditional loads of row slots beyond the count, relying on the padded list allocation that now validates the pitch.

```diff
diff --git a/lammps-induced-dipole-polarization-pair-style_amd/csrc/lab/api_env_knobs.inc b/lammps-induced-dipole-polarization-pair-style_amd/csrc/lab/api_env_knobs.inc
--- a/lammps-induced-dipole-polarization-pair-style_amd/csrc/lab/api_env_knobs.inc
+++ b/lammps-induced-dipole-polarization-pair-style_amd/csrc/lab/api_env_knobs.inc
@@ -19,3 +19,5 @@
   if (const char *e = getenv("POLAR_FIELD_BLOCK")) { int v = atoi(e); if (v >= 64 && v <= 1024 && v % 64 == 0) h->field_block = v; }
   if (const char *e = getenv("POLAR_FORCE_LITERAL")) h->force_literal = atoi(e) != 0;
   if (const char *e = getenv("POLAR_NL_DENSE")) h->nl_dense = atoi(e) != 0;
+  if (const char *e = getenv("POLAR_ROW_CONSTS")) h->row_consts = atoi(e) != 0;
+  if (const char *e = getenv("POLAR_ROW_SPEC")) h->row_spec = atoi(e) != 0;
diff --git a/lammps-induced-dipole-polarization-pair-style_amd/csrc/polar_api.hip b/lammps-induced-dipole-polarization-pair-style_amd/csrc/polar_api.hip
--- a/lammps-induced-dipole-polarization-pair-style_amd/csrc/polar_api.hip
+++ b/lammps-induced-dipole-polarization-pair-style_amd/csrc/polar_api.hip
@@ -276,6 +276,8 @@
   if (dim) *dim = 0;
   if (strcmp(name, "cut_coul") == 0) return &h->ph.st.cut_coul;
   if (strcmp(name, "nl_dense") == 0) return &h->nl_dense_used;
+  if (strcmp(name, "row_consts") == 0) return &h->row_consts_used;
+  if (strcmp(name, "row_spec") == 0) return &h->row_spec_used;
   if (strcmp(name, "lj_walked") == 0 || strcmp(name, "lj_entries") == 0) {
     polar_handle *m = const_cast<polar_handle *>(h);
     if (guarded(m, [&]() { lj_counters(m); return POLAR_OK; }) != POLAR_OK) return nullptr;
diff --git a/lammps-induced-dipole-polarization-pair-style_amd/csrc/polar_common.hpp b/lammps-induced-dipole-polarization-pair-style_amd/csrc/polar_common.hpp
--- a/lammps-induced-dipole-polarization-pair-style_amd/csrc/polar_common.hpp
+++ b/lammps-induced-dipole-polarization-pair-style_amd/csrc/polar_common.hpp
@@ -93,6 +93,17 @@
   v += dpp_get<0x142, 0xA>(v);
   v += dpp_get<0x143, 0xC>(v);
   return lane63(v);
+}
+__device__ __forceinline__ double wave_sum4(double a, double b, double c, double d, int lane) {
+  const bool odd = lane & 1, hi = lane & 2;
+  double v = (odd ? b : a) + dpp_full<0xB1>(odd ? a : b);
+  double w = (odd ? d : c) + dpp_full<0xB1>(odd ? c : d);
+  v = (hi ? w : v) + dpp_full<0x4E>(hi ? v : w);
+  v += dpp_full<0x12C>(v);
+  v += dpp_full<0x128>(v);
+  v += __shfl_xor(v, 16, 64);
+  v += __shfl_xor(v, 32, 64);
+  return v;
 }
 __device__ __forceinline__ double wave_min(double v) {
 #pragma unroll
diff --git a/lammps-induced-dipole-polarization-pair-style_amd/csrc/polar_handle.hpp b/lammps-induced-dipole-polarization-pair-style_amd/csrc/polar_handle.hpp
--- a/lammps-induced-dipole-polarization-pair-style_amd/csrc/polar_handle.hpp
+++ b/lammps-induced-dipole-polarization-pair-style_amd/csrc/polar_handle.hpp
@@ -199,7 +199,11 @@
   int static_xq = 1;
   int pol_first = 1;
   double nl_dense_used = 1.0;
+  double row_consts_used = 1.0;
+  double row_spec_used = 1.0;
 #ifdef POLAR_LAB
+  int row_consts = 1;
+  int row_spec = 1;
   int nl_dense = 1;
   int force_literal = 0;
 #endif
diff --git a/lammps-induced-dipole-polarization-pair-style_amd/csrc/polar_lists.hpp b/lammps-induced-dipole-polarization-pair-style_amd/csrc/polar_lists.hpp
--- a/lammps-induced-dipole-polarization-pair-style_amd/csrc/polar_lists.hpp
+++ b/lammps-induced-dipole-polarization-pair-style_amd/csrc/polar_lists.hpp
@@ -485,9 +485,9 @@
   __device__ __forceinline__ int end(int sr) const { return __builtin_amdgcn_readlane(endv, sr); }
   __device__ __forceinline__ bool two(int sr) const { return (m1 >> sr) & 1u; }
 };
-template <bool TRI, bool RECHECK, bool DENSE = true>
+template <bool TRI, bool RECHECK, bool DENSE = true, bool HOSTC = true>
 static __global__ __launch_bounds__(POLAR_BLOCK) void k_nl_build(const int *__restrict__ rows, int nrows,
-                                                          const double4 *__restrict__ pos4, Box box, CellGrid g,
+                                                          const double4 *__restrict__ pos4, Box box, CellGrid g, NlRowConsts kc,
                                                           const long long *__restrict__ cell_first, double cutallsq,
                                                           double ddcutsq, long long nl_pitch, long long dd_pitch,
                                                           int *__restrict__ nl_cnt, int *__restrict__ dd_cnt,
@@ -521,7 +521,8 @@
       int ck = (int)t;
       ck = ck >= g.nc[k] ? g.nc[k] - 1 : ck;
       cc[k] = __builtin_amdgcn_readfirstlane(ck);
-      uu[k] = wave_uniform(t - ck); edge[k] = wave_uniform(box.prd[k] / g.nc[k]);
+      uu[k] = wave_uniform(t - ck);
+      edge[k] = HOSTC ? kc.edge[k] : wave_uniform(box.prd[k] / g.nc[k]);
     }
   }
   const int c0 = cc[0], c1 = cc[1], c2 = cc[2];
@@ -534,16 +535,20 @@
   const unsigned long long dd_im = (ipol && slot_i >= 0) ? ~0ull : 0ull;
   Box pbox = box;
 #pragma unroll
-  for (int k = 0; k < 3; k++) { pbox.inv[k] = box.periodic[k] ? box.inv[k] : 0.0; pbox.periodic[k] = 1; }
+  for (int k = 0; k < 3; k++) { pbox.inv[k] = HOSTC ? kc.pinv[k] : (box.periodic[k] ? box.inv[k] : 0.0); pbox.periodic[k] = 1; }
   int ncount = 0, dcount = 0;
   unsigned long long wrap_m = 0ull;
   const int same_i = imol != 0 ? POLAR_NL_SAMEMOL : 0;
   const unsigned long long below = (lane == 0) ? 0ull : (~0ull >> (64 - lane));
-  const int n0 = g.nc[0], n1 = g.nc[1], n2 = g.nc[2];
-  const int zlo = n2 >= 5 ? c2 - 2 : 0, zcnt = n2 >= 5 ? 5 : n2;
-  const int ylo = n1 >= 5 ? c1 - 2 : 0, ycnt = n1 >= 5 ? 5 : n1;
-  const double reach = sqrt(cutallsq > ddcutsq ? cutallsq : ddcutsq) + 1e-6;
-  const double reach2 = wave_uniform(reach * reach);
+  const int n0 = HOSTC ? kc.n[0] : g.nc[0], n1 = HOSTC ? kc.n[1] : g.nc[1], n2 = HOSTC ? kc.n[2] : g.nc[2];
+  const bool full0 = HOSTC ? kc.full[0] != 0 : n0 >= 5, full1 = HOSTC ? kc.full[1] != 0 : n1 >= 5, full2 = HOSTC ? kc.full[2] != 0 : n2 >= 5;
+  const int zlo = full2 ? c2 - 2 : 0, zcnt = HOSTC ? kc.cnt[2] : (n2 >= 5 ? 5 : n2);
+  const int ylo = full1 ? c1 - 2 : 0, ycnt = HOSTC ? kc.cnt[1] : (n1 >= 5 ? 5 : n1);
+  double reach2 = kc.reach2;
+  if (!HOSTC) {
+    const double reach = sqrt(cutallsq > ddcutsq ? cutallsq : ddcutsq) + 1e-6;
+    reach2 = wave_uniform(reach * reach);
+  }
   const int nsr = zcnt * ycnt;
   int ra0 = 0, rb0 = 0, ra1 = 0, rb1 = 0;
   if (lane < nsr) {
@@ -554,12 +559,12 @@
     if (b2 < 0 || b2 >= n2) { if (!box.periodic[2]) ok = false; b2 = b2 < 0 ? b2 + n2 : b2 - n2; }
     if (b1 < 0 || b1 >= n1) { if (!box.periodic[1]) ok = false; b1 = b1 < 0 ? b1 + n1 : b1 - n1; }
     double dzmin = 0.0, dymin = 0.0;
-    if (n2 >= 5) { const int d = zz - c2; dzmin = d > 0 ? (d - uu[2]) * edge[2] : (d < 0 ? (uu[2] - (d + 1)) * edge[2] : 0.0); }
-    if (n1 >= 5) { const int d = yy - c1; dymin = d > 0 ? (d - uu[1]) * edge[1] : (d < 0 ? (uu[1] - (d + 1)) * edge[1] : 0.0); }
+    if (full2) { const int d = zz - c2; dzmin = d > 0 ? (d - uu[2]) * edge[2] : (d < 0 ? (uu[2] - (d + 1)) * edge[2] : 0.0); }
+    if (full1) { const int d = yy - c1; dymin = d > 0 ? (d - uu[1]) * edge[1] : (d < 0 ? (uu[1] - (d + 1)) * edge[1] : 0.0); }
     const double rem2 = reach2 - dzmin * dzmin - dymin * dymin;
     if (g.trim && rem2 < 0.0) ok = false;
-    int xlo = n0 >= 5 ? c0 - 2 : 0, xhi = n0 >= 5 ? c0 + 2 : n0 - 1;
-    if (ok && g.trim && n0 >= 5) {
+    int xlo = full0 ? c0 - 2 : 0, xhi = full0 ? c0 + 2 : n0 - 1;
+    if (ok && g.trim && full0) {
       const double xr = sqrt(rem2) / edge[0];
       int lo_off = (int)floor(uu[0] - xr), hi_off = (int)floor(uu[0] + xr);
       lo_off = lo_off < -2 ? -2 : lo_off; hi_off = hi_off > 2 ? 2 : hi_off;
diff --git a/lammps-induced-dipole-polarization-pair-style_amd/csrc/polar_plan.hpp b/lammps-induced-dipole-polarization-pair-style_amd/csrc/polar_plan.hpp
--- a/lammps-induced-dipole-polarization-pair-style_amd/csrc/polar_plan.hpp
+++ b/lammps-induced-dipole-polarization-pair-style_amd/csrc/polar_plan.hpp
@@ -47,6 +47,31 @@
 }
 inline bool cell_bins_fit(long long ncell, bool split) { return cell_bins(ncell, split).nbins < (1ll << 31) - 1; }
 
+struct NlRowConsts {
+  double edge[3];
+  double reach2;
+  double pinv[3];
+  int n[3];
+  int full[3];
+  int cnt[3];
+};
+template <class B>
+inline NlRowConsts nl_row_consts(const B &box, const int nc[3], double cutallsq, double ddcutsq) {
+  NlRowConsts c;
+  for (int k = 0; k < 3; k++) {
+    c.edge[k] = box.prd[k] / nc[k];
+    c.pinv[k] = box.periodic[k] ? box.inv[k] : 0.0;
+    c.n[k] = nc[k];
+    c.full[k] = nc[k] >= 5;
+    c.cnt[k] = nc[k] >= 5 ? 5 : nc[k];
+  }
+  const double reach = std::sqrt(cutallsq > ddcutsq ? cutallsq : ddcutsq) + 1e-6;
+  c.reach2 = reach * reach;
+  return c;
+}
+
+inline bool pitch_ok(long long pitch) { return pitch >= 64 && pitch % 64 == 0; }
+inline size_t row_list_words(long long n, long long pitch) { return (size_t)n * (size_t)pitch + 64; }
 inline long long pitch_first(double mean, double factor) { return (((long long)(factor * mean) + 64) / 64 + 1) * 64; }
 inline long long pitch_grown(int flag) { return ((long long)(1.25 * flag) / 64 + 1) * 64; }
 inline int pitch_forced(int value) { return ((std::max(64, value) + 63) / 64) * 64; }
diff --git a/lammps-induced-dipole-polarization-pair-style_amd/csrc/polar_rows.hpp b/lammps-induced-dipole-polarization-pair-style_amd/csrc/polar_rows.hpp
--- a/lammps-induced-dipole-polarization-pair-style_amd/csrc/polar_rows.hpp
+++ b/lammps-induced-dipole-polarization-pair-style_amd/csrc/polar_rows.hpp
@@ -7,9 +7,15 @@
 #include "lab/force_pair_literal.hpp"
 #define POLAR_LIT_PARAM , int literal
 #define POLAR_LIT_PASS , literal
+#define POLAR_SPEC_PARAM , int row_spec
+#define POLAR_SPEC_PASS , row_spec
+#define POLAR_SPEC_ON (row_spec != 0)
 #else
 #define POLAR_LIT_PARAM
 #define POLAR_LIT_PASS
+#define POLAR_SPEC_PARAM
+#define POLAR_SPEC_PASS
+#define POLAR_SPEC_ON true
 #endif
 
 namespace polar {
@@ -494,17 +500,23 @@
                                                               double e2s, double gamma, int use_previous,
                                                               double *__restrict__ ef, AtomRec *__restrict__ rec0,
                                                               AtomRec *__restrict__ rec1, const double4 *__restrict__ xq_s,
-                                                              double g_ewald, const double *__restrict__ erec) {
+                                                              double g_ewald, const double *__restrict__ erec POLAR_SPEC_PARAM) {
   const int lane = threadIdx.x & 63;
   const int row = blockIdx.x * POLAR_ROWS_PER_BLOCK + (threadIdx.x >> 6);
   if (row >= nrows) return;
   const int i = rows ? rows[row] : row;
+  const bool spec = POLAR_SPEC_ON;
+  int w0 = 0, w1 = 0, wc = 0;
+  if (!ALLPAIRS && spec) { const int *wp = nl_j + (long long)i * nl.pitch + lane; w0 = wp[0]; w1 = wp[64]; wc = nl.cnt[i]; }
   const AtomRec ri = uniform_rec(rec[i]);
   const int mi = mol[i];
   const double f_shift = -1.0 / cut_coulsq;
   double ex = 0, ey = 0, ez = 0;
   long long beg = 0, end = nlocal;
-  if (!ALLPAIRS) row_range(nl, i, beg, end);
+  if (!ALLPAIRS) {
+    if (spec) { beg = (long long)i * nl.pitch; end = beg + (wc < nl.pitch ? wc : nl.pitch); }
+    else row_range(nl, i, beg, end);
+  }
   if (ALLPAIRS) {
     for (long long p = beg + lane; p < end; p += 64) {
       const int j = (int)p;
@@ -527,10 +539,17 @@
   } else {
     __shared__ double2 s_stage[POLAR_ROWS_PER_BLOCK][64 * 5];
     double2 *stage = s_stage[threadIdx.x >> 6];
+    int e_n1 = i, e_n2 = i;
+    if (spec) {
+      asm volatile("" : "+v"(w0), "+v"(w1));
+      e_n1 = beg + lane < end ? w0 : i; e_n2 = beg + lane + 64 < end ? w1 : i;
+    }
     for (long long base = beg; base < end; base += 64) {
       const long long p = base + lane;
       const bool valid = p < end;
-      const int e = valid ? nl_j[p] : i;
+      int e;
+      if (spec) { e = e_n1; e_n1 = e_n2; e_n2 = p + 128 < end ? nl_j[p + 128] : i; }
+      else e = valid ? nl_j[p] : i;
       const int j = e & POLAR_NL_MASK;
       double xj, yj, zj, qj;
       if (xq_s) { const XQ t = fetch_xq(xq_s, j, stage, lane); xj = t.a.x; yj = t.a.y; zj = t.b.x; qj = t.b.y; }
@@ -550,6 +569,21 @@
       }
     }
   }
+  if (spec) {
+    double e = wave_sum4(ex, ey, ez, 0.0, lane);
+    if (lane < 3) {
+      e *= e2s;
+      if (EW) e += erec[3 * i + lane];
+      ef[3 * i + lane] = e;
+      if (!use_previous) {
+        double m = ri.a * e;
+        m *= gamma;
+        reinterpret_cast<double *>(rec0 + i)[2 * lane + 1] = m;
+        reinterpret_cast<double *>(rec1 + i)[2 * lane + 1] = m;
+      }
+    }
+    return;
+  }
   ex = wave_sum(ex); ey = wave_sum(ey); ez = wave_sum(ez);
   if (lane == 0) {
     ex *= e2s; ey *= e2s; ez *= e2s;
@@ -573,9 +607,9 @@
                                                               const int *__restrict__ nl_j, double cut_coulsq,
                                                               double e2s, double gamma, int use_previous,
                                                               double *__restrict__ ef, AtomRec *__restrict__ rec0,
-                                                              AtomRec *__restrict__ rec1, const double4 *__restrict__ xq_s) {
+                                                              AtomRec *__restrict__ rec1, const double4 *__restrict__ xq_s POLAR_SPEC_PARAM) {
   static_field_body<ALLPAIRS, false>(rows, nrows, nlocal, rec, mol, box, nl, nl_j, cut_coulsq, e2s, gamma, use_previous, ef, rec0, rec1,
-                                     xq_s, 0.0, nullptr);
+                                     xq_s, 0.0, nullptr POLAR_SPEC_PASS);
 }
 template <bool ALLPAIRS>
 static __global__ __launch_bounds__(POLAR_BLOCK) void k_ew_static_field(const int *__restrict__ rows, int nrows, int nlocal,
@@ -586,9 +620,9 @@
                                                                  double e2s, double gamma, int use_previous,
                                                                  double *__restrict__ ef, AtomRec *__restrict__ rec0,
                                                                  AtomRec *__restrict__ rec1, const double4 *__restrict__ xq_s,
-                                                                 double g_ewald, const double *__restrict__ erec) {
+                                                                 double g_ewald, const double *__restrict__ erec POLAR_SPEC_PARAM) {
   static_field_body<ALLPAIRS, true>(rows, nrows, nlocal, rec, mol, box, nl, nl_j, cut_coulsq, e2s, gamma, use_previous, ef, rec0, rec1,
-                                    xq_s, g_ewald, erec);
+                                    xq_s, g_ewald, erec POLAR_SPEC_PASS);
 }
 
 struct PairMath {
@@ -610,11 +644,14 @@
                                                              double ddcutsq, double pd, double e2s,
                                                              double *__restrict__ f, double *__restrict__ slots,
                                                              double *__restrict__ vatom, int vglobal, ExpCoef K,
-                                                             double *__restrict__ dbg6, double g_ewald, int skip_inert POLAR_LIT_PARAM) {
+                                                             double *__restrict__ dbg6, double g_ewald, int skip_inert POLAR_LIT_PARAM POLAR_SPEC_PARAM) {
   const int lane = threadIdx.x & 63;
   const int row = blockIdx.x * POLAR_ROWS_PER_BLOCK + (threadIdx.x >> 6);
   if (row >= nrows) return;
   const int i = rows ? rows[row] : row;
+  const bool spec = POLAR_SPEC_ON;
+  int w0 = 0, w1 = 0, wc = 0;
+  if (!ALLPAIRS && spec) { const int *wp = nl_j + (long long)i * nl.pitch + lane; w0 = wp[0]; w1 = wp[64]; wc = nl.cnt[i]; }
   const AtomRec *__restrict__ rec = __builtin_amdgcn_readfirstlane(scal_in->cur) ? recB : recA;
   const AtomRec ri = uniform_rec(rec[i]);
   if (skip_inert && site_is_inert(ri.q, ri.a)) return;
@@ -627,7 +664,10 @@
   const bool isdbg = dbg6 && (perm ? perm[i] : i) == 0;
   double ddx = 0, ddy = 0, ddz = 0;
   long long beg = 0, end = nlocal;
-  if (!ALLPAIRS) row_range(nl, i, beg, end);
+  if (!ALLPAIRS) {
+    if (spec) { beg = (long long)i * nl.pitch; end = beg + (wc < nl.pitch ? wc : nl.pitch); }
+    else row_range(nl, i, beg, end);
+  }
   Box pbox = box;
   if (!ALLPAIRS) {
 #pragma unroll
@@ -635,8 +675,13 @@
   }
   int e_n1 = i, e_n2 = i;
   if (!ALLPAIRS) {
-    if (beg + lane < end) e_n1 = nl_j[beg + lane];
-    if (beg + lane + 64 < end) e_n2 = nl_j[beg + lane + 64];
+    if (spec) {
+      if (beg + lane < end) e_n1 = w0;
+      if (beg + lane + 64 < end) e_n2 = w1;
+    } else {
+      if (beg + lane < end) e_n1 = nl_j[beg + lane];
+      if (beg + lane + 64 < end) e_n2 = nl_j[beg + lane + 64];
+    }
   }
   AtomRec r_n1 = rec[e_n1 & POLAR_NL_MASK];
   for (long long p = beg + lane; p < end; p += 64) {
@@ -672,21 +717,40 @@
     }
   }
   fx += ddx; fy += ddy; fz += ddz;
-  fx = wave_sum(fx); fy = wave_sum(fy); fz = wave_sum(fz);
-  if (lane == 0) {
+  if (spec) {
+    const double s4 = wave_sum4(fx, fy, fz, EFLAG ? uef : 0.0, lane);
     const int o = perm ? perm[i] : i;
-    atomicAdd(&f[3 * o], fx); atomicAdd(&f[3 * o + 1], fy); atomicAdd(&f[3 * o + 2], fz);
-  }
-  if (isdbg) {
-    ddx = wave_sum(ddx); ddy = wave_sum(ddy); ddz = wave_sum(ddz);
-    if (lane == 0) { dbg6[0] = fx; dbg6[1] = fy; dbg6[2] = fz; dbg6[3] = ddx; dbg6[4] = ddy; dbg6[5] = ddz; }
-  }
-  if (EFLAG) {
-    uef = wave_sum(uef); udd = wave_sum(udd);
+    if (lane < 3) atomicAdd(&f[3 * o + lane], s4);
+    if (isdbg) {
+      if (lane < 3) dbg6[lane] = s4;
+      ddx = wave_sum(ddx); ddy = wave_sum(ddy); ddz = wave_sum(ddz);
+      if (lane == 0) { dbg6[3] = ddx; dbg6[4] = ddy; dbg6[5] = ddz; }
+    }
+    if (EFLAG) {
+      udd = wave_sum(udd);
+      if (lane == 3) atomicAdd(slot_ptr(slots, SL_UEF), 0.5 * s4);
+      if (lane == 0) {
+        if (ri.a != 0.0) atomicAdd(slot_ptr(slots, SL_USELF), 0.5 * (ri.mx * ri.mx + ri.my * ri.my + ri.mz * ri.mz) / ri.a);
+        atomicAdd(slot_ptr(slots, SL_UDD), 0.5 * udd);
+      }
+    }
+  } else {
+    fx = wave_sum(fx); fy = wave_sum(fy); fz = wave_sum(fz);
     if (lane == 0) {
-      if (ri.a != 0.0) atomicAdd(slot_ptr(slots, SL_USELF), 0.5 * (ri.mx * ri.mx + ri.my * ri.my + ri.mz * ri.mz) / ri.a);
-      atomicAdd(slot_ptr(slots, SL_UEF), 0.5 * uef);
-      atomicAdd(slot_ptr(slots, SL_UDD), 0.5 * udd);
+      const int o = perm ? perm[i] : i;
+      atomicAdd(&f[3 * o], fx); atomicAdd(&f[3 * o + 1], fy); atomicAdd(&f[3 * o + 2], fz);
+    }
+    if (isdbg) {
+      ddx = wave_sum(ddx); ddy = wave_sum(ddy); ddz = wave_sum(ddz);
+      if (lane == 0) { dbg6[0] = fx; dbg6[1] = fy; dbg6[2] = fz; dbg6[3] = ddx; dbg6[4] = ddy; dbg6[5] = ddz; }
+    }
+    if (EFLAG) {
+      uef = wave_sum(uef); udd = wave_sum(udd);
+      if (lane == 0) {
+        if (ri.a != 0.0) atomicAdd(slot_ptr(slots, SL_USELF), 0.5 * (ri.mx * ri.mx + ri.my * ri.my + ri.mz * ri.mz) / ri.a);
+        atomicAdd(slot_ptr(slots, SL_UEF), 0.5 * uef);
+        atomicAdd(slot_ptr(slots, SL_UDD), 0.5 * udd);
+      }
     }
   }
   if (VPAIR) {
@@ -709,16 +773,16 @@
     const int *__restrict__ rows, int nrows, const int *__restrict__ perm, int nlocal, const Scal *scal_in,
     const AtomRec *__restrict__ recA, const AtomRec *__restrict__ recB, const int *__restrict__ mol, Box box, RowList nl,
     const int *__restrict__ nl_j, double cut_coulsq, double ddcutsq, double pd, double e2s, double *__restrict__ f,
-    double *__restrict__ slots, double *__restrict__ vatom, int vglobal, ExpCoef K, double *__restrict__ dbg6, int skip_inert POLAR_LIT_PARAM) {
-  polar_force_body<ALLPAIRS, DAMP, EFLAG, VPAIR, false>(rows, nrows, perm, nlocal, scal_in, recA, recB, mol, box, nl, nl_j, cut_coulsq, ddcutsq, pd, e2s, f, slots, vatom, vglobal, K, dbg6, 0.0, skip_inert POLAR_LIT_PASS);
+    double *__restrict__ slots, double *__restrict__ vatom, int vglobal, ExpCoef K, double *__restrict__ dbg6, int skip_inert POLAR_LIT_PARAM POLAR_SPEC_PARAM) {
+  polar_force_body<ALLPAIRS, DAMP, EFLAG, VPAIR, false>(rows, nrows, perm, nlocal, scal_in, recA, recB, mol, box, nl, nl_j, cut_coulsq, ddcutsq, pd, e2s, f, slots, vatom, vglobal, K, dbg6, 0.0, skip_inert POLAR_LIT_PASS POLAR_SPEC_PASS);
 }
 template <bool ALLPAIRS, int DAMP, bool EFLAG, bool VPAIR>
 static __global__ __launch_bounds__(POLAR_BLOCK) void k_ew_polar_force(
     const int *__restrict__ rows, int nrows, const int *__restrict__ perm, int nlocal, const Scal *scal_in,
     const AtomRec *__restrict__ recA, const AtomRec *__restrict__ recB, const int *__restrict__ mol, Box box, RowList nl,
     const int *__restrict__ nl_j, double cut_coulsq, double ddcutsq, double pd, double e2s, double *__restrict__ f,
-    double *__restrict__ slots, double *__restrict__ vatom, int vglobal, ExpCoef K, double *__restrict__ dbg6, double g_ewald, int skip_inert POLAR_LIT_PARAM) {
-  polar_force_body<ALLPAIRS, DAMP, EFLAG, VPAIR, true>(rows, nrows, perm, nlocal, scal_in, recA, recB, mol, box, nl, nl_j, cut_coulsq, ddcutsq, pd, e2s, f, slots, vatom, vglobal, K, dbg6, g_ewald, skip_inert POLAR_LIT_PASS);
+    double *__restrict__ slots, double *__restrict__ vatom, int vglobal, ExpCoef K, double *__restrict__ dbg6, double g_ewald, int skip_inert POLAR_LIT_PARAM POLAR_SPEC_PARAM) {
+  polar_force_body<ALLPAIRS, DAMP, EFLAG, VPAIR, true>(rows, nrows, perm, nlocal, scal_in, recA, recB, mol, box, nl, nl_j, cut_coulsq, ddcutsq, pd, e2s, f, slots, vatom, vglobal, K, dbg6, g_ewald, skip_inert POLAR_LIT_PASS POLAR_SPEC_PASS);
 }
 
 static __global__ void k_add_into(long long n, const double *__restrict__ src, double *__restrict__ dst) {
@@ -746,3 +810,6 @@
 
 #undef POLAR_LIT_PARAM
 #undef POLAR_LIT_PASS
+#undef POLAR_SPEC_PARAM
+#undef POLAR_SPEC_PASS
+#undef POLAR_SPEC_ON
diff --git a/lammps-induced-dipole-polarization-pair-style_amd/csrc/polar_step.hip b/lammps-induced-dipole-polarization-pair-style_amd/csrc/polar_step.hip
--- a/lammps-induced-dipole-polarization-pair-style_amd/csrc/polar_step.hip
+++ b/lammps-induced-dipole-polarization-pair-style_amd/csrc/polar_step.hip
@@ -112,7 +112,8 @@
   if ((h->sweep_kernel == 2 || h->sweep_kernel == 3) && ((long long)n + 1) * (long long)sizeof(AtomRec) >= (1ll << 31))
     throw InputError("more than 2^25 atoms on one handle: the 32-bit record offsets of the sweep's index stream would wrap (shard the system)");
   h->d_nl_cnt.ensure(n + 1); h->d_dd_cnt.ensure(n + 1);
-  h->d_nl_j.ensure((size_t)n * h->nl_pitch + 64);
+  if (!pitch_ok(h->nl_pitch)) throw std::logic_error("build_lists: the list pitch is not a positive multiple of 64");
+  h->d_nl_j.ensure(row_list_words(n, h->nl_pitch));
   if (h->sweep_kernel < 3) h->d_dd_j.ensure((size_t)n * h->dd_pitch + 1024);
   else h->d_dd_j.ensure(64);
   const int mode = h->stream_mode = stream_mode(h->cache_r2, h->sweep_kernel, h->dd_pairs, own_n(h), h->dd_pitch);
@@ -140,22 +141,27 @@
   }
   if (((long long)n + 1) * (long long)sizeof(double4) >= (1ll << 32))
     throw InputError("more than 2^27 atoms on one handle: the 32-bit position offsets of the list build would wrap (shard the system)");
-#define NLB3(TRI, RC, DENSE)                                                                                                  \
-  k_nl_build<TRI, RC, DENSE><<<nblk(nr, POLAR_ROWS_PER_BLOCK), POLAR_BLOCK, 0, s>>>(                                          \
-      rows, nr, h->d_pos4.p, h->box, g, h->d_cell_first.p, cutallsq, ddsq, h->nl_pitch, h->dd_pitch, h->d_nl_cnt.p,            \
+  const NlRowConsts kc = nl_row_consts(h->box, g.nc, cutallsq, ddsq);
+#define NLB4(TRI, RC, DENSE, HOSTC)                                                                                           \
+  k_nl_build<TRI, RC, DENSE, HOSTC><<<nblk(nr, POLAR_ROWS_PER_BLOCK), POLAR_BLOCK, 0, s>>>(                                   \
+      rows, nr, h->d_pos4.p, h->box, g, kc, h->d_cell_first.p, cutallsq, ddsq, h->nl_pitch, h->dd_pitch, h->d_nl_cnt.p,            \
       h->d_dd_cnt.p, h->d_nl_j.p, h->d_dd_j.p, fuse ? r2p : nullptr, fuse ? 1 : 0, lp ? (6 | (h->lp_quad_major << 8)) : 0,    \
       lp ? n : -1, lp ? h->d_dd_wrap.p : nullptr, recheck ? h->d_color_s.p : nullptr, h->color_keep * h->color_keep,           \
       h->d_overflow.p + 8, lp ? h->d_slot.p : nullptr, h->d_overflow.p, h->d_ddtot.p)
 #ifdef POLAR_LAB
+#define NLB3(TRI, RC, DENSE) do { if (h->row_consts) NLB4(TRI, RC, DENSE, true); else NLB4(TRI, RC, DENSE, false); } while (0)
 #define NLB(TRI, RC) do { if (h->nl_dense) NLB3(TRI, RC, true); else NLB3(TRI, RC, false); } while (0)
   h->nl_dense_used = h->nl_dense ? 1.0 : 0.0;
+  h->row_consts_used = h->row_consts ? 1.0 : 0.0;
+  h->row_spec_used = h->row_spec ? 1.0 : 0.0;
 #else
-#define NLB(TRI, RC) NLB3(TRI, RC, true)
+#define NLB(TRI, RC) NLB4(TRI, RC, true, true)
 #endif
   if (h->box.triclinic) { if (recheck) NLB(true, true); else NLB(true, false); }
   else                  { if (recheck) NLB(false, true); else NLB(false, false); }
 #undef NLB
 #undef NLB3
+#undef NLB4
   const RowList ddl{h->d_dd_cnt.p, h->dd_pitch};
   if (fuse || mode == 4) {
   }
@@ -363,7 +369,7 @@
   const bool ew = ewald_on(h);
   const double g = h->P.g_ewald;
 #ifdef POLAR_LAB
-#define POLAR_LIT_ARG , h->force_literal
+#define POLAR_LIT_ARG , h->force_literal, h->row_spec
 #else
 #define POLAR_LIT_ARG
 #endif
@@ -850,17 +856,23 @@
 
   HIPCHECK(hipEventRecord(h->ev[3], s));
 
+#ifdef POLAR_LAB
+#define POLAR_SPEC_ARG , h->row_spec
+#else
+#define POLAR_SPEC_ARG
+#endif
   {
     dim3 grid(nblk(own_n(h), POLAR_ROWS_PER_BLOCK)), block(POLAR_BLOCK);
     const double ccs = st.cut_coul * st.cut_coul, e2s = std::sqrt(h->P.qqrd2e);
     if (ewald_on(h)) {
       ewald_field(h);
       const double g = h->P.g_ewald;
-      if (ap) k_ew_static_field<true><<<grid, block, 0, s>>>(nullptr, n, n, h->d_rec0.p, h->d_mol_s.p, h->box, RowList{nullptr, 0}, nullptr, ccs, e2s, st.polar_gamma, st.use_previous, h->d_ef_s.p, h->d_rec0.p, h->d_rec1.p, nullptr, g, h->d_ew_erec.p);
-      else    k_ew_static_field<false><<<grid, block, 0, s>>>(own_rows(h), own_n(h), n, h->d_rec0.p, h->d_mol_s.p, h->box, RowList{h->d_nl_cnt.p, h->nl_pitch}, h->d_nl_j.p, ccs, e2s, st.polar_gamma, st.use_previous, h->d_ef_s.p, h->d_rec0.p, h->d_rec1.p, h->static_xq ? h->d_xq_s.p : nullptr, g, h->d_ew_erec.p);
-    } else if (ap) k_static_field<true><<<grid, block, 0, s>>>(nullptr, n, n, h->d_rec0.p, h->d_mol_s.p, h->box, RowList{nullptr, 0}, nullptr, ccs, e2s, st.polar_gamma, st.use_previous, h->d_ef_s.p, h->d_rec0.p, h->d_rec1.p, nullptr);
-    else    k_static_field<false><<<grid, block, 0, s>>>(own_rows(h), own_n(h), n, h->d_rec0.p, h->d_mol_s.p, h->box, RowList{h->d_nl_cnt.p, h->nl_pitch}, h->d_nl_j.p, ccs, e2s, st.polar_gamma, st.use_previous, h->d_ef_s.p, h->d_rec0.p, h->d_rec1.p, h->static_xq ? h->d_xq_s.p : nullptr);
-  }
+      if (ap) k_ew_static_field<true><<<grid, block, 0, s>>>(nullptr, n, n, h->d_rec0.p, h->d_mol_s.p, h->box, RowList{nullptr, 0}, nullptr, ccs, e2s, st.polar_gamma, st.use_previous, h->d_ef_s.p, h->d_rec0.p, h->d_rec1.p, nullptr, g, h->d_ew_erec.p POLAR_SPEC_ARG);
+      else    k_ew_static_field<false><<<grid, block, 0, s>>>(own_rows(h), own_n(h), n, h->d_rec0.p, h->d_mol_s.p, h->box, RowList{h->d_nl_cnt.p, h->nl_pitch}, h->d_nl_j.p, ccs, e2s, st.polar_gamma, st.use_previous, h->d_ef_s.p, h->d_rec0.p, h->d_rec1.p, h->static_xq ? h->d_xq_s.p : nullptr, g, h->d_ew_erec.p POLAR_SPEC_ARG);
+    } else if (ap) k_static_field<true><<<grid, block, 0, s>>>(nullptr, n, n, h->d_rec0.p, h->d_mol_s.p, h->box, RowList{nullptr, 0}, nullptr, ccs, e2s, st.polar_gamma, st.use_previous, h->d_ef_s.p, h->d_rec0.p, h->d_rec1.p, nullptr POLAR_SPEC_ARG);
+    else    k_static_field<false><<<grid, block, 0, s>>>(own_rows(h), own_n(h), n, h->d_rec0.p, h->d_mol_s.p, h->box, RowList{h->d_nl_cnt.p, h->nl_pitch}, h->d_nl_j.p, ccs, e2s, st.polar_gamma, st.use_previous, h->d_ef_s.p, h->d_rec0.p, h->d_rec1.p, h->static_xq ? h->d_xq_s.p : nullptr POLAR_SPEC_ARG);
+  }
+#undef POLAR_SPEC_ARG
 #ifdef POLAR_LAB
   if (!ap && h->sweep_kernel == 4 && !st.zodid)
     k_srec_pack<<<nblk(n, 256), 256, 0, s>>>(n, h->d_rec0.p, h->d_srec0.p, h->d_srec1.p);
```

After: 17.23 million, median of 6. Within noise of the previous version (+0.7%).
